# lambdaclass/AES_zero_knowledge_proof_circuit

Measured on AMD Instinct MI355X. Metric: AES-ECB blocks proven/sec (Marlin), proof verifies, higher is better.
Workload: dtype u32 limbs (253-bit Fr / 377-bit Fq modular integers)

## Files before the change

### aes_zero_knowledge_proof_circuit_amd/api.py

```python
import ctypes as C
import os

import numpy as np

HERE = os.path.dirname(os.path.abspath(__file__))
CIRCUIT_AES, CIRCUIT_OPS_XOR, CIRCUIT_OPS_ADD = 0, 1, 2
CIRCUIT_AES_CBC = 3
CIRCUIT_AES_CTR = 4
CIRCUIT_AES_GCM = 5
KEY_NO_TABLES = 1
PARITY = "parity"


class ZkAesError(RuntimeError):
    """The Err(..) side of the reference's anyhow::Result."""


def lib_path():
    return os.path.join(HERE, "libzkaes.so")


_lib = None


# ... 369 lines not shown
def verify_chunked_tagged(verifying_key, circuit, proofs, ciphertext, key_tag, iv=None):
    if len(key_tag) not in (16, 32):
        raise ZkAesError("key_tag must be 16 or 32 bytes")
    if iv is not None and len(iv) != 16:
        raise ZkAesError("iv / icb must be 16 bytes")
    n = len(proofs)
    lens = (C.c_size_t * max(n, 1))(*[len(p) for p in proofs])
    each = (C.c_int * max(n, 1))()
    ok = C.c_size_t()
    _check(lib().zkaes_verify_chunked_kt(verifying_key._p, int(circuit), b"".join(bytes(p) for p in proofs), lens, C.c_size_t(n), None if iv is None else bytes(iv), bytes(ciphertext),
                                         C.c_size_t(len(ciphertext)), bytes(key_tag), C.c_size_t(len(key_tag)), each, C.byref(ok)))
    return [bool(each[i]) for i in range(n)]


def _host_key(secret_key):
    if len(secret_key) not in (16, 24, 32):
        raise ZkAesError("secret_key must be 16, 24 or 32 bytes")


def ecb_ciphertext(message, secret_key):
    _host_key(secret_key)
    ct = C.create_string_buffer(max(len(message), 1))
    _check(lib().zkaes_ecb_ciphertext_ks(bytes(message), C.c_size_t(len(message)), bytes(secret_key), C.c_size_t(len(secret_key)), ct))
    return ct.raw[:len(message)]


def encrypt(message, secret_key, proving_key, zk_seed=None):
    proving_key._need_key(secret_key)
    out, n = C.c_void_p(), C.c_size_t()
    _check(lib().zkaes_encrypt_seeded(bytes(message), C.c_size_t(len(message)), bytes(secret_key), proving_key._p, zk_seed, C.byref(out), C.byref(n)))
    return _take(out, n)


def verify_encryption(verifying_key, proof, ciphertext):
    acc = C.c_int()
    _check(lib().zkaes_verify_encryption(verifying_key._p, bytes(proof), C.c_size_t(len(proof)), bytes(ciphertext), C.c_size_t(len(ciphertext)), C.byref(acc)))
    return bool(acc.value)


def cbc_ciphertext(message, secret_key, iv):
    if len(secret_key) not in (16, 24, 32) or len(iv) != 16:
        raise ZkAesError("secret_key must be 16, 24 or 32 bytes and iv 16 bytes")
    ct = C.create_string_buffer(max(len(message), 1))
    _check(lib().zkaes_cbc_ciphertext_ks(bytes(message), C.c_size_t(len(message)), bytes(secret_key), C.c_size_t(len(secret_key)), bytes(iv), ct))
    return ct.raw[:len(message)]


def encrypt_cbc(message, secret_key, iv, proving_key, zk_seed=None):
    proving_key._need_key(secret_key, iv, "iv")
    ct = C.create_string_buffer(max(len(message), 1))
    out, n = C.c_void_p(), C.c_size_t()
    _check(lib().zkaes_encrypt_cbc_seeded(bytes(message), C.c_size_t(len(message)), bytes(secret_key), bytes(iv), proving_key._p, zk_seed, ct, C.byref(out), C.byref(n)))
    return ct.raw[:len(message)], _take(out, n)


def verify_encryption_cbc(verifying_key, proof, iv, ciphertext):
    if len(iv) != 16:
        raise ZkAesError("iv must be 16 bytes")
    acc = C.c_int()
    _check(lib().zkaes_verify_encryption_cbc(verifying_key._p, bytes(proof), C.c_size_t(len(proof)), bytes(iv), bytes(ciphertext), C.c_size_t(len(ciphertext)), C.byref(acc)))
    return bool(acc.value)


def verify_cbc_chunked(verifying_key, proofs, iv, ciphertext):
    if len(iv) != 16:
        raise ZkAesError("iv must be 16 bytes")
    n = len(proofs)
    lens = (C.c_size_t * max(n, 1))(*[len(p) for p in proofs])
    each = (C.c_int * max(n, 1))()
    ok = C.c_size_t()
    _check(lib().zkaes_verify_cbc_chunked(verifying_key._p, b"".join(bytes(p) for p in proofs), lens, C.c_size_t(n), bytes(iv), bytes(ciphertext), C.c_size_t(len(ciphertext)), each, C.byref(ok)))
    return [bool(each[i]) for i in range(n)]


def ctr_crypt(data, secret_key, icb):
    if len(secret_key) not in (16, 24, 32) or len(icb) != 16:
        raise ZkAesError("secret_key must be 16, 24 or 32 bytes and icb 16 bytes")
    out = C.create_string_buffer(max(len(data), 1))
    _check(lib().zkaes_ctr_crypt_ks(bytes(data), C.c_size_t(len(data)), bytes(secret_key), C.c_size_t(len(secret_key)), bytes(icb), out))
    return out.raw[:len(data)]


def ctr_counter_add(icb, n_blocks):
    if len(icb) != 16 or not 0 <= n_blocks < 1 << 64:
        raise ZkAesError("icb must be 16 bytes and n_blocks a 64-bit count")
    out = C.create_string_buffer(16)
    _check(lib().zkaes_ctr_counter_add(bytes(icb), C.c_uint64(n_blocks), out))
    return out.raw


def encrypt_ctr(message, secret_key, icb, proving_key, zk_seed=None):
    proving_key._need_key(secret_key, icb, "icb")
    ct = C.create_string_buffer(max(len(message), 1))
    out, n = C.c_void_p(), C.c_size_t()
    _check(lib().zkaes_encrypt_ctr_seeded(bytes(message), C.c_size_t(len(message)), bytes(secret_key), bytes(icb), proving_key._p, zk_seed, ct, C.byref(out), C.byref(n)))
    return ct.raw[:len(message)], _take(out, n)


def verify_encryption_ctr(verifying_key, proof, icb, ciphertext):
    if len(icb) != 16:
        raise ZkAesError("icb must be 16 bytes")
    acc = C.c_int()
    _check(lib().zkaes_verify_encryption_ctr(verifying_key._p, bytes(proof), C.c_size_t(len(proof)), bytes(icb), bytes(ciphertext), C.c_size_t(len(ciphertext)), C.byref(acc)))
    return bool(acc.value)


def verify_ctr_chunked(verifying_key, proofs, icb, ciphertext):
    if len(icb) != 16:
        raise ZkAesError("icb must be 16 bytes")
    n = len(proofs)
    lens = (C.c_size_t * max(n, 1))(*[len(p) for p in proofs])
    each = (C.c_int * max(n, 1))()
    ok = C.c_size_t()
    _check(lib().zkaes_verify_ctr_chunked(verifying_key._p, b"".join(bytes(p) for p in proofs), lens, C.c_size_t(n), bytes(icb), bytes(ciphertext), C.c_size_t(len(ciphertext)), each, C.byref(ok)))
    return [bool(each[i]) for i in range(n)]


def _gcm_args(secret_key, iv, key_bytes=None):
    if key_bytes is None:
        _host_key(secret_key)
    elif len(secret_key) != key_bytes:
        raise ZkAesError("secret_key must be %d bytes" % key_bytes)
    if len(iv) != 12:
        raise ZkAesError("GCM: only 96-bit (12-byte) IVs are supported")


def synthesize_keys_gcm(plaintext_length, aad_length=0, srs=(866_944, 513, 4_062_064), flags=0, key_bits=128, key_tag_blocks=0):
    return _synthesize(CIRCUIT_AES_GCM, key_bits, plaintext_length, aad_length, srs, flags, key_tag_blocks)


def gcm_encrypt(message, secret_key, iv, aad=b""):
    _gcm_args(secret_key, iv)
    ct, tag = C.create_string_buffer(max(len(message), 1)), C.create_string_buffer(16)
    _check(lib().zkaes_gcm_encrypt_ks(bytes(message), C.c_size_t(len(message)), bytes(secret_key), C.c_size_t(len(secret_key)), bytes(iv), bytes(aad), C.c_size_t(len(aad)), ct, tag))
    return ct.raw[:len(message)], tag.raw


def gcm_decrypt(ciphertext, secret_key, iv, aad, tag):
    _gcm_args(secret_key, iv)
    if len(tag) != 16:
        raise ZkAesError("GCM: only full 16-byte tags are supported")
    msg, ok = C.create_string_buffer(max(len(ciphertext), 1)), C.c_int()
    _check(lib().zkaes_gcm_decrypt_ks(bytes(ciphertext), C.c_size_t(len(ciphertext)), bytes(secret_key), C.c_size_t(len(secret_key)), bytes(iv), bytes(aad), C.c_size_t(len(aad)), bytes(tag),
                                      msg, C.byref(ok)))
    if not ok.value:
        return None
    return msg.raw[:len(ciphertext)]


def encrypt_gcm(message, secret_key, iv, aad, proving_key, zk_seed=None):
    _gcm_args(secret_key, iv, proving_key.key_bytes())
    ct, tag = C.create_string_buffer(max(len(message), 1)), C.create_string_buffer(16)
    out, n = C.c_void_p(), C.c_size_t()
    _check(lib().zkaes_encrypt_gcm_seeded(bytes(message), C.c_size_t(len(message)), bytes(secret_key), bytes(iv), bytes(aad), C.c_size_t(len(aad)), proving_key._p, zk_seed, ct, tag,
                                          C.byref(out), C.byref(n)))
    return ct.raw[:len(message)], tag.raw, _take(out, n)


def verify_encryption_gcm(verifying_key, proof, iv, aad, ciphertext, tag):
    if len(iv) != 12:
        raise ZkAesError("GCM: only 96-bit (12-byte) IVs are supported")
    if len(tag) != 16:
        raise ZkAesError("GCM: only full 16-byte tags are supported")
    acc = C.c_int()
    _check(lib().zkaes_verify_encryption_gcm(verifying_key._p, bytes(proof), C.c_size_t(len(proof)), bytes(iv), bytes(aad), C.c_size_t(len(aad)), bytes(ciphertext),
                                             C.c_size_t(len(ciphertext)), bytes(tag), C.byref(acc)))
    return bool(acc.value)


def verify_encryption_gcm_tagged(verifying_key, proof, iv, aad, ciphertext, tag, key_tag):
    if len(iv) != 12:
        raise ZkAesError("GCM: only 96-bit (12-byte) IVs are supported")
    if len(tag) != 16:
        raise ZkAesError("GCM: only full 16-byte tags are supported")
    if len(key_tag) not in (16, 32):
        raise ZkAesError("key_tag must be 16 or 32 bytes")
    acc = C.c_int()
    _check(lib().zkaes_verify_encryption_gcm_kt(verifying_key._p, bytes(proof), C.c_size_t(len(proof)), bytes(iv), bytes(aad), C.c_size_t(len(aad)), bytes(ciphertext),
                                                C.c_size_t(len(ciphertext)), bytes(tag), bytes(key_tag), C.c_size_t(len(key_tag)), C.byref(acc)))
    return bool(acc.value)


def proof_roundtrip(proof):
    out, n = C.c_void_p(), C.c_size_t()
    _check(lib().zkaes_proof_roundtrip(bytes(proof), C.c_size_t(len(proof)), C.byref(out), C.byref(n)))
    return _take(out, n)


def circuit_info(circuit, plaintext_length, aad_length=0, key_bits=128, key_tag_blocks=0):
    out = (C.c_uint64 * 12)()
    _check(lib().zkaes_circuit_info_kt(int(circuit), C.c_uint(int(key_bits)), _tag_blocks(key_tag_blocks), C.c_size_t(plaintext_length), C.c_size_t(aad_length), out))
    keys = ["raw_constraints", "raw_instance", "raw_witness", "nnz_a", "nnz_b", "nnz_c", "constraints", "instance", "witness", "joint_nnz", "h", "k"]
    return dict(zip(keys, out))


def circuit_matrix(circuit, plaintext_length, which, aad_length=0, key_bits=128, key_tag_blocks=0):
    rows, nnz = C.c_uint64(), C.c_uint64()
    head = (int(circuit), C.c_uint(int(key_bits)), _tag_blocks(key_tag_blocks), C.c_size_t(plaintext_length), C.c_size_t(aad_length), which)
    _check(lib().zkaes_circuit_matrix_kt(*head, C.byref(rows), C.byref(nnz), None, None, None))
    rowptr = np.zeros(rows.value + 1, dtype=np.uint32)
    col = np.zeros(max(nnz.value, 1), dtype=np.uint32)
    coeff = np.zeros(max(nnz.value, 1), dtype=np.int64)
    _check(lib().zkaes_circuit_matrix_kt(*head, None, None, rowptr.ctypes.data_as(C.c_void_p), col.ctypes.data_as(C.c_void_p), coeff.ctypes.data_as(C.c_void_p)))
    return rowptr, col[:nnz.value], coeff[:nnz.value]


def ntt(field_id, data_mont_bytes, inverse=False):
    n = len(data_mont_bytes) // 32
    buf = C.create_string_buffer(bytes(data_mont_bytes), len(data_mont_bytes))
    _check(lib().zkaes_ntt(int(field_id), buf, C.c_size_t(n), 1 if inverse else 0))
    return buf.raw


def ntt_coset(field_id, data_mont_bytes, coset_c, lg_big, inverse=False):
    n = len(data_mont_bytes) // 32
    buf = C.create_string_buffer(bytes(data_mont_bytes), len(data_mont_bytes))
    _check(lib().zkaes_ntt_coset(int(field_id), buf, C.c_size_t(n), 1 if inverse else 0, int(coset_c), int(lg_big)))
    return buf.raw


def ntt_batch(field_id, vectors, cosets=None, lg_big=0, inverse=False):
    count, n = len(vectors), len(vectors[0]) // 32
    if any(len(v) != 32 * n for v in vectors):
        raise ZkAesError("ntt_batch: vectors of one length")
    buf = C.create_string_buffer(b"".join(bytes(v) for v in vectors), 32 * n * count)
    cs = (C.c_int * count)(*[int(c) for c in cosets]) if cosets is not None else None
    _check(lib().zkaes_ntt_batch(int(field_id), buf, C.c_size_t(n), count, 1 if inverse else 0, cs, int(lg_big)))
    return [buf.raw[32 * n * i:32 * n * (i + 1)] for i in range(count)]


def _ptr_array(bufs):
    n = len(bufs)
    return (C.c_char_p * n)(*[bytes(b) if len(b) else None for b in bufs]), (C.c_size_t * n)(*[len(b) // 32 for b in bufs])


def poly_divide_by_vanishing(p, m, with_scratch=False, want_rem=True):
    n = len(p) // 32
    q = C.create_string_buffer(32 * max(n - m, 0) or 1)
    rem = C.create_string_buffer(32 * m or 1) if want_rem else None
    _check(lib().zkaes_poly_divide_by_vanishing(bytes(p), C.c_size_t(n), C.c_size_t(m), 1 if with_scratch else 0, q, rem))
    return q.raw[:32 * (n - m)], (rem.raw[:32 * m] if want_rem else None)


def poly_divide_by_linear(p, z):
    n = len(p) // 32
    q = C.create_string_buffer(32 * max(n - 1, 0) or 1)
    _check(lib().zkaes_poly_divide_by_linear(bytes(p), C.c_size_t(n), bytes(z), q))
    return q.raw[:32 * max(n - 1, 0)]


def poly_eval_multi(polys, xs):
    count = len(polys)
    ptrs, lens = _ptr_array(polys)
    out = C.create_string_buffer(32 * max(count, 1))
    _check(lib().zkaes_poly_eval_multi(ptrs, lens, b"".join(bytes(x) for x in xs), count, out))
    return [out.raw[32 * i:32 * i + 32] for i in range(count)]


def batch_inverse(v, post=None, throughput_variant=False):
    n = len(v) // 32
    buf = C.create_string_buffer(bytes(v), max(len(v), 1))
    _check(lib().zkaes_batch_inverse(buf, C.c_size_t(n), None if post is None else bytes(post), 1 if throughput_variant else 0))
    return buf.raw[:32 * n]


def poly_lincomb(polys, scalars, n):
    count = len(polys)
    ptrs, lens = _ptr_array(polys)
    out = C.create_string_buffer(32 * n or 1)
    _check(lib().zkaes_poly_lincomb(ptrs, lens, b"".join(bytes(x) for x in scalars), count, C.c_size_t(n), out))
    return out.raw[:32 * n]


def vanishing_quotient_evals(lg_n, gs, a, indices=None):
    ncosets, per = len(gs), (1 << lg_n) if indices is None else len(indices)
    out = C.create_string_buffer(32 * per * ncosets or 1)
    idx = None if indices is None else (C.c_uint32 * max(per, 1))(*indices)
    _check(lib().zkaes_vanishing_quotient_evals(int(lg_n), b"".join(bytes(g) for g in gs), ncosets, bytes(a), idx, C.c_size_t(0 if indices is None else per), out))
    return [out.raw[32 * per * c:32 * per * (c + 1)] for c in range(ncosets)]


def q1_coset_pointwise(r, za, zb, t, z, ca, cb, cz, eta_a, eta_b, eta_c):
    n = len(r) // 32
    out = C.create_string_buffer(32 * n or 1)
    consts = b"".join(bytes(x) for x in (ca, cb, cz, eta_a, eta_b, eta_c))
    _check(lib().zkaes_q1_coset_pointwise(bytes(r), bytes(za), bytes(zb), bytes(t), bytes(z), consts, C.c_size_t(n), out))
    return out.raw[:32 * n]


def h2_coset(row, col, va, vb, vc, rc, f, alpha, beta, alpha_beta, ea, eb, ec, vinv):
    k = len(row) // 32
    out = C.create_string_buffer(32 * k or 1)
    arrays = (C.c_char_p * 7)(*[bytes(x) for x in (row, col, va, vb, vc, rc, f)])
    consts = b"".join(bytes(x) for x in (alpha, beta, alpha_beta, ea, eb, ec, vinv))
    _check(lib().zkaes_h2_coset(arrays, consts, C.c_size_t(k), out))
    return out.raw[:32 * k]


def q1_combine(q0, q1, q3, mask, inv2, inv2zeta):
    n = len(q0) // 32
    h1, g1 = C.create_string_buffer(64 * n or 1), C.create_string_buffer(32 * max(n - 1, 0) or 1)
    _check(lib().zkaes_q1_combine(bytes(q0), bytes(q1), bytes(q3), bytes(mask), bytes(inv2), bytes(inv2zeta), C.c_size_t(n), h1, g1))
    return h1.raw[:64 * n], g1.raw[:32 * max(n - 1, 0)]


def coset_scale(data, g, n):
    out = C.create_string_buffer(32 * n or 1)
    _check(lib().zkaes_coset_scale(bytes(data), C.c_size_t(len(data) // 32), bytes(g), C.c_size_t(n), out))
    return out.raw[:32 * n]


def z_poly_from_w(w, x_poly, n):
    out = C.create_string_buffer(32 * (n + 1))
    _check(lib().zkaes_z_poly_from_w(bytes(w), C.c_size_t(len(w) // 32), bytes(x_poly), C.c_uint32(len(x_poly) // 32), C.c_size_t(n), out))
    return out.raw


def ntt_padded(field_id, data_mont_bytes, n, inverse=False, coset_c=0, lg_big=0):
    out = C.create_string_buffer(32 * n)
    _check(lib().zkaes_ntt_padded(int(field_id), bytes(data_mont_bytes), C.c_size_t(len(data_mont_bytes) // 32), C.c_size_t(n), 1 if inverse else 0, int(coset_c), int(lg_big), out))
    return out.raw


def ntt_scaled(g, data_mont_bytes, n, inverse=False):
    out = C.create_string_buffer(32 * n)
    _check(lib().zkaes_ntt_scaled(bytes(g), bytes(data_mont_bytes), C.c_size_t(len(data_mont_bytes) // 32), C.c_size_t(n), 1 if inverse else 0, out))
    return out.raw


def _arith_ops():
    t = {}
    for base, f, n in ((0, "fr377", 8), (16, "fr381", 8), (32, "fq377", 12), (48, "fq381", 12)):
        for i, (name, nin) in enumerate((("mul", 2 * n), ("add", 2 * n), ("sub", 2 * n), ("neg", n), ("dbl", n), ("inverse", n), ("from_i64", 2), ("pow_u64", n + 2), ("from_raw", n), ("to_raw", n))):
            t["%s.%s" % (f, name)] = (base + i, nin, n)
    for base, f in ((64, "fq377x28"), (96, "fq381x28")):
        ops = [("mul", 28, 14), ("sqr", 14, 14), ("fma2", 56, 14), ("add", 28, 14), ("add_lazy", 28, 14), ("dbl_lazy", 14, 14)]
        ops += [("sub%d" % k, 28, 14) for k in (2, 3, 4, 5, 6, 7)] + [("sub_lazy%d" % k, 28, 14) for k in (2, 3)]
        ops += [("canonical", 14, 14), ("product_is_zero", 14, 1), ("is_zero_mod_p", 14, 1), ("from_std", 12, 14), ("to_std", 14, 12)]
        if f == "fq377x28":
            ops.append(("mul_biased", 28, 14))
        for i, (name, nin, nout) in enumerate(ops):
            t["%s.%s" % (f, name)] = (base + i, nin, nout)
    for base, f in ((128, "fr377x29"), (160, "fr381x29")):
        ops = [("mul", 18, 9), ("dot2", 36, 9), ("dot3", 54, 9), ("dot4", 72, 9), ("add", 18, 9), ("add_lazy", 18, 9)]
        ops += [("sub%d" % k, 18, 9) for k in (1, 2, 4, 8)] + [("sub_lazy2", 18, 9), ("normalized", 9, 9), ("shl5", 9, 9)]
        ops += [("canonical%d" % k, 9, 9) for k in (0, 1, 4)] + [("reduce_by_top_limb", 9, 9), ("twiddle_from_std", 8, 9), ("split", 8, 9), ("pack", 9, 8)]
        for i, (name, nin, nout) in enumerate(ops):
            t["%s.%s" % (f, name)] = (base + i, nin, nout)
    for i, (name, nin, nout) in enumerate((("te_madd", 98, 56), ("te_add", 112, 56), ("te_dbl", 56, 56), ("te_neg", 56, 56), ("te_to_std_point", 56, 48), ("niels_from_weierstrass", 24, 43),
                                           ("te_madd_hot", 142, 98), ("te_add_quad", 112, 56), ("te_dbl_quad", 56, 56))):
        t["te377.%s" % name] = (192 + i, nin, nout)
    for base, f in ((208, "w377"), (216, "w381")):
        for i, (name, nin, nout) in enumerate((("madd28", 84, 57), ("add28", 112, 56), ("dbl28", 56, 56), ("neg28", 56, 56), ("to_std_point", 56, 48))):
            t["%s.%s" % (f, name)] = (base + i, nin, nout)
    return t


ARITH_OPS = _arith_ops()
ARITH_QUAD_OPS = ("te377.te_add_quad", "te377.te_dbl_quad")


def arith_probe(op_name, cases):
    op, nin, nout = ARITH_OPS[op_name]
    cases = bytes(cases)
    n, rest = divmod(len(cases), 4 * nin)
    if rest:
        raise ZkAesError("arith_probe: %s takes %d words per case" % (op_name, nin))
    out = C.create_string_buffer(4 * nout * n or 1)
    _check(lib().zkaes_arith_probe(int(op), cases, C.c_size_t(n), out))
    return out.raw[:4 * nout * n]


def msm(curve_id, bases_bytes, scalars_bytes):
    n = len(scalars_bytes) // 32
    out = C.create_string_buffer(96)
    inf = C.c_int()
    _check(lib().zkaes_msm(int(curve_id), bytes(bases_bytes), bytes(scalars_bytes), C.c_size_t(n), out, C.byref(inf)))
    return out.raw, bool(inf.value)


def g1_sum(curve_id, points):
    n = len(points)
    buf = b"".join(bytes(p[0]) for p in points)
    inf = (C.c_int * max(n, 1))(*[1 if p[1] else 0 for p in points])
    out = C.create_string_buffer(96)
    oinf = C.c_int()
    _check(lib().zkaes_g1_sum(int(curve_id), buf, inf, C.c_size_t(n), out, C.byref(oinf)))
    return out.raw, bool(oinf.value)


def msm_sharded_plan(curve_id, n_total):
    c, w, b = C.c_int(), C.c_int(), C.c_size_t()
    _check(lib().zkaes_msm_sharded_plan(int(curve_id), C.c_size_t(n_total), C.byref(c), C.byref(w), C.byref(b)))
    return c.value, w.value, b.value


def msm_window_sums_dev(curve_id, bases_bytes, scalars_bytes, n_total, dev_ptr, dev_bytes):
    n = len(scalars_bytes) // 32
    _check(lib().zkaes_msm_window_sums_dev(int(curve_id), bytes(bases_bytes), bytes(scalars_bytes), C.c_size_t(n), C.c_size_t(n_total), C.c_void_p(dev_ptr), C.c_size_t(dev_bytes)))


def msm_fold_window_sums_dev(curve_id, dev_ptr, world, n_total):
    out = C.create_string_buffer(96)
    inf = C.c_int()
    _check(lib().zkaes_msm_fold_window_sums_dev(int(curve_id), C.c_void_p(dev_ptr), int(world), C.c_size_t(n_total), out, C.byref(inf)))
    return out.raw, bool(inf.value)


def msm_fold_partials_dev(curve_id, dev_ptr, world):
    out = C.create_string_buffer(96)
    inf = C.c_int()
    _check(lib().zkaes_msm_fold_partials_dev(int(curve_id), C.c_void_p(dev_ptr), int(world), out, C.byref(inf)))
    return out.raw, bool(inf.value)


def msm_table(curve_id, bases_bytes, scalars_bytes, window_bits, srs=False):
    n = len(scalars_bytes) // 32
    out = C.create_string_buffer(96)
    inf = C.c_int()
    if srs:
        if int(curve_id) != 377:
            raise ValueError("the SRS (twisted Edwards) table path exists for BLS12-377 only")
        _check(lib().zkaes_msm_table_srs(bytes(bases_bytes), bytes(scalars_bytes), C.c_size_t(n), int(window_bits), out, C.byref(inf)))
    else:
        _check(lib().zkaes_msm_table(int(curve_id), bytes(bases_bytes), bytes(scalars_bytes), C.c_size_t(n), int(window_bits), out, C.byref(inf)))
    return out.raw, bool(inf.value)


def _host(buf):
    if isinstance(buf, np.ndarray):
        if not buf.flags["C_CONTIGUOUS"]:
            raise ValueError("array arguments must be C-contiguous")
        return buf.ctypes.data_as(C.c_void_p)
    return bytes(buf)


def _nbytes(buf):
    return buf.nbytes if isinstance(buf, np.ndarray) else len(buf)


def class_sum(bases, vals, edwards=True, prior_msm_points=0):
    n, count = _nbytes(bases) // 96, len(vals)
    v = np.ascontiguousarray(np.stack([np.asarray(x, dtype=np.int8) for x in vals])) if count else np.zeros((0, n), dtype=np.int8)
    if count and v.shape[1] != n:
        raise ValueError("every value vector needs one value per base")
    ok, inf, out = (C.c_int * max(count, 1))(), (C.c_int * max(count, 1))(), C.create_string_buffer(96 * max(count, 1))
    _check(lib().zkaes_class_sum(_host(bases), C.c_size_t(n), v.ctypes.data_as(C.c_void_p), int(count), 1 if edwards else 0, C.c_size_t(prior_msm_points), ok, out, inf))
    return [(bool(ok[i]), out.raw[96 * i:96 * i + 96], bool(inf[i])) for i in range(count)]


def msm_pair(bases, scal1, scal2, val_off2, edwards=True):
    out, inf = C.create_string_buffer(96), C.c_int()
    _check(lib().zkaes_msm_pair(_host(bases), C.c_size_t(_nbytes(bases) // 96), bytes(scal1), C.c_size_t(len(scal1) // 32), bytes(scal2), C.c_size_t(len(scal2) // 32), C.c_size_t(val_off2),
                                1 if edwards else 0, out, C.byref(inf)))
    return out.raw, bool(inf.value)


def msm_table_pair(bases, scal1, off1, scal2, off2, window_bits, edwards=True):
    out, inf = C.create_string_buffer(96), C.c_int()
    _check(lib().zkaes_msm_table_pair(_host(bases), C.c_size_t(_nbytes(bases) // 96), bytes(scal1), C.c_size_t(len(scal1) // 32), C.c_size_t(off1), bytes(scal2), C.c_size_t(len(scal2) // 32),
                                      C.c_size_t(off2), int(window_bits), 1 if edwards else 0, out, C.byref(inf)))
    return out.raw, bool(inf.value)


def msm_second_bases(bases, scalars, off, shift, window_bits=0):
    out, inf = C.create_string_buffer(192), (C.c_int * 2)()
    _check(lib().zkaes_msm_second_bases(_host(bases), C.c_size_t(_nbytes(bases) // 96), bytes(scalars), C.c_size_t(len(scalars) // 32), C.c_size_t(off), C.c_size_t(shift), int(window_bits), out, inf))
    return [(out.raw[96 * i:96 * i + 96], bool(inf[i])) for i in range(2)]


def msm_bench(curve_id, bases_bytes, scalars_bytes, reps=3):
    n = len(scalars_bytes) // 32
    t, a = C.c_double(), C.c_double()
    _check(lib().zkaes_msm_bench(int(curve_id), bytes(bases_bytes), bytes(scalars_bytes), C.c_size_t(n), int(reps), C.byref(t), C.byref(a)))
    return t.value, a.value


def msm_bench_synth(n, window_bits=0, reps=3, want_point=False):
    t, a = C.c_double(), C.c_double()
    out = C.create_string_buffer(96)
    _check(lib().zkaes_msm_bench_synth(C.c_size_t(n), int(window_bits), int(reps), C.byref(t), C.byref(a), out))
    return (t.value, a.value, out.raw) if want_point else (t.value, a.value)


def set_default_contexts(n):
    _check(lib().zkaes_set_default_contexts(C.c_size_t(n)))


def srs_hold(hold=True):
    _check(lib().zkaes_srs_hold(1 if hold else 0))


def int_rate_bench(seconds=0.5):
    out = (C.c_double * 8)()
    _check(lib().zkaes_int_rate_bench(C.c_double(seconds), out))
    return {"fq_products_per_s": out[0], "fq_stream_sclk_mhz": out[1], "mad_per_s": 378.0 * out[0], "hot_loop_l2_additions_per_s": out[2], "hot_loop_l2_sclk_mhz": out[3],
            "hot_loop_cycles_per_addition_per_wave": out[4], "rounds": int(out[5])}


def stream_copy_bench(nbytes=1 << 30, reps=20):
    g = C.c_double()
    _check(lib().zkaes_stream_copy_bench(C.c_size_t(nbytes), int(reps), C.byref(g)))
    return g.value


def mem_info():
    f, t = C.c_uint64(), C.c_uint64()
    _check(lib().zkaes_mem_info(C.byref(f), C.byref(t)))
    return int(f.value), int(t.value)


def msm_stats(reset=False):
    out = (C.c_double * 5)()
    _check(lib().zkaes_msm_stats(out, 1 if reset else 0))
    return dict(accumulate_ms=out[0], total_ms=out[1], points=int(out[2]), launches=int(out[3]), pairs=int(out[4]))
```

### aes_zero_knowledge_proof_circuit_amd/build.py

```python
import os
import subprocess
import sys
from concurrent.futures import ThreadPoolExecutor

HERE = os.path.dirname(os.path.abspath(__file__))
CSRC = os.path.join(HERE, "csrc")
OUT = os.path.join(HERE, "libzkaes.so")
OBJ = os.path.join(CSRC, "build")
HIPCC = os.environ.get("HIPCC", "/opt/rocm/bin/hipcc")
HIP_SOURCES = ["runtime.hip", "kernels_ntt.hip", "kernels_msm.hip", "kernels_poly.hip", "kernels_witness.hip", "capi_kernels.hip", "capi_probe.hip"]
CXX_SOURCES = ["circuit.cpp", "marlin.cpp", "marlin_codec.cpp", "capi.cpp", "capi_host.cpp"]
HOST_ONLY_SOURCES = ["circuit.cpp", "marlin_codec.cpp", "capi_host.cpp"]
HEADERS = ["ff.cuh", "ff28.cuh", "ff29.cuh", "ec.cuh", "ec28.cuh", "te28.cuh", "gpu.hpp", "hip_util.hpp", "consts32.h", "trace_layout.h", "circuit.hpp", "marlin.hpp", "marlin_host.hpp", "capi_common.hpp", "pairing.hpp", "transcript.hpp", "arith_probe.cuh",
           os.path.join("..", "..", "include", "zkaes.h")]
COMMON = ["-O3", "-std=c++17", "-fPIC", "-I", CSRC, "-Wno-unused-result"]
if os.environ.get("ZK_EXTRA_DEFINES"):
    COMMON += os.environ["ZK_EXTRA_DEFINES"].split()


def _newer(target, deps):
    if not os.path.exists(target):
        return True
    t = os.path.getmtime(target)
    return any(os.path.getmtime(d) > t for d in deps)


def _compile(src):
    obj = os.path.join(OBJ, src + ".o")
    deps = [os.path.join(CSRC, src)] + [os.path.join(CSRC, h) for h in HEADERS]
    if not _newer(obj, deps):
        return obj
    if src.endswith(".hip"):
        cmd = [HIPCC, "--offload-arch=gfx950", "-x", "hip"] + COMMON + ["-c", os.path.join(CSRC, src), "-o", obj]
    else:
        cmd = [HIPCC, "-x", "c++"] + COMMON + ["-c", os.path.join(CSRC, src), "-o", obj]
    subprocess.check_call(cmd)
    return obj


def build(force=False):
    os.makedirs(OBJ, exist_ok=True)
    if force:
        for f in os.listdir(OBJ):
            os.remove(os.path.join(OBJ, f))
    with ThreadPoolExecutor(max_workers=8) as ex:
        objs = list(ex.map(_compile, HIP_SOURCES + CXX_SOURCES))
    if force or _newer(OUT, objs):
        subprocess.check_call([HIPCC, "--offload-arch=gfx950", "-shared", "-fPIC", "-o", OUT] + objs)
    return OUT


if __name__ == "__main__":
    print(build(force="--force" in sys.argv))
```

### aes_zero_knowledge_proof_circuit_amd/csrc/capi_kernels.hip

```cpp
#include "../../include/zkaes.h"
#include <cstring>
#include <string>
#include <type_traits>
#include <vector>
#include "hip_util.hpp"
#include "marlin.hpp"
#include "te28.cuh"
#include <algorithm>
#include <chrono>

typedef unsigned int v4u __attribute__((ext_vector_type(4)));
__global__ void __launch_bounds__(256) k_stream_copy(uint4 *__restrict__ dst_, const uint4 *__restrict__ src_, size_t n16) {
    v4u *dst = (v4u *)dst_; const v4u *src = (const v4u *)src_;
    size_t base = (size_t)blockIdx.x * 1024 + threadIdx.x;
    if (base + 768 < n16) {
        v4u v0 = __builtin_nontemporal_load(src + base), v1 = __builtin_nontemporal_load(src + base + 256);
        v4u v2 = __builtin_nontemporal_load(src + base + 512), v3 = __builtin_nontemporal_load(src + base + 768);
        __builtin_nontemporal_store(v0, dst + base); __builtin_nontemporal_store(v1, dst + base + 256);
        __builtin_nontemporal_store(v2, dst + base + 512); __builtin_nontemporal_store(v3, dst + base + 768);
    } else {
        for (size_t i = base; i < n16; i += 256) dst[i] = src[i];
    }
}

// ... 237 lines not shown
    WorkspaceGuard ws;
    if (prior) {
        std::vector<MFr> sc(prior);
        uint64_t x = 88172645463325252ull;
        for (size_t i = 0; i < prior; i++) { for (int k = 0; k < 8; k += 2) { x ^= x << 13; x ^= x >> 7; x ^= x << 17; sc[i].l[k] = (uint32_t)x; sc[i].l[k + 1] = (uint32_t)(x >> 32); } sc[i].l[7] &= 0x0fffffffu; }
        DevPtr<MFr> ds = upload_scalars((const uint8_t *)sc.data(), prior, s);
        zk::gpu::sync(s);
        (void)zk::gpu::msm<MC>(ws, (const MsmBase<EDWARDS> *)dl.get(), (const MFr *)ds.get(), prior, s);
    }
    for (int v = 0; v < count; v++) {
        zk::XYZZ<MFq> r;
        const bool ok = zk::gpu::class_sum<MC>(ws, (const MsmBase<EDWARDS> *)dl.get(), (const int8_t *)dv.get() + (size_t)v * n, n, &r, s);
        ok_out[v] = ok ? 1 : 0;
        if (ok) give_affine(r.to_affine(), out_xy + 96 * (size_t)v, out_inf + v);
        else { memset(out_xy + 96 * (size_t)v, 0, 96); out_inf[v] = 0; }
    }
}
template <bool EDWARDS>
void run_msm_pair(const uint8_t *bases, size_t nbases, const uint8_t *scal1, size_t n1, const uint8_t *scal2, size_t n2, size_t val_off2, uint8_t *out_xy, int *out_inf) {
    zk::gpu::require_device();
    StreamGuard s;
    DevPtr<zk::Affine<MFq>> db = upload_points(bases, nbases, nbases, s);
    DevPtr<MsmBase<EDWARDS>> dl = law_bases<EDWARDS>(db, nbases, s);
    DevPtr<MFr> d1 = upload_scalars(scal1, n1, s), d2 = upload_scalars(scal2, n2, s);
    zk::gpu::sync(s);
    WorkspaceGuard ws;
    zk::gpu::msm_prepare<MC>(ws, d1, n1, n2 ? d2.get() : nullptr, n2, n2 ? val_off2 : 0, s);
    give_affine(zk::gpu::msm_finish<MC>(ws, (const MsmBase<EDWARDS> *)dl.get(), s).to_affine(), out_xy, out_inf);
}
template <bool EDWARDS> DevPtr<MsmBase<EDWARDS>> law_tables(const uint8_t *bases, size_t stride, int c, zk::gpu::stream_t s) {
    const size_t nt = (size_t)zk::gpu::table_windows<MC>(c);
    DevPtr<zk::Affine<MFq>> tab = upload_points(bases, stride, nt * stride, s);
    zk::gpu::build_window_tables<MC>(tab, stride, c, s);
    return law_bases<EDWARDS>(tab, nt * stride, s);
}
template <bool EDWARDS>
void run_msm_table_pair(const uint8_t *bases, size_t stride, const uint8_t *scal1, size_t n1, size_t off1, const uint8_t *scal2, size_t n2, size_t off2, int c, uint8_t *out_xy, int *out_inf) {
    zk::gpu::require_device();
    StreamGuard s;
    DevPtr<MsmBase<EDWARDS>> tabs = law_tables<EDWARDS>(bases, stride, c, s);
    DevPtr<MFr> d1 = upload_scalars(scal1, n1, s), d2 = upload_scalars(scal2, n2, s);
    zk::gpu::sync(s);
    WorkspaceGuard ws;
    zk::gpu::msm_prepare_table<MC>(ws, d1, n1, off1, n2 ? d2.get() : nullptr, n2, n2 ? off2 : 0, c, stride, s);
    give_affine(zk::gpu::msm_finish<MC>(ws, (const MsmBase<EDWARDS> *)tabs.get(), s).to_affine(), out_xy, out_inf);
}
void run_msm_second_bases(const uint8_t *bases, size_t nbases, const uint8_t *scalars, size_t n, size_t off, size_t shift, int c, uint8_t *out_xy, int *out_inf) {
    zk::gpu::require_device();
    StreamGuard s;
    DevPtr<MFr> ds = upload_scalars(scalars, n, s);
    WorkspaceGuard ws;
    zk::XYZZ<MFq> r[2];
    if (c == 0) {
        DevPtr<zk::Affine<MFq>> db = upload_points(bases, nbases, nbases, s);
        DevPtr<zk::Niels28<MP>> dl = law_bases<true>(db, nbases, s);
        zk::gpu::msm_prepare<MC>(ws, ds, n, nullptr, 0, 0, s);
        zk::gpu::msm_finish2<MC>(ws, dl.get() + off, dl.get() + off + shift, r, s);
    } else {
        DevPtr<zk::Niels28<MP>> tabs = law_tables<true>(bases, nbases, c, s);
        zk::gpu::msm_prepare_table<MC>(ws, ds, n, off, nullptr, 0, 0, c, nbases, s);
        zk::gpu::msm_finish2<MC>(ws, tabs.get(), tabs.get() + shift, r, s);
    }
    for (int i = 0; i < 2; i++) give_affine(r[i].to_affine(), out_xy + 96 * i, out_inf + i);
}
}

extern "C" {
int zkaes_class_sum(const uint8_t *bases, size_t n, const int8_t *vals, int count, int edwards, size_t prior_msm_points, int *ok_out, uint8_t *out_xy, int *out_inf) {
    return guardk([&] {
        const char *who = "zkaes_class_sum";
        need(count >= 1 && count <= 8, who, "1..8 value vectors");
        need(bases && vals && ok_out && out_xy && out_inf, who, "null argument");
        need(n >= 1 && n <= MSM_FORM_MAX, who, "n out of range");
        need(prior_msm_points <= n, who, "the prior MSM runs over the same bases: at most n points");
        if (edwards) run_class_sum<true>(bases, n, vals, count, prior_msm_points, ok_out, out_xy, out_inf);
        else run_class_sum<false>(bases, n, vals, count, prior_msm_points, ok_out, out_xy, out_inf);
    });
}
int zkaes_msm_pair(const uint8_t *bases, size_t nbases, const uint8_t *scal1, size_t n1, const uint8_t *scal2, size_t n2, size_t val_off2, int edwards, uint8_t *out_xy, int *out_inf) {
    return guardk([&] {
        const char *who = "zkaes_msm_pair";
        need(out_xy && out_inf && (bases || !nbases) && (scal1 || !n1) && (scal2 || !n2), who, "null argument");
        need(nbases <= MSM_FORM_MAX, who, "too many bases");
        need(n1 <= nbases && val_off2 <= nbases && n2 <= nbases - val_off2, who, "range exceeds the bases");
        if (edwards) run_msm_pair<true>(bases, nbases, scal1, n1, scal2, n2, val_off2, out_xy, out_inf);
        else run_msm_pair<false>(bases, nbases, scal1, n1, scal2, n2, val_off2, out_xy, out_inf);
    });
}
int zkaes_msm_table_pair(const uint8_t *bases, size_t stride, const uint8_t *scal1, size_t n1, size_t off1, const uint8_t *scal2, size_t n2, size_t off2, int window_bits, int edwards,
                         uint8_t *out_xy, int *out_inf) {
    return guardk([&] {
        const char *who = "zkaes_msm_table_pair";
        need(out_xy && out_inf && (bases || !stride) && (scal1 || !n1) && (scal2 || !n2), who, "null argument");
        need(stride <= MSM_FORM_MAX, who, "too many bases");
        check_table_bits(window_bits, stride, who);
        if (off1 > stride || n1 > stride - off1 || off2 > stride || n2 > stride - off2) throw std::invalid_argument("msm_table: range exceeds the table");
        if (edwards) run_msm_table_pair<true>(bases, stride, scal1, n1, off1, scal2, n2, off2, window_bits, out_xy, out_inf);
        else run_msm_table_pair<false>(bases, stride, scal1, n1, off1, scal2, n2, off2, window_bits, out_xy, out_inf);
    });
}
int zkaes_msm_second_bases(const uint8_t *bases, size_t nbases, const uint8_t *scalars, size_t n, size_t off, size_t shift, int window_bits, uint8_t *out_xy, int *out_inf) {
    return guardk([&] {
        const char *who = "zkaes_msm_second_bases";
        need(out_xy && out_inf && (bases || !nbases) && (scalars || !n), who, "null argument");
        need(nbases <= MSM_FORM_MAX, who, "too many bases");
        if (window_bits) check_table_bits(window_bits, nbases, who);
        if (off > nbases || shift > nbases - off || n > nbases - off - shift) throw std::invalid_argument(window_bits ? "msm_table: range exceeds the table" : "zkaes_msm_second_bases: range exceeds the bases");
        run_msm_second_bases(bases, nbases, scalars, n, off, shift, window_bits, out_xy, out_inf);
    });
}
int zkaes_msm_sharded_plan(int curve_id, size_t n_total, int *window_bits, int *n_windows, size_t *bytes_per_rank) {
    return guardk([&] {
        int c = 0, w = 0;
        if (curve_id == 381) zk::gpu::msm_sharded_plan<zk::Bls381>(n_total, &c, &w); else if (curve_id == 377) zk::gpu::msm_sharded_plan<zk::Bls377>(n_total, &c, &w); else throw std::invalid_argument("curve_id must be 377 or 381");
        if (window_bits) *window_bits = c;
        if (n_windows) *n_windows = w;
        if (bytes_per_rank) *bytes_per_rank = (size_t)w * 192;
    });
}
int zkaes_msm_window_sums_dev(int curve_id, const uint8_t *bases, const uint8_t *scalars, size_t n_local, size_t n_total, void *dev_out, size_t dev_out_bytes) {
    return guardk([&] { if (curve_id == 381) run_msm_window_sums_dev<zk::Bls381>(bases, scalars, n_local, n_total, dev_out, dev_out_bytes); else if (curve_id == 377) run_msm_window_sums_dev<zk::Bls377>(bases, scalars, n_local, n_total, dev_out, dev_out_bytes); else throw std::invalid_argument("curve_id must be 377 or 381"); });
}
int zkaes_msm_fold_window_sums_dev(int curve_id, const void *dev_in, int world, size_t n_total, uint8_t *out_xy, int *out_inf) {
    return guardk([&] { if (curve_id == 381) run_msm_fold_dev<zk::Bls381>(dev_in, world, n_total, out_xy, out_inf); else if (curve_id == 377) run_msm_fold_dev<zk::Bls377>(dev_in, world, n_total, out_xy, out_inf); else throw std::invalid_argument("curve_id must be 377 or 381"); });
}
int zkaes_g1_sum(int curve_id, const uint8_t *points_xy, const int *inf, size_t n, uint8_t *out_xy, int *out_inf) {
    return guardk([&] { if (curve_id == 381) run_g1_sum<zk::Bls381>(points_xy, inf, n, out_xy, out_inf); else if (curve_id == 377) run_g1_sum<zk::Bls377>(points_xy, inf, n, out_xy, out_inf); else throw std::invalid_argument("curve_id must be 377 or 381"); });
}
int zkaes_msm_fold_partials_dev(int curve_id, const void *dev_in, int world, uint8_t *out_xy, int *out_inf) {
    return guardk([&] {
        if (!dev_in || world < 1 || world > MAX_FOLD_WORLD) throw std::invalid_argument("zkaes_msm_fold_partials_dev: bad arguments (world must be 1..4096)");
        if (curve_id != 377 && curve_id != 381) throw std::invalid_argument("curve_id must be 377 or 381");
        zk::gpu::require_device();
        StreamGuard s;
        if (curve_id == 377) give_affine(zk::gpu::msm_fold_points_device<zk::Bls377>((const zk::XYZZ<zk::Fq377> *)dev_in, world, s).to_affine(), out_xy, out_inf);
        else give_affine(zk::gpu::msm_fold_points_device<zk::Bls381>((const zk::XYZZ<zk::Fq381> *)dev_in, world, s).to_affine(), out_xy, out_inf);
    });
}
int zkaes_msm_table(int curve_id, const uint8_t *bases, const uint8_t *scalars, size_t n, int window_bits, uint8_t *out_xy, int *out_inf) {
    return guardk([&] { if (curve_id == 381) run_msm_table<zk::Bls381, false>(bases, scalars, n, window_bits, out_xy, out_inf); else if (curve_id == 377) run_msm_table<zk::Bls377, false>(bases, scalars, n, window_bits, out_xy, out_inf); else throw std::invalid_argument("curve_id must be 377 or 381"); });
}
int zkaes_msm_table_srs(const uint8_t *bases, const uint8_t *scalars, size_t n, int window_bits, uint8_t *out_xy, int *out_inf) {
    return guardk([&] { run_msm_table<zk::Bls377, true>(bases, scalars, n, window_bits, out_xy, out_inf); });
}
int zkaes_set_device(int ordinal) { return guardk([&] { HIP_CHECK(hipSetDevice(ordinal)); }); }
int zkaes_ntt(int field_id, uint8_t *data, size_t n, int inverse) {
    return guardk([&] { if (field_id == 381) run_ntt<zk::Fr381>(data, n, inverse, 0, 0); else if (field_id == 377) run_ntt<zk::Fr377>(data, n, inverse, 0, 0); else throw std::invalid_argument("field_id must be 377 or 381"); });
}
int zkaes_ntt_coset(int field_id, uint8_t *data, size_t n, int inverse, int coset_c, int lg_big) {
    return guardk([&] {
        if (coset_c <= 0) throw std::invalid_argument("zkaes_ntt_coset: coset index must be positive");
        if (field_id == 381) run_ntt<zk::Fr381>(data, n, inverse, coset_c, lg_big); else if (field_id == 377) run_ntt<zk::Fr377>(data, n, inverse, coset_c, lg_big); else throw std::invalid_argument("field_id must be 377 or 381");
    });
}
int zkaes_ntt_batch(int field_id, uint8_t *data, size_t n, int count, int inverse, const int *coset_c, int lg_big) {
    return guardk([&] {
        if (field_id == 381) run_ntt_batch<zk::Fr381>(data, n, count, inverse, coset_c, lg_big); else if (field_id == 377) run_ntt_batch<zk::Fr377>(data, n, count, inverse, coset_c, lg_big);
        else throw std::invalid_argument("field_id must be 377 or 381");
    });
}
int zkaes_poly_divide_by_vanishing(const uint8_t *p, size_t len, size_t m, int with_scratch, uint8_t *q, uint8_t *rem_or_null) {
    return guardk([&] {
        const char *who = "zkaes_poly_divide_by_vanishing";
        if (m == 0 || len <= m) throw std::invalid_argument("divide_by_vanishing: dividend shorter than divisor");
        need(p && q, who, "null argument"); need(len <= POLY_MAX, who, "polynomial too long");
        zk::gpu::require_device();
        StreamGuard s;
        DevPtr<PF> dp = upload(p, len, s), dq(len - m), drem(m), scratch;
        size_t scratch_len = 0;
        if (with_scratch) { scratch_len = zk::gpu::divide_by_vanishing_scratch(len, m); scratch.alloc(scratch_len ? scratch_len : 1); }
        zk::gpu::divide_by_vanishing(dq, rem_or_null ? drem.get() : nullptr, dp, len, m, s, with_scratch ? scratch.get() : nullptr, scratch_len);
        zk::gpu::d2h(q, dq, (len - m) * sizeof(PF), s);
        if (rem_or_null) zk::gpu::d2h(rem_or_null, drem, m * sizeof(PF), s);
    });
}
int zkaes_poly_divide_by_linear(const uint8_t *p, size_t len, const uint8_t z[32], uint8_t *q) {
    return guardk([&] {
        const char *who = "zkaes_poly_divide_by_linear";
        const PF zf = load_f(z, who);
        need(len <= POLY_MAX, who, "polynomial too long"); need(len < 2 || (p && q), who, "null argument");
        if (len < 2) return;
        zk::gpu::require_device();
        StreamGuard s;
        const size_t scratch_len = zk::gpu::divide_by_linear_scratch(len);
        DevPtr<PF> dp = upload(p, len, s), dq(len - 1), scratch(scratch_len);
        zk::gpu::divide_by_linear(dq, dp, len, zf, scratch, scratch_len, s);
        zk::gpu::d2h(q, dq, (len - 1) * sizeof(PF), s);
    });
}
int zkaes_poly_eval_multi(const uint8_t *const *polys, const size_t *lens, const uint8_t *x, int count, uint8_t *out) {
    return guardk([&] {
        const char *who = "zkaes_poly_eval_multi";
        need(count >= 1 && count <= 8, who, "1..8 polynomials"); need(polys && lens && x && out, who, "null argument");
        size_t scratch_len = 8;
        for (int i = 0; i < count; i++) { need(lens[i] <= POLY_MAX, who, "polynomial too long"); need(!lens[i] || polys[i], who, "null polynomial"); scratch_len += zk::gpu::poly_eval_scratch(lens[i]); }
        zk::gpu::require_device();
        StreamGuard s;
        DevPtr<PF> dp[8];
        const PF *ptr[8];
        PF xs[8], res[8];
        for (int i = 0; i < count; i++) { dp[i] = upload(polys[i], lens[i], s); ptr[i] = dp[i]; xs[i] = load_f(x + 32 * i, who); }
        DevPtr<PF> scratch(scratch_len);
        zk::gpu::poly_eval_multi(ptr, lens, xs, count, res, scratch, scratch_len, s);
        memcpy(out, res, (size_t)count * sizeof(PF));
    });
}
int zkaes_batch_inverse(uint8_t *v, size_t n, const uint8_t *post_or_null, int throughput_variant) {
    return guardk([&] {
        const char *who = "zkaes_batch_inverse";
        need(v || !n, who, "null argument"); need(n <= POLY_MAX, who, "vector too long");
        PF post; if (post_or_null) post = load_f(post_or_null, who);
        if (!n) return;
        zk::gpu::require_device();
        StreamGuard s;
        DevPtr<PF> dv = upload(v, n, s);
        {
            zk::gpu::ThroughputWaits as_between_overlapping_proofs(throughput_variant != 0);
            zk::gpu::batch_inverse(dv, n, post_or_null ? &post : nullptr, s);
            zk::gpu::sync(s);
        }
        zk::gpu::d2h(v, dv, n * sizeof(PF), s);
    });
}
int zkaes_poly_lincomb(const uint8_t *const *polys, const size_t *lens, const uint8_t *scalars, int count, size_t n, uint8_t *out) {
    return guardk([&] {
        const char *who = "zkaes_poly_lincomb";
        need(count >= 1 && count <= 8, who, "1..8 terms"); need(polys && lens && scalars && (out || !n), who, "null argument"); need(n <= POLY_MAX, who, "polynomial too long");
        for (int i = 0; i < count; i++) { need(lens[i] <= n, who, "a term longer than the result"); need(!lens[i] || polys[i], who, "null polynomial"); }
        if (!n) return;
        zk::gpu::require_device();
        StreamGuard s;
        DevPtr<PF> dp[8], dout(n);
        const PF *ptr[8];
        PF sc[8];
        for (int i = 0; i < count; i++) { dp[i] = upload(polys[i], lens[i], s); ptr[i] = dp[i]; sc[i] = load_f(scalars + 32 * i, who); }
        zk::gpu::poly_lincomb_n(dout, n, ptr, lens, sc, count, s);
        zk::gpu::d2h(out, dout, n * sizeof(PF), s);
    });
}
int zkaes_vanishing_quotient_evals(int lg_n, const uint8_t *g, int ncosets, const uint8_t a[32], const uint32_t *idx_or_null, size_t nidx, uint8_t *out) {
    return guardk([&] {
        const char *who = "zkaes_vanishing_quotient_evals";
        need(lg_n >= 0 && lg_n <= 24, who, "lg_n must be in [0, 24]"); need(ncosets >= 1 && ncosets <= 3, who, "1..3 cosets"); need(g && out, who, "null argument");
        const size_t n = (size_t)1 << lg_n;
        for (size_t i = 0; idx_or_null && i < nidx; i++) need(idx_or_null[i] < n, who, "index out of range");
        const PF af = load_f(a, who);
        PF gs[3];
        for (int c = 0; c < ncosets; c++) gs[c] = load_f(g + 32 * c, who);
        zk::gpu::require_device();
        StreamGuard s;
        const PF *elems = zk::gpu::domain_elements<zk::Fr377>(lg_n);
        const size_t scratch_len = zk::gpu::vanishing_quotient_scratch(lg_n, ncosets);
        DevPtr<PF> tabs[3], scratch(scratch_len);
        PF *outs[3] = {nullptr, nullptr, nullptr};
        for (int c = 0; c < ncosets; c++) { tabs[c].alloc(n); outs[c] = tabs[c]; }
        zk::gpu::vanishing_quotient_evals(outs, gs, ncosets, af, elems, (uint32_t)n, lg_n, scratch, scratch_len, s);
        if (!idx_or_null) { for (int c = 0; c < ncosets; c++) zk::gpu::d2h(out + (size_t)c * n * sizeof(PF), tabs[c], n * sizeof(PF), s); return; }
        std::vector<PF> host(n);
        for (int c = 0; c < ncosets; c++) {
            zk::gpu::d2h(host.data(), tabs[c], n * sizeof(PF), s);
            for (size_t i = 0; i < nidx; i++) memcpy(out + ((size_t)c * nidx + i) * sizeof(PF), &host[idx_or_null[i]], sizeof(PF));
        }
    });
}
int zkaes_q1_coset_pointwise(const uint8_t *r, const uint8_t *za, const uint8_t *zb, const uint8_t *t, const uint8_t *z, const uint8_t consts[192], size_t n, uint8_t *out) {
    return guardk([&] {
        const char *who = "zkaes_q1_coset_pointwise";
        need(r && za && zb && t && z && consts && out, who, "null argument"); need(n >= 1 && n <= POLY_MAX, who, "n out of range");
        PF c[6];
        for (int i = 0; i < 6; i++) c[i] = load_f(consts + 32 * i, who);
        zk::gpu::require_device();
        StreamGuard s;
        DevPtr<PF> dr = upload(r, n, s), dza = upload(za, n, s), dzb = upload(zb, n, s), dt = upload(t, n, s), dz = upload(z, n, s), dout(n);
        zk::gpu::q1_coset_pointwise(dout, dr, dza, dzb, dt, dz, c[0], c[1], c[2], c[3], c[4], c[5], n, s);
        zk::gpu::d2h(out, dout, n * sizeof(PF), s);
    });
}
int zkaes_h2_coset(const uint8_t *const arrays[7], const uint8_t consts[224], size_t k, uint8_t *out) {
    return guardk([&] {
        const char *who = "zkaes_h2_coset";
        need(arrays && consts && out, who, "null argument"); need(k >= 1 && k <= POLY_MAX, who, "k out of range");
        for (int i = 0; i < 7; i++) need(arrays[i], who, "null array");
        PF c[7];
        for (int i = 0; i < 7; i++) c[i] = load_f(consts + 32 * i, who);
        zk::gpu::require_device();
        StreamGuard s;
        DevPtr<PF> d[7], dout(k);
        for (int i = 0; i < 7; i++) d[i] = upload(arrays[i], k, s);
        zk::gpu::h2_coset(dout, d[0], d[1], d[2], d[3], d[4], d[5], d[6], c[0], c[1], c[2], c[3], c[4], c[5], c[6], k, s);
        zk::gpu::d2h(out, dout, k * sizeof(PF), s);
    });
}
int zkaes_q1_combine(const uint8_t *q0, const uint8_t *q1, const uint8_t *q3, const uint8_t *mask, const uint8_t inv2[32], const uint8_t inv2zeta[32], size_t n, uint8_t *h1, uint8_t *g1) {
    return guardk([&] {
        const char *who = "zkaes_q1_combine";
        need(q0 && q1 && q3 && mask && h1 && (g1 || n < 2), who, "null argument"); need(n >= 1 && n <= POLY_MAX / 4, who, "n out of range");
        const PF i2 = load_f(inv2, who), i2z = load_f(inv2zeta, who);
        zk::gpu::require_device();
        StreamGuard s;
        DevPtr<PF> d0 = upload(q0, n, s), d1 = upload(q1, n, s), d3 = upload(q3, n, s), dm = upload(mask, 3 * n, s), dh(2 * n), dg(n);
        zk::gpu::q1_combine(dh, dg, d0, d1, d3, dm, i2, i2z, n, s);
        zk::gpu::d2h(h1, dh, 2 * n * sizeof(PF), s);
        zk::gpu::d2h(g1, dg, (n - 1) * sizeof(PF), s);
    });
}
int zkaes_coset_scale(const uint8_t *in, size_t in_len, const uint8_t g[32], size_t n, uint8_t *out) {
    return guardk([&] {
        const char *who = "zkaes_coset_scale";
        need((in || !in_len) && (out || !n), who, "null argument"); need(n <= POLY_MAX && in_len <= POLY_MAX, who, "polynomial too long");
        const PF gf = load_f(g, who);
        if (!n) return;
        zk::gpu::require_device();
        StreamGuard s;
        DevPtr<PF> din = upload(in, in_len, s), dout(n);
        zk::gpu::coset_scale(dout, din, gf, in_len, n, s);
        zk::gpu::d2h(out, dout, n * sizeof(PF), s);
    });
}
int zkaes_z_poly_from_w(const uint8_t *w, size_t wlen, const uint8_t *x_poly, uint32_t m, size_t n, uint8_t *zp) {
    return guardk([&] {
        const char *who = "zkaes_z_poly_from_w";
        need((w || !wlen) && (x_poly || !m) && zp, who, "null argument"); need(n < POLY_MAX && wlen <= POLY_MAX, who, "polynomial too long");
        zk::gpu::require_device();
        StreamGuard s;
        DevPtr<PF> dw = upload(w, wlen, s), dx = upload(x_poly, m, s), dz(n + 1);
        zk::gpu::z_poly_from_w(dz, dw, wlen, dx, m, n, s);
        zk::gpu::d2h(zp, dz, (n + 1) * sizeof(PF), s);
    });
}
int zkaes_ntt_padded(int field_id, const uint8_t *in, size_t in_len, size_t n, int inverse, int coset_c, int lg_big, uint8_t *out) {
    return guardk([&] {
        if (field_id == 381) run_ntt_padded<zk::Fr381>(in, in_len, n, inverse, coset_c, lg_big, out); else if (field_id == 377) run_ntt_padded<zk::Fr377>(in, in_len, n, inverse, coset_c, lg_big, out);
        else throw std::invalid_argument("field_id must be 377 or 381");
    });
}
int zkaes_ntt_scaled(const uint8_t g[32], const uint8_t *in, size_t in_len, size_t n, int inverse, uint8_t *out) {
    return guardk([&] {
        const char *who = "zkaes_ntt_scaled";
        const int lg = exact_log2(n, who);
        need(lg >= 1 && lg <= 28, who, "n must be in [2, 2^28]"); need(in_len <= n, who, "in_len must not exceed n"); need(out && (in || !in_len), who, "null argument");
        const PF gf = load_f(g, who);
        need(!gf.is_zero(), who, "the coset generator must not be zero");
        zk::gpu::require_device();
        StreamGuard s;
        DevPtr<void> table = zk::gpu::coset_power_table<PF>(inverse ? gf.inverse() : gf, n, s);
        DevPtr<PF> a = upload(in, in_len, s), b(n);
        zk::gpu::ntt_scaled<PF>(b, a, in_len, lg, inverse != 0, table, s);
        zk::gpu::d2h(out, b, n * sizeof(PF), s);
    });
}
int zkaes_msm(int curve_id, const uint8_t *bases, const uint8_t *scalars, size_t n, uint8_t *out_xy, int *out_inf) {
    return guardk([&] { if (curve_id == 381) run_msm<zk::Bls381>(bases, scalars, n, out_xy, out_inf, 0, nullptr, nullptr); else if (curve_id == 377) run_msm<zk::Bls377>(bases, scalars, n, out_xy, out_inf, 0, nullptr, nullptr); else throw std::invalid_argument("curve_id must be 377 or 381"); });
}
int zkaes_msm_bench(int curve_id, const uint8_t *bases, const uint8_t *scalars, size_t n, int reps, double *ms_total, double *ms_accumulate) {
    return guardk([&] { if (curve_id == 381) run_msm<zk::Bls381>(bases, scalars, n, nullptr, nullptr, reps, ms_total, ms_accumulate); else run_msm<zk::Bls377>(bases, scalars, n, nullptr, nullptr, reps, ms_total, ms_accumulate); });
}
int zkaes_msm_bench_synth(size_t n, int window_bits, int reps, double *ms_total, double *ms_accumulate, uint8_t *out_xy) {
    return guardk([&] {
        using Fq = zk::Fq377; using Fr = zk::Fr377;
        if (!ms_total || !ms_accumulate || reps < 1 || n == 0 || window_bits > 22) throw std::invalid_argument("zkaes_msm_bench_synth: bad arguments");
        zk::gpu::require_device();
        const size_t nt = window_bits > 0 ? (size_t)zk::gpu::table_windows<zk::Bls377>(window_bits) : 1;
        if ((uint64_t)nt * n >= (1ull << 30)) throw std::invalid_argument("zkaes_msm_bench_synth: n x table copies exceeds the 2^30 base indices of one MSM");
        StreamGuard s;
        DevPtr<zk::Affine<Fq>> tab(nt * n);
        zk::Affine<Fq> g; for (int i = 0; i < 12; i++) { g.x.l[i] = G1_377_X_MONT[i]; g.y.l[i] = G1_377_Y_MONT[i]; }
        Fr beta = Fr::from_u64(0x9e3779b97f4a7c15ull) * Fr::from_u64(0xc2b2ae3d27d4eb4full);
        zk::gpu::fixed_base_powers<zk::Bls377>(tab, g, beta, 1, n, s);
        if (window_bits > 0) zk::gpu::build_window_tables<zk::Bls377>(tab, n, window_bits, s);
        const bool edwards = window_bits != 0;
        DevPtr<zk::Affine28<zk::Fq377P>> tab28;
        DevPtr<zk::Niels28<zk::Fq377P>> tabte;
        if (edwards) { tabte.alloc(nt * n); zk::gpu::convert_bases_te<zk::Bls377>(tabte, tab, nt * n, s); }
        else { tab28.alloc(nt * n); zk::gpu::convert_bases<zk::Bls377>(tab28, tab, nt * n, s); }
        std::vector<Fr> sc(n);
        uint64_t x = 88172645463325252ull;
        for (size_t i = 0; i < n; i++) { for (int k = 0; k < 8; k += 2) { x ^= x << 13; x ^= x >> 7; x ^= x << 17; sc[i].l[k] = (uint32_t)x; sc[i].l[k + 1] = (uint32_t)(x >> 32); } sc[i].l[7] &= 0x0fffffffu; }
        DevPtr<Fr> ds(n);
        zk::gpu::h2d(ds, sc.data(), n * 32, s);
        zk::gpu::sync(s);
        WorkspaceGuard ws;
        auto run = [&]() -> zk::XYZZ<Fq> {
            if (edwards) return window_bits > 0 ? zk::gpu::msm_table<zk::Bls377>(ws, tabte, n, 0, window_bits, ds, n, s) : zk::gpu::msm<zk::Bls377>(ws, tabte.get(), ds.get(), n, s);
            return window_bits > 0 ? zk::gpu::msm_table<zk::Bls377>(ws, tab28, n, 0, window_bits, ds, n, s) : zk::gpu::msm<zk::Bls377>(ws, tab28.get(), ds.get(), n, s);
        };
        give_affine(run().to_affine(), out_xy, nullptr);
        zk::gpu::MsmStats before = zk::gpu::msm_stats(false);
        EventGuard e0, e1;
        zk::gpu::event_record(e0, s);
        for (int i = 0; i < reps; i++) run();
        zk::gpu::event_record(e1, s);
        float ms = zk::gpu::event_elapsed_ms(e0, e1);
        zk::gpu::MsmStats after = zk::gpu::msm_stats(false);
        *ms_total = ms / reps; *ms_accumulate = (after.accumulate_ms - before.accumulate_ms) / reps;
    });
}

int zkaes_stream_copy_bench(size_t bytes, int reps, double *gb_per_s) {
    return guardk([&] {
        if (bytes < 4096 || reps < 1 || !gb_per_s) throw std::invalid_argument("zkaes_stream_copy_bench: bytes >= 4096, reps >= 1");
        zk::gpu::require_device();
        StreamGuard s;
        const size_t n16 = bytes / 16;
        DevPtr<uint4> a(n16), b(n16);
        zk::gpu::dzero(a, n16 * 16, s);
        hipStream_t hs = (hipStream_t)s.h;
        k_stream_copy<<<(unsigned)((n16 + 1023) / 1024), 256, 0, hs>>>(b, a, n16);
        EventGuard e0, e1;
        zk::gpu::event_record(e0, s);
        for (int i = 0; i < reps; i++) k_stream_copy<<<(unsigned)((n16 + 1023) / 1024), 256, 0, hs>>>(i & 1 ? a.get() : b.get(), i & 1 ? b.get() : a.get(), n16);
        zk::gpu::event_record(e1, s);
        float ms = zk::gpu::event_elapsed_ms(e0, e1);
        *gb_per_s = 2.0 * (double)(n16 * 16) * reps / 1e9 / (ms / 1e3);
    });
}
int zkaes_int_rate_bench(double seconds, double out[8]) {
    return guardk([&] {
        if (!out || !(seconds > 0.0) || seconds > 30.0) throw std::invalid_argument("zkaes_int_rate_bench: 0 < seconds <= 30, out != NULL");
        zk::gpu::require_device();
        using P = zk::Fq377P; using G = zk::FpMsm<P>;
        StreamGuard s;
        hipStream_t hs = (hipStream_t)s.h;
        const int GRID_A = 4096, ITERS_A = 300, GRID_B = 8192, ITERS_B = 83;
        const uint32_t NREC = 4096;
        DevPtr<CalStamp> st(GRID_B);
        DevPtr<G> sink_a((size_t)GRID_A * 64);
        DevPtr<zk::AccTE<P>> sink_b((size_t)GRID_B * 64);
        DevPtr<zk::Niels28<P>> tab(NREC);
        k_cal_fill<<<NREC / 256, 256, 0, hs>>>(tab, NREC);
        G ga; for (int k = 0; k < 14; k++) ga.l[k] = 0x0123457u + 977u * k;
        std::vector<double> rate_a, mhz_a, rate_b, mhz_b, cyc_b;
        std::vector<CalStamp> h(GRID_B);
        auto median = [](std::vector<double> &v) { std::sort(v.begin(), v.end()); return v.empty() ? 0.0 : v[v.size() / 2]; };
        auto stamps = [&](int grid, double per_wave_units, double *mhz, double *cyc_per_unit) {
            zk::gpu::d2h(h.data(), st, (size_t)grid * sizeof(CalStamp), s);
            std::vector<double> m(grid), c(grid);
            for (int i = 0; i < grid; i++) { m[i] = (double)h[i].cyc / ((double)h[i].rt / 1e8) / 1e6; c[i] = (double)h[i].cyc / per_wave_units; }
            *mhz = median(m); *cyc_per_unit = median(c);
        };
        EventGuard e0, e1;
        const auto t_begin = std::chrono::steady_clock::now();
        int rounds = 0;
        while (rounds < 3 || std::chrono::duration<double>(std::chrono::steady_clock::now() - t_begin).count() < seconds) {
            double mhz, cyc;
            zk::gpu::event_record(e0, s);
            k_cal_fqmul<<<GRID_A, 64, 0, hs>>>(st, sink_a, ga, ITERS_A);
            zk::gpu::event_record(e1, s);
            stamps(GRID_A, 2.0 * ITERS_A, &mhz, &cyc);
            rate_a.push_back(2.0 * ITERS_A * 64.0 * GRID_A / (zk::gpu::event_elapsed_ms(e0, e1) * 1e-3)); mhz_a.push_back(mhz);
            zk::gpu::event_record(e0, s);
            k_cal_hot_loop<<<GRID_B, 64, 0, hs>>>(st, sink_b, tab, NREC - 1, ITERS_B);
            zk::gpu::event_record(e1, s);
            stamps(GRID_B, (double)ITERS_B, &mhz, &cyc);
            rate_b.push_back((double)ITERS_B * 64.0 * GRID_B / (zk::gpu::event_elapsed_ms(e0, e1) * 1e-3)); mhz_b.push_back(mhz); cyc_b.push_back(cyc);
            rounds++;
        }
        out[0] = median(rate_a); out[1] = median(mhz_a); out[2] = median(rate_b); out[3] = median(mhz_b); out[4] = median(cyc_b); out[5] = (double)rounds; out[6] = 0; out[7] = 0;
    });
}
int zkaes_mem_info(uint64_t *free_bytes, uint64_t *total_bytes) {
    return guardk([&] {
        zk::gpu::require_device();
        size_t f = 0, t = 0;
        HIP_CHECK(hipMemGetInfo(&f, &t));
        if (free_bytes) *free_bytes = f;
        if (total_bytes) *total_bytes = t;
    });
}
}
```

### aes_zero_knowledge_proof_circuit_amd/csrc/kernels_poly.hip

```cpp
#include <cstring>
#include <rocprim/device/device_scan.hpp>
#include "ff29.cuh"
#include "hip_util.hpp"

namespace zk {
namespace gpu {

#define GRID(n) dim3((unsigned)(((n) + 255) / 256)), dim3(256)

__global__ void k_set_at(F *p, size_t idx, F val, bool add) { if (threadIdx.x == 0 && blockIdx.x == 0) p[idx] = add ? p[idx] + val : val; }
void poly_set_at(F *p, size_t idx, const F &val, stream_t s) { hipLaunchKernelGGL(k_set_at, dim3(1), dim3(64), 0, (hipStream_t)s, p, idx, val, false); HIP_LAUNCH_CHECK(); }
void poly_add_at(F *p, size_t idx, const F &val, stream_t s) { hipLaunchKernelGGL(k_set_at, dim3(1), dim3(64), 0, (hipStream_t)s, p, idx, val, true); HIP_LAUNCH_CHECK(); }

__global__ void k_scale(F *p, F sc, size_t n) { size_t i = (size_t)blockIdx.x * blockDim.x + threadIdx.x; if (i < n) p[i] = p[i] * sc; }
void poly_scale(F *p, const F &sc, size_t n, stream_t s) { if (!n) return; hipLaunchKernelGGL(k_scale, GRID(n), 0, (hipStream_t)s, p, sc, n); HIP_LAUNCH_CHECK(); }
using G29 = Fp29<Fr377P>;
__device__ __forceinline__ G29 ld29(const F &x) { return G29::split(x.l); }
__device__ __forceinline__ F st29(const G29 &g) { F r; g.template canonical<1>().pack(r.l); return r; }
struct LincombArgs { const F *p[8]; size_t len[8]; G29 sc[8]; int count; };
__global__ void k_lincomb_n(F *__restrict__ out, LincombArgs a, size_t n) {
    size_t i = (size_t)blockIdx.x * blockDim.x + threadIdx.x;
    if (i >= n) return;
    G29 v[8];
#pragma unroll
    for (int j = 0; j < 8; j++) v[j] = (j < a.count && i < a.len[j]) ? ld29(a.p[j][i]) : G29::zero();
    G29 acc = G29::dot<4>(v, a.sc);
    if (a.count > 4) acc = acc + G29::dot<4>(v + 4, a.sc + 4);
    out[i] = st29(acc);
}
void poly_lincomb_n(F *out, size_t n, const F *const *polys, const size_t *lens, const F *scalars, int count, stream_t s) {
    if (!n) return;
    if (count < 1 || count > 8) throw GpuError("poly_lincomb_n: 1..8 terms");
    LincombArgs a;
    a.count = count;
    for (int j = 0; j < 8; j++) { a.p[j] = j < count ? polys[j] : nullptr; a.len[j] = j < count ? lens[j] : 0; a.sc[j] = j < count ? G29::twiddle_from_std(scalars[j]) : G29::zero(); }
    hipLaunchKernelGGL(k_lincomb_n, GRID(n), 0, (hipStream_t)s, out, a, n); HIP_LAUNCH_CHECK();
}

__global__ void k_div_vanishing(F *__restrict__ q, F *__restrict__ rem, const F *__restrict__ p, size_t len, size_t m) {
    size_t j = (size_t)blockIdx.x * blockDim.x + threadIdx.x;
    if (j >= m) return;
    size_t qlen = len - m;
    F carry = F::zero();
    if (qlen > j) {
        size_t top = j + ((qlen - 1 - j) / m) * m;
        for (size_t i = top;; i -= m) {
            carry = p[i + m] + carry;
            q[i] = carry;
            if (i < m) break;
        }
    }
    if (rem) rem[j] = (j < len ? p[j] : F::zero()) + carry;
}
__global__ void k_divvan_sums(F *__restrict__ part, const F *__restrict__ p, size_t qlen, size_t m, size_t C, size_t S) {
    size_t idx = (size_t)blockIdx.x * blockDim.x + threadIdx.x;
    if (idx >= S * m) return;
    const size_t seg = idx / m, j = idx % m;
    F sum = F::zero();
    for (size_t t = seg * C; t < (seg + 1) * C; t++) { size_t i = j + t * m; if (i < qlen) sum = sum + p[i + m]; }
    part[idx] = sum;
}
__global__ void k_divvan_apply(F *__restrict__ q, F *__restrict__ rem, const F *__restrict__ p, const F *__restrict__ part, size_t len, size_t m, size_t C, size_t S) {
    size_t idx = (size_t)blockIdx.x * blockDim.x + threadIdx.x;
    if (idx >= S * m) return;
    const size_t seg = idx / m, j = idx % m, qlen = len - m;
    F carry = F::zero();
    for (size_t u = S; u-- > seg + 1;) carry = carry + part[u * m + j];
    for (size_t t = (seg + 1) * C; t-- > seg * C;) { size_t i = j + t * m; if (i < qlen) { carry = carry + p[i + m]; q[i] = carry; } }
    if (seg == 0 && rem) rem[j] = (j < len ? p[j] : F::zero()) + carry;
}
size_t divide_by_vanishing_scratch(size_t len, size_t m) {
    if (m == 0 || len <= m) return 0;
    const size_t chain = (len - m + m - 1) / m;
    return chain >= 64 ? (chain + 15) / 16 * m : 0;
}
void divide_by_vanishing(F *q, F *rem, const F *p, size_t len, size_t m, stream_t s, F *scratch, size_t scratch_len) {
    if (m == 0 || len <= m) throw GpuError("divide_by_vanishing: dividend shorter than divisor");
    const size_t chain = (len - m + m - 1) / m;
    const size_t C = 16, S = (chain + C - 1) / C;
    if (chain >= 64 && scratch && S * m <= scratch_len) {
        hipLaunchKernelGGL(k_divvan_sums, GRID(S * m), 0, (hipStream_t)s, scratch, p, len - m, m, C, S); HIP_LAUNCH_CHECK();
        hipLaunchKernelGGL(k_divvan_apply, GRID(S * m), 0, (hipStream_t)s, q, rem, p, (const F *)scratch, len, m, C, S); HIP_LAUNCH_CHECK();
        return;
    }
    hipLaunchKernelGGL(k_div_vanishing, GRID(m), 0, (hipStream_t)s, q, rem, p, len, m); HIP_LAUNCH_CHECK();
}

constexpr int DL_B = 16;
__global__ void k_divlin_local(F *__restrict__ q, const F *__restrict__ p, size_t len, F z, F *__restrict__ v, F *__restrict__ zp) {
    if (blockIdx.x == 0 && threadIdx.x < DL_B) zp[threadIdx.x] = z.pow_u64(threadIdx.x);
    const size_t t = (size_t)blockIdx.x * blockDim.x + threadIdx.x, s0 = t * DL_B;
    if (s0 >= len) return;
    const size_t e = s0 + DL_B < len ? s0 + DL_B : len;
    F l = F::zero();
    for (size_t i = e; i-- > s0;) {
        if (i + 1 < len) q[i] = l;
        l = p[i] + z * l;
    }
    v[t] = l;
}
constexpr int DL_TOP_THREADS = 256;
constexpr size_t DL_TOP = (size_t)DL_TOP_THREADS * DL_B;
__global__ void __launch_bounds__(DL_TOP_THREADS) k_divlin_top(F *__restrict__ q, const F *__restrict__ p, size_t len, F z) {
    __shared__ F sh[DL_TOP_THREADS];
    const uint32_t t = threadIdx.x;
    const size_t s0 = (size_t)t * DL_B, e = s0 + DL_B < len ? s0 + DL_B : len;
    F l = F::zero();
    if (s0 < len) {
        for (size_t i = e; i-- > s0;) {
            if (i + 1 < len) q[i] = l;
            l = p[i] + z * l;
        }
    }
    sh[t] = l;
    __syncthreads();
    F y = z.pow_u64(DL_B);
    for (int k = 1; k < DL_TOP_THREADS; k <<= 1) {
        const F other = t + k < DL_TOP_THREADS ? sh[t + k] : F::zero();
        __syncthreads();
        sh[t] = sh[t] + y * other;
        __syncthreads();
        y = y.sqr();
    }
    if (s0 >= len || e >= len) return;
    const F c = sh[t + 1];
    F w = F::one();
    for (size_t i = e; i-- > s0;) { q[i] = q[i] + w * c; w = w * z; }
}
__global__ void __launch_bounds__(256) k_divlin_apply(F *__restrict__ q, size_t qlen, const F *__restrict__ zp_table, const F *__restrict__ carry, size_t nblocks) {
    __shared__ F zp[DL_B];
    if (threadIdx.x < DL_B) zp[threadIdx.x] = zp_table[threadIdx.x];
    __syncthreads();
    const size_t i = (size_t)blockIdx.x * blockDim.x + threadIdx.x;
    if (i >= qlen) return;
    const size_t t = i / DL_B;
    if (t + 1 >= nblocks) return;
    const size_t e = (t + 1) * DL_B;
    q[i] = q[i] + zp[e - 1 - i] * carry[t];
}
size_t divide_by_linear_scratch(size_t len) {
    size_t total = 8;
    for (size_t n = len; n > DL_B; ) { n = (n + DL_B - 1) / DL_B; total += 2 * n + 2 + DL_B; }
    return total;
}
static void divlin_rec(F *q, const F *p, size_t len, const F &z, F *scratch, hipStream_t s) {
    if (len < 2) return;
    if (len <= DL_TOP) { hipLaunchKernelGGL(k_divlin_top, dim3(1), dim3(DL_TOP_THREADS), 0, s, q, p, len, z); HIP_LAUNCH_CHECK(); return; }
    const size_t nblocks = (len + DL_B - 1) / DL_B;
    F *v = scratch, *carry = scratch + nblocks + 1, *zp = carry + nblocks + 1;
    hipLaunchKernelGGL(k_divlin_local, GRID(nblocks), 0, s, q, p, len, z, v, zp); HIP_LAUNCH_CHECK();
    divlin_rec(carry, v, nblocks, z.pow_u64(DL_B), zp + DL_B, s);
    hipLaunchKernelGGL(k_divlin_apply, GRID(len - 1), 0, s, q, len - 1, (const F *)zp, (const F *)carry, nblocks); HIP_LAUNCH_CHECK();
}
void divide_by_linear(F *q, const F *p, size_t len, const F &z, F *scratch, size_t scratch_elems, stream_t s_) {
    hipStream_t s = (hipStream_t)s_;
    if (len < 2) return;
    if (len >= ((size_t)1 << 31)) throw GpuError("divide_by_linear: polynomial too long");
    if (z.is_zero()) { HIP_CHECK(hipMemcpyAsync(q, p + 1, (len - 1) * sizeof(F), hipMemcpyDeviceToDevice, s)); return; }
    if (divide_by_linear_scratch(len) > scratch_elems) throw GpuError("divide_by_linear: scratch too small");
    divlin_rec(q, p, len, z, scratch, s);
}

constexpr size_t EV_CHUNK = 16, EV_COMBINE_MAX = 1024;
__global__ void k_eval_chunks(const F *__restrict__ p, size_t len, F x, F *__restrict__ partial) {
    size_t t = (size_t)blockIdx.x * blockDim.x + threadIdx.x;
    size_t nch = (len + EV_CHUNK - 1) / EV_CHUNK;
    if (t >= nch) return;
    size_t s0 = t * EV_CHUNK, e = s0 + EV_CHUNK < len ? s0 + EV_CHUNK : len;
    F acc = F::zero();
    for (size_t i = e; i-- > s0;) acc = acc * x + p[i];
    partial[t] = acc;
}
__global__ void __launch_bounds__(256) k_eval_combine(const F *__restrict__ partial, size_t nch, F y, F *__restrict__ out) {
    __shared__ F sh[256];
    uint32_t t = threadIdx.x;
    F y256 = y.pow_u64(256), pw = y.pow_u64(t), acc = F::zero();
    for (size_t i = t; i < nch; i += 256) { acc = acc + partial[i] * pw; pw = pw * y256; }
    sh[t] = acc;
    __syncthreads();
    for (int s = 128; s > 0; s >>= 1) { if ((int)t < s) sh[t] = sh[t] + sh[t + s]; __syncthreads(); }
    if (t == 0) out[0] = sh[0];
}
size_t poly_eval_scratch(size_t len) {
    size_t tot = 0, n = len;
    do { n = (n + EV_CHUNK - 1) / EV_CHUNK; tot += n; } while (n > EV_COMBINE_MAX);
    return tot;
}
static void eval_launch(const F *p, size_t len, F x, F *scratch, F *out, hipStream_t s) {
    const F *src = p;
    size_t n = len;
    F y = x;
    do {
        size_t nch = (n + EV_CHUNK - 1) / EV_CHUNK;
        hipLaunchKernelGGL(k_eval_chunks, GRID(nch), 0, s, src, n, y, scratch); HIP_LAUNCH_CHECK();
        src = scratch; scratch += nch; n = nch; y = y.pow_u64(EV_CHUNK);
    } while (n > EV_COMBINE_MAX);
    hipLaunchKernelGGL(k_eval_combine, dim3(1), dim3(256), 0, s, src, n, y, out); HIP_LAUNCH_CHECK();
}
void poly_eval_multi(const F *const *p, const size_t *len, const F *x, int count, F *out, F *scratch, size_t scratch_elems, stream_t s_) {
    hipStream_t s = (hipStream_t)s_;
    if (count < 1 || count > 8) throw GpuError("poly_eval_multi: 1..8 polynomials");
    size_t need = 8;
    for (int i = 0; i < count; i++) need += poly_eval_scratch(len[i]);
    if (need > scratch_elems) throw GpuError("poly_eval_multi: scratch too small");
    F *res = scratch, *at = scratch + 8;
    bool any = false;
    for (int i = 0; i < count; i++) {
        if (!len[i]) continue;
        eval_launch(p[i], len[i], x[i], at, res + i, s);
        at += poly_eval_scratch(len[i]); any = true;
    }
    F host[8];
    if (any) {
        sync((stream_t)s);
        HIP_CHECK(hipMemcpyAsync(host, res, count * sizeof(F), hipMemcpyDeviceToHost, s));
        sync((stream_t)s);
    }
    for (int i = 0; i < count; i++) out[i] = len[i] ? host[i] : F::zero();
}
F poly_eval(const F *p, size_t len, const F &x, F *scratch, stream_t s_) {
    F out;
    poly_eval_multi(&p, &len, &x, 1, &out, scratch, 8 + poly_eval_scratch(len), s_);
    return out;
}

constexpr int BI_BLOCK = 512;
template <int BI_CHUNK>
__global__ void __launch_bounds__(BI_BLOCK) k_batch_inverse(F *__restrict__ v, size_t n, bool has_post, F post) {
    __shared__ F pre_s[BI_BLOCK], suf_s[BI_BLOCK];
    __shared__ F inv_total;
    const int lane = threadIdx.x;
    size_t t = (size_t)blockIdx.x * BI_BLOCK + lane;
    size_t s0 = t * BI_CHUNK;
    if (s0 > n) s0 = n;
    size_t e = s0 + BI_CHUNK < n ? s0 + BI_CHUNK : n;
    F pre[BI_CHUNK];
    F acc = F::one();
    for (size_t i = s0; i < e; i++) { pre[i - s0] = acc; F x = v[i]; if (!x.is_zero()) acc = acc * x; }
    pre_s[lane] = acc; suf_s[lane] = acc;
    __syncthreads();
    for (int d = 1; d < BI_BLOCK; d <<= 1) {
        F a, b;
        const bool ha = lane >= d, hb = lane + d < BI_BLOCK;
        if (ha) a = pre_s[lane - d];
        if (hb) b = suf_s[lane + d];
        __syncthreads();
        if (ha) pre_s[lane] = pre_s[lane] * a;
        if (hb) suf_s[lane] = suf_s[lane] * b;
        __syncthreads();
    }
    if (lane == 0) { F iv = BI_CHUNK == 4 ? suf_s[0].inverse() : suf_s[0].inverse_fermat(); inv_total = has_post ? iv * post : iv; }
    __syncthreads();
    acc = inv_total;
    if (lane > 0) acc = acc * pre_s[lane - 1];
    if (lane + 1 < BI_BLOCK) acc = acc * suf_s[lane + 1];
    for (size_t i = e; i-- > s0;) {
        F x = v[i];
        if (x.is_zero()) continue;
        v[i] = acc * pre[i - s0];
        acc = acc * x;
    }
}
constexpr int VQ_MAX_COSETS = 3, VQ_STEP = 10;
struct VqArgs { F *out[VQ_MAX_COSETS]; const F *tab; const F *elems; uint32_t n; int lg_n; bool unit_g[VQ_MAX_COSETS]; };
__device__ __forceinline__ F vq_factor(const VqArgs &A, int c, int k, uint32_t j) {
    const F e = A.elems[(size_t)j << k];
    return A.tab[k] + (A.unit_g[c] ? e : e * A.tab[(size_t)(c + 1) * A.lg_n + k]);
}
__global__ void __launch_bounds__(1024) k_vq_top(VqArgs A, F *__restrict__ mid) {
    __shared__ F buf[2][1 << VQ_STEP];
    const int c = blockIdx.x, L = A.lg_n, k_stop = L > VQ_STEP ? L - VQ_STEP : 0;
    const uint32_t t = threadIdx.x;
    if (t == 0) buf[0][0] = F::one();
    __syncthreads();
    int cur = 0;
    for (int k = L - 1; k >= k_stop; k--) {
        const uint32_t s = A.n >> k;
        if (t < s) buf[cur ^ 1][t] = vq_factor(A, c, k, t) * buf[cur][t & ((s >> 1) - 1)];
        __syncthreads();
        cur ^= 1;
    }
    const uint32_t s = A.n >> k_stop;
    F *dst = k_stop == 0 ? A.out[c] : mid + (size_t)c * (1u << VQ_STEP);
    if (t < s) dst[t] = buf[cur][t];
}
__global__ void __launch_bounds__(256) k_vq_expand(VqArgs A, const F *__restrict__ src, F *__restrict__ dst, int k_hi, int k_lo) {
    __shared__ F buf[2][1 << VQ_STEP];
    const uint32_t s_hi = A.n >> k_hi;
    const int c = blockIdx.x / s_hi;
    const uint32_t j = blockIdx.x % s_hi, t = threadIdx.x;
    if (t == 0) buf[0][0] = src[(size_t)c * s_hi + j];
    __syncthreads();
    int cur = 0;
    for (int k = k_hi - 1; k >= k_lo; k--) {
        const uint32_t cnt = 1u << (k_hi - k);
        for (uint32_t m = t; m < cnt; m += 256) buf[cur ^ 1][m] = vq_factor(A, c, k, j + m * s_hi) * buf[cur][m & ((cnt >> 1) - 1)];
        __syncthreads();
        cur ^= 1;
    }
    const uint32_t cnt = 1u << (k_hi - k_lo);
    F *o = k_lo == 0 ? A.out[c] : dst + (size_t)c * (A.n >> k_lo);
    for (uint32_t m = t; m < cnt; m += 256) o[j + (size_t)m * s_hi] = buf[cur][m];
}
static inline int vq_next_level(int k_hi) { const int r = k_hi % VQ_STEP; return k_hi - (r ? r : VQ_STEP); }
size_t vanishing_quotient_scratch(int lg_n, int ncosets) {
    size_t tab = (size_t)(ncosets + 1) * (lg_n > 0 ? lg_n : 1), mids = 0;
    for (int k = lg_n - VQ_STEP; k > 0; k = vq_next_level(k)) mids += (size_t)ncosets << (lg_n - k);
    return tab + mids + 8;
}
void vanishing_quotient_evals(F *const *out, const F *g, int ncosets, const F &a, const F *elems, uint32_t n, int lg_n, F *scratch, size_t scratch_elems, stream_t s_) {
    hipStream_t s = (hipStream_t)s_;
    if (ncosets < 1 || ncosets > VQ_MAX_COSETS) throw GpuError("vanishing_quotient_evals: 1..3 cosets");
    if (n == 0 || n != (1u << lg_n)) throw GpuError("vanishing_quotient_evals: n must be 2^lg_n");
    if (vanishing_quotient_scratch(lg_n, ncosets) > scratch_elems) throw GpuError("vanishing_quotient_evals: scratch too small");
    if (lg_n == 0) { for (int c = 0; c < ncosets; c++) { F one = F::one(); h2d(out[c], &one, sizeof(F), s_); } return; }
    std::vector<F> tab((size_t)(ncosets + 1) * lg_n);
    F v = a;
    for (int k = 0; k < lg_n; k++) { tab[k] = v; v = v.sqr(); }
    VqArgs A;
    for (int c = 0; c < VQ_MAX_COSETS; c++) { A.out[c] = c < ncosets ? out[c] : nullptr; A.unit_g[c] = true; }
    for (int c = 0; c < ncosets; c++) {
        A.unit_g[c] = g[c] == F::one();
        v = g[c];
        for (int k = 0; k < lg_n; k++) { tab[(size_t)(c + 1) * lg_n + k] = v; v = v.sqr(); }
    }
    h2d(scratch, tab.data(), tab.size() * sizeof(F), s_);
    A.tab = scratch; A.elems = elems; A.n = n; A.lg_n = lg_n;
    F *mid = scratch + tab.size();
    hipLaunchKernelGGL(k_vq_top, dim3(ncosets), dim3(1024), 0, s, A, mid); HIP_LAUNCH_CHECK();
    for (int k_hi = lg_n - VQ_STEP; k_hi > 0; ) {
        const int k_lo = vq_next_level(k_hi);
        F *dst = mid + ((size_t)ncosets << (lg_n - k_hi));
        hipLaunchKernelGGL(k_vq_expand, dim3((unsigned)((size_t)ncosets * (n >> k_hi))), dim3(256), 0, s, A, (const F *)mid, dst, k_hi, k_lo); HIP_LAUNCH_CHECK();
        mid = dst; k_hi = k_lo;
    }
}
__global__ void k_f_from_tables(F *__restrict__ out, const F *__restrict__ va, const F *__restrict__ vb, const F *__restrict__ vc, G29 ea, G29 eb, G29 ec, const F *__restrict__ ra,
                                const F *__restrict__ rb, const uint32_t *__restrict__ ri, const uint32_t *__restrict__ ci, size_t k) {
    size_t i = (size_t)blockIdx.x * blockDim.x + threadIdx.x;
    if (i >= k) return;
    const G29 v[3] = {ld29(va[i]), ld29(vb[i]), ld29(vc[i])}, w[3] = {ea, eb, ec};
    const F num = st29(G29::dot<3>(v, w));
    out[i] = num.is_zero() ? num : num * (rb[ci[i]] * ra[ri[i]]);
}
void f_evals_from_tables(F *out, const F *va, const F *vb, const F *vc, const F &ea, const F &eb, const F &ec, const F *ra, const F *rb, const uint32_t *ri, const uint32_t *ci, size_t k,
                         stream_t s) {
    if (!k) return;
    hipLaunchKernelGGL(k_f_from_tables, GRID(k), 0, (hipStream_t)s, out, va, vb, vc, G29::twiddle_from_std(ea), G29::twiddle_from_std(eb), G29::twiddle_from_std(ec), ra, rb, ri, ci, k);
    HIP_LAUNCH_CHECK();
}
void batch_inverse(F *v, size_t n, const F *post, stream_t s) {
    if (!n) return;
    const F post_v = post ? *post : F::one();
    if (throughput_mode() || n > ((size_t)1 << 21)) {
        size_t threads = (n + 15) / 16;
        hipLaunchKernelGGL(k_batch_inverse<16>, dim3((unsigned)((threads + BI_BLOCK - 1) / BI_BLOCK)), dim3(BI_BLOCK), 0, (hipStream_t)s, v, n, post != nullptr, post_v); HIP_LAUNCH_CHECK();
    } else {
        size_t threads = (n + 3) / 4;
        hipLaunchKernelGGL(k_batch_inverse<4>, dim3((unsigned)((threads + BI_BLOCK - 1) / BI_BLOCK)), dim3(BI_BLOCK), 0, (hipStream_t)s, v, n, post != nullptr, post_v); HIP_LAUNCH_CHECK();
    }
}

__global__ void k_q1_coset(F *__restrict__ out, const F *__restrict__ r, const F *__restrict__ za, const F *__restrict__ zb, const F *__restrict__ t, const F *__restrict__ z,
                           F ca, F cb, F cz, G29 ea, G29 eb, G29 ec, size_t n) {
    size_t i = (size_t)blockIdx.x * blockDim.x + threadIdx.x;
    if (i >= n) return;
    const G29 a = ld29(za[i]) + ld29(ca), b = ld29(zb[i]) + ld29(cb), zz = ld29(z[i]) + ld29(cz);
    const G29 v[3] = {a.shl5() * b, a, b}, w[3] = {ec, ea, eb};
    const G29 sum = G29::dot<3>(v, w);
    const G29 l[2] = {ld29(r[i]).shl5(), ld29(t[i]).shl5()}, m[2] = {sum, G29::zero().template sub<2>(zz)};
    out[i] = st29(G29::dot<2>(l, m));
}
void q1_coset_pointwise(F *out, const F *r, const F *za, const F *zb, const F *t, const F *z, const F &ca, const F &cb, const F &cz, const F &ea, const F &eb, const F &ec, size_t n, stream_t s) {
    hipLaunchKernelGGL(k_q1_coset, GRID(n), 0, (hipStream_t)s, out, r, za, zb, t, z, ca, cb, cz, G29::twiddle_from_std(ea), G29::twiddle_from_std(eb), G29::twiddle_from_std(ec), n); HIP_LAUNCH_CHECK();
}
__global__ void k_z_evals_h(F *__restrict__ out, const uint8_t *__restrict__ z, uint32_t n, uint32_t m, uint32_t num_witness) {
    uint32_t k = blockIdx.x * blockDim.x + threadIdx.x;
    if (k >= n) return;
    const uint32_t ratio = n / m;
    uint8_t bit;
    if (k % ratio == 0) bit = z[k / ratio];
    else { const uint32_t wi = k - k / ratio - 1; bit = wi < num_witness ? z[m + wi] : 0; }
    out[k] = bit ? F::one() : F::zero();
}
void z_evals_h(F *out, const uint8_t *z, uint32_t n, uint32_t m, uint32_t num_witness, stream_t s) {
    hipLaunchKernelGGL(k_z_evals_h, GRID(n), 0, (hipStream_t)s, out, z, n, m, num_witness); HIP_LAUNCH_CHECK();
}
__global__ void k_q1_combine(F *__restrict__ h1, F *__restrict__ g1, const F *__restrict__ q0, const F *__restrict__ q1, const F *__restrict__ q3, const F *__restrict__ mask,
                             F inv2, F inv2zeta, size_t n) {
    size_t i = (size_t)blockIdx.x * blockDim.x + threadIdx.x;
    if (i >= n) return;
    const F a = q1[i], b = q3[i], c = q0[i];
    const F q_mid = (a - b) * inv2zeta;
    const F q_hi = ((c - q_mid) - (a + b) * inv2) * inv2;
    const F m_lo = mask[i], m_mid = mask[n + i], m_hi = mask[2 * n + i];
    h1[i] = q_mid + q_hi + m_mid + m_hi;
    h1[n + i] = q_hi + m_hi;
    if (i >= 1) g1[i - 1] = c + m_lo + m_mid + m_hi;
}
void q1_combine(F *h1, F *g1, const F *q0, const F *q1, const F *q3, const F *mask, const F &inv2, const F &inv2zeta, size_t n, stream_t s) {
    hipLaunchKernelGGL(k_q1_combine, GRID(n), 0, (hipStream_t)s, h1, g1, q0, q1, q3, mask, inv2, inv2zeta, n); HIP_LAUNCH_CHECK();
}
__global__ void k_coset_scale(F *__restrict__ out, const F *__restrict__ in, F g, size_t in_len, size_t n) {
    size_t t = (size_t)blockIdx.x * blockDim.x + threadIdx.x;
    size_t j0 = t * 16;
    if (j0 >= n) return;
    size_t e = j0 + 16 < n ? j0 + 16 : n;
    F pw = g.pow_u64(j0);
    for (size_t j = j0; j < e; j++) { out[j] = j < in_len ? in[j] * pw : F::zero(); pw = pw * g; }
}
void coset_scale(F *out, const F *in, const F &g, size_t in_len, size_t n, stream_t s) {
    if (!n) return;
    hipLaunchKernelGGL(k_coset_scale, GRID((n + 15) / 16), 0, (hipStream_t)s, out, in, g, in_len, n); HIP_LAUNCH_CHECK();
}
__global__ void k_h2_coset(F *__restrict__ out, const F *__restrict__ row, const F *__restrict__ col, const F *__restrict__ va, const F *__restrict__ vb,
                           const F *__restrict__ vc, const F *__restrict__ rc, const F *__restrict__ f, G29 alpha, G29 beta, F alpha_beta, G29 ea, G29 eb, G29 ec, G29 vinv, size_t k) {
    size_t i = (size_t)blockIdx.x * blockDim.x + threadIdx.x;
    if (i >= k) return;
    const G29 v3[3] = {ld29(va[i]), ld29(vb[i]), ld29(vc[i])}, w3[3] = {ea, eb, ec};
    const G29 a = G29::dot<3>(v3, w3);
    const G29 v2[2] = {ld29(row[i]), ld29(col[i])}, w2[2] = {alpha, beta};
    const G29 b = (ld29(alpha_beta) + ld29(rc[i])).template sub<2>(G29::dot<2>(v2, w2));
    const G29 bf = b.shl5() * ld29(f[i]);
    out[i] = st29(a.template sub<2>(bf) * vinv);
}
void h2_coset(F *out, const F *row, const F *col, const F *va, const F *vb, const F *vc, const F *rc, const F *f, const F &alpha, const F &beta, const F &alpha_beta,
              const F &ea, const F &eb, const F &ec, const F &vinv, size_t k, stream_t s) {
    hipLaunchKernelGGL(k_h2_coset, GRID(k), 0, (hipStream_t)s, out, row, col, va, vb, vc, rc, f, G29::twiddle_from_std(alpha), G29::twiddle_from_std(beta), alpha_beta,
                       G29::twiddle_from_std(ea), G29::twiddle_from_std(eb), G29::twiddle_from_std(ec), G29::twiddle_from_std(vinv), k); HIP_LAUNCH_CHECK();
}
__global__ void k_z_poly(F *__restrict__ zp, const F *__restrict__ w, size_t wlen, const F *__restrict__ x, uint32_t m, size_t n1) {
    size_t i = (size_t)blockIdx.x * blockDim.x + threadIdx.x;
    if (i >= n1) return;
    F v = F::zero();
    if (i >= m && i - m < wlen) v = w[i - m];
    if (i < wlen) v = v - w[i];
    if (i < m) v = v + x[i];
    zp[i] = v;
}
void z_poly_from_w(F *zp, const F *w, size_t wlen, const F *x_poly, uint32_t m, size_t n, stream_t s) { hipLaunchKernelGGL(k_z_poly, GRID(n + 1), 0, (hipStream_t)s, zp, w, wlen, x_poly, m, n + 1); HIP_LAUNCH_CHECK(); }

__device__ __forceinline__ uint32_t rotl32(uint32_t x, int n) { return (x << n) | (x >> (32 - n)); }
__global__ void k_chacha_blocks(uint32_t *__restrict__ words, uint64_t first_block, uint32_t nblocks, uint32_t k0, uint32_t k1, uint32_t k2, uint32_t k3, uint32_t k4, uint32_t k5,
                                uint32_t k6, uint32_t k7, int rounds) {
    uint32_t b = blockIdx.x * blockDim.x + threadIdx.x;
    if (b >= nblocks) return;
    uint64_t ctr = first_block + b;
    uint32_t s[16] = {0x61707865u, 0x3320646eu, 0x79622d32u, 0x6b206574u, k0, k1, k2, k3, k4, k5, k6, k7, (uint32_t)ctr, (uint32_t)(ctr >> 32), 0, 0};
    uint32_t x[16];
#pragma unroll
    for (int i = 0; i < 16; i++) x[i] = s[i];
#define ZK_QR(a, b, c, d) \
    x[a] += x[b]; x[d] = rotl32(x[d] ^ x[a], 16); x[c] += x[d]; x[b] = rotl32(x[b] ^ x[c], 12); \
    x[a] += x[b]; x[d] = rotl32(x[d] ^ x[a], 8); x[c] += x[d]; x[b] = rotl32(x[b] ^ x[c], 7);
    for (int r = 0; r < rounds; r += 2) {
        ZK_QR(0, 4, 8, 12) ZK_QR(1, 5, 9, 13) ZK_QR(2, 6, 10, 14) ZK_QR(3, 7, 11, 15)
        ZK_QR(0, 5, 10, 15) ZK_QR(1, 6, 11, 12) ZK_QR(2, 7, 8, 13) ZK_QR(3, 4, 9, 14)
    }
#undef ZK_QR
#pragma unroll
    for (int i = 0; i < 16; i++) words[(size_t)b * 16 + i] = x[i] + s[i];
}
__global__ void k_rand_flags(const uint32_t *__restrict__ words, uint32_t word_off, uint32_t ncand, uint32_t *__restrict__ flags) {
    uint32_t j = blockIdx.x * blockDim.x + threadIdx.x;
    if (j >= ncand) return;
    uint32_t l[8];
#pragma unroll
    for (int i = 0; i < 8; i++) l[i] = words[(size_t)word_off + 8 * (size_t)j + i];
    l[7] &= 0xffffffffu >> (256 - F::BITS);
    flags[j] = F::geq_mod(l) ? 0u : 1u;
}
__global__ void k_rand_compact(const uint32_t *__restrict__ words, uint32_t word_off, uint32_t ncand, const uint32_t *__restrict__ flags, const uint32_t *__restrict__ pos,
                               F *__restrict__ out, uint32_t count, uint32_t *__restrict__ last_cand) {
    uint32_t j = blockIdx.x * blockDim.x + threadIdx.x;
    if (j >= ncand || !flags[j]) return;
    uint32_t q = pos[j];
    if (q >= count) return;
    F v;
#pragma unroll
    for (int i = 0; i < 8; i++) v.l[i] = words[(size_t)word_off + 8 * (size_t)j + i];
    v.l[7] &= 0xffffffffu >> (256 - F::BITS);
    out[q] = v;
    if (q + 1 == count) *last_cand = j;
}
uint64_t chacha_field_stream(F *out, size_t count, const uint32_t key[8], int rounds, uint64_t word_pos, void *scratch, size_t scratch_bytes, stream_t s_) {
    hipStream_t s = (hipStream_t)s_;
    if (count == 0) return word_pos;
    const double accept = 0.58;
    uint64_t pos_words = word_pos;
    size_t done = 0;
    while (done < count) {
        size_t want = count - done;
        uint32_t ncand = (uint32_t)((double)want / accept * 1.02) + 4096;
        uint64_t first_block = pos_words / 16;
        uint32_t word_off = (uint32_t)(pos_words % 16);
        uint32_t nblocks = (uint32_t)(((uint64_t)word_off + 8ull * ncand + 15) / 16);
        size_t need = (size_t)nblocks * 64 + (size_t)ncand * 8 + 64 + (1 << 20);
        if (need > scratch_bytes) throw GpuError("chacha_field_stream: scratch too small");
        uint32_t *words = (uint32_t *)scratch, *flags = words + (size_t)nblocks * 16, *pos = flags + ncand, *last = pos + ncand;
        void *tmp = (void *)(last + 16);
        size_t tmp_bytes = scratch_bytes - ((char *)tmp - (char *)scratch);
        hipLaunchKernelGGL(k_chacha_blocks, GRID(nblocks), 0, s, words, first_block, nblocks, key[0], key[1], key[2], key[3], key[4], key[5], key[6], key[7], rounds); HIP_LAUNCH_CHECK();
        hipLaunchKernelGGL(k_rand_flags, GRID(ncand), 0, s, (const uint32_t *)words, word_off, ncand, flags); HIP_LAUNCH_CHECK();
        size_t tb = 0;
        HIP_CHECK(rocprim::exclusive_scan(nullptr, tb, flags, pos, 0u, (size_t)ncand, rocprim::plus<uint32_t>(), s));
        if (tb > tmp_bytes) throw GpuError("chacha_field_stream: scan scratch too small");
        HIP_CHECK(rocprim::exclusive_scan(tmp, tb, flags, pos, 0u, (size_t)ncand, rocprim::plus<uint32_t>(), s));
        HIP_CHECK(hipMemsetAsync(last, 0xff, 4, s));
        hipLaunchKernelGGL(k_rand_compact, GRID(ncand), 0, s, (const uint32_t *)words, word_off, ncand, (const uint32_t *)flags, (const uint32_t *)pos, out + done, (uint32_t)want, last); HIP_LAUNCH_CHECK();
        uint32_t h_last = 0, h_tail[2] = {0, 0};
        sync((stream_t)s);
        HIP_CHECK(hipMemcpyAsync(&h_last, last, 4, hipMemcpyDeviceToHost, s));
        HIP_CHECK(hipMemcpyAsync(&h_tail[0], pos + ncand - 1, 4, hipMemcpyDeviceToHost, s));
        HIP_CHECK(hipMemcpyAsync(&h_tail[1], flags + ncand - 1, 4, hipMemcpyDeviceToHost, s));
        sync((stream_t)s);
        if (h_last != 0xffffffffu) { pos_words += 8ull * ((uint64_t)h_last + 1); done = count; }
        else { done += (size_t)h_tail[0] + h_tail[1]; pos_words += 8ull * ncand; }
    }
    return pos_words;
}
__global__ void k_mask_fixup(F *p, size_t n) { if (blockIdx.x == 0 && threadIdx.x == 0) p[0] = p[0] - (p[0] + p[n] + p[2 * n]); }
void mask_fixup(F *p, size_t n, stream_t s) { hipLaunchKernelGGL(k_mask_fixup, dim3(1), dim3(64), 0, (hipStream_t)s, p, n); HIP_LAUNCH_CHECK(); }

__global__ void k_index_rowcol(F *__restrict__ row, F *__restrict__ col, F *__restrict__ rowcol, F *__restrict__ u, const uint32_t *__restrict__ ci, const uint32_t *__restrict__ ri,
                               size_t cnt, size_t k, const F *__restrict__ elems, uint32_t n, F n_fe) {
    size_t i = (size_t)blockIdx.x * blockDim.x + threadIdx.x;
    if (i >= k) return;
    if (i < cnt) {
        uint32_t c = ci[i], r = ri[i];
        F rv = elems[c], cv = elems[r];
        row[i] = rv; col[i] = cv; rowcol[i] = rv * cv;
        u[i] = elems[(n - c) & (n - 1)] * n_fe;
    } else {
        row[i] = elems[0]; col[i] = elems[0]; rowcol[i] = elems[0]; u[i] = F::zero();
    }
}
__global__ void k_index_vals(F *__restrict__ va, F *__restrict__ vb, F *__restrict__ vc, const F *__restrict__ uinv, const int64_t *__restrict__ ca, const int64_t *__restrict__ cb,
                             const int64_t *__restrict__ cc, size_t cnt, size_t k) {
    size_t i = (size_t)blockIdx.x * blockDim.x + threadIdx.x;
    if (i >= k) return;
    if (i < cnt) {
        F w = uinv[i];
        va[i] = ca[i] ? F::from_i64(ca[i]) * w : F::zero();
        vb[i] = cb[i] ? F::from_i64(cb[i]) * w : F::zero();
        vc[i] = cc[i] ? F::from_i64(cc[i]) * w : F::zero();
    } else { va[i] = F::zero(); vb[i] = F::zero(); vc[i] = F::zero(); }
}
void index_evals(F *row, F *col, F *rowcol, F *va, F *vb, F *vc, F *tmp, const uint32_t *ci, const uint32_t *ri, const int64_t *ca, const int64_t *cb, const int64_t *cc, size_t cnt,
                 size_t k, const F *elems, uint32_t n, stream_t s) {
    hipLaunchKernelGGL(k_index_rowcol, GRID(k), 0, (hipStream_t)s, row, col, rowcol, tmp, ci, ri, cnt, k, elems, n, F::from_u64(n)); HIP_LAUNCH_CHECK();
    batch_inverse(tmp, k, nullptr, s);
    hipLaunchKernelGGL(k_index_vals, GRID(k), 0, (hipStream_t)s, va, vb, vc, tmp, ca, cb, cc, cnt, k); HIP_LAUNCH_CHECK();
}

}
}
```

### aes_zero_knowledge_proof_circuit_amd/csrc/kernels_witness.hip

```cpp
#include <mutex>
#include "hip_util.hpp"
#include "trace_layout.h"

namespace zk {
namespace gpu {

#define GRID(n) dim3((unsigned)(((n) + 255) / 256)), dim3(256)

static uint8_t *g_sbox_dev[64] = {nullptr};
static std::mutex g_sbox_mu;
static uint8_t *sbox_here() {
    int d = 0;
    HIP_CHECK(hipGetDevice(&d));
    if (d < 0 || d >= 64) throw GpuError("device ordinal out of range");
    std::lock_guard<std::mutex> g(g_sbox_mu);
    return g_sbox_dev[d];
}
void upload_sbox(const uint8_t table[256]) {
    int d = 0;
    HIP_CHECK(hipGetDevice(&d));
    if (d < 0 || d >= 64) throw GpuError("device ordinal out of range");
    std::lock_guard<std::mutex> g(g_sbox_mu);
    if (!g_sbox_dev[d]) g_sbox_dev[d] = (uint8_t *)dmalloc(256);
    HIP_CHECK(hipMemcpy(g_sbox_dev[d], table, 256, hipMemcpyHostToDevice));
}

static int trace_nk(const char *who, size_t key_bytes) {
    if (key_bytes != 16 && key_bytes != 24 && key_bytes != 32) throw GpuError(std::string(who) + ": the AES key must have 16, 24 or 32 bytes");
    return (int)(key_bytes / 4);
}
static size_t trace_bytes_of(int nk, size_t b4, size_t b6, size_t b8) { return nk == 4 ? b4 : nk == 6 ? b6 : b8; }

__device__ __forceinline__ uint8_t xtime(uint8_t c) { return (uint8_t)((c << 1) ^ (((c >> 7) & 1) * 0x1B)); }

template <bool STORE, int NK = 4>
__device__ __forceinline__ void aes_block_rounds(uint8_t s[16], const uint8_t (*w)[4], const uint8_t *__restrict__ sbox, uint8_t *__restrict__ bl) {
    uint8_t u[16], v[16];
    for (int r = 1; r <= TRK_NR(NK); r++) {
        for (int i = 0; i < 16; i++) { v[i] = sbox[s[i]]; if (STORE) bl[TRK_BL_SB(NK) + 16 * (r - 1) + i] = v[i]; }
        for (int c = 0; c < 4; c++) for (int rr = 0; rr < 4; rr++) u[4 * c + rr] = v[4 * ((c + rr) & 3) + rr];
        if (r <= TRK_NR(NK) - 1) {
            for (int c = 0; c < 4; c++) {
                uint8_t a[4], xb[4];
                for (int k = 0; k < 4; k++) { a[k] = u[4 * c + k]; xb[k] = xtime(a[k]); if (STORE) bl[TRK_BL_XT(NK) + 16 * (r - 1) + 4 * c + k] = xb[k]; }
                const uint8_t term[4][5] = {{xb[0], a[3], a[2], xb[1], a[1]}, {xb[1], a[0], a[3], xb[2], a[2]}, {xb[2], a[1], a[0], xb[3], a[3]}, {xb[3], a[2], a[1], xb[0], a[0]}};
                for (int o = 0; o < 4; o++) {
                    uint8_t acc = term[o][0];
                    for (int q = 1; q < 5; q++) { acc ^= term[o][q]; if (STORE) bl[TRK_BL_MP(NK) + 64 * (r - 1) + 4 * (4 * c + o) + (q - 1)] = acc; }
                    v[4 * c + o] = acc;
                }
            }
        } else {
            for (int i = 0; i < 16; i++) v[i] = u[i];
        }
        for (int i = 0; i < 16; i++) { s[i] = v[i] ^ w[4 * r + i / 4][i % 4]; if (STORE) bl[TRK_BL_S(NK) + 16 * r + i] = s[i]; }
    }
}

template <int NK = 4>
__device__ __forceinline__ void aes_key_schedule(const uint8_t *__restrict__ key, const uint8_t *__restrict__ sbox, uint8_t (*w)[4], uint8_t *__restrict__ tr) {
    const uint8_t rc[10] = {0x01, 0x02, 0x04, 0x08, 0x10, 0x20, 0x40, 0x80, 0x1B, 0x36};
    for (int i = 0; i < NK; i++) for (int k = 0; k < 4; k++) w[i][k] = key[4 * i + k];
    for (int i = NK; i < TRK_KS_WORDS(NK); i++) {
        if (i % NK == 0) {
            int q = TRK_KS_INST_OF(NK, i);
            uint8_t sub[4], pre[4];
            for (int k = 0; k < 4; k++) sub[k] = sbox[w[i - 1][(k + 1) & 3]];
            for (int k = 0; k < 4; k++) { pre[k] = w[i - NK][k] ^ sub[k]; w[i][k] = pre[k]; }
            w[i][0] ^= rc[i / NK - 1];
            if (tr) for (int k = 0; k < 4; k++) { tr[TRK_KS_SUB(NK) + 4 * q + k] = sub[k]; tr[TRK_KS_PRE(NK) + 4 * q + k] = pre[k]; }
        } else if (NK == 8 && i % 8 == 4) {
            int q = TRK_KS_INST_OF(NK, i);
            uint8_t sub[4];
            for (int k = 0; k < 4; k++) sub[k] = sbox[w[i - 1][k]];
            for (int k = 0; k < 4; k++) w[i][k] = w[i - NK][k] ^ sub[k];
            if (tr) for (int k = 0; k < 4; k++) { tr[TRK_KS_SUB(NK) + 4 * q + k] = sub[k]; tr[TRK_KS_PRE(NK) + 4 * q + k] = w[i][k]; }
        } else {
            for (int k = 0; k < 4; k++) w[i][k] = w[i - NK][k] ^ w[i - 1][k];
        }
    }
}
template <int NK = 4>
__device__ __forceinline__ void aes_store_schedule(uint8_t *__restrict__ tr, const uint8_t *__restrict__ key, const uint8_t (*w)[4]) {
    for (int i = 0; i < TRK_KEY_BYTES(NK); i++) tr[TR_KEY + i] = key[i];
    for (int i = 0; i < TRK_KS_WORDS(NK); i++) for (int k = 0; k < 4; k++) tr[TRK_KS_W(NK) + 4 * i + k] = w[i][k];
}

template <bool CBC, int NK = 4>
__global__ void k_aes_trace(uint8_t *__restrict__ trace, size_t stride, const uint8_t *__restrict__ msgs, const uint8_t *__restrict__ keys, const uint8_t *__restrict__ ivs,
                            uint32_t nproofs, uint32_t nblocks, const uint8_t *__restrict__ sbox) {
    uint32_t t = blockIdx.x * blockDim.x + threadIdx.x;
    if (t >= nproofs * (nblocks + 1)) return;
    uint32_t p = t / (nblocks + 1), which = t % (nblocks + 1);
    uint8_t *tr = trace + (size_t)p * stride;
    const uint8_t *key = keys + TRK_KEY_BYTES(NK) * (size_t)p;
    uint8_t w[TRK_KS_WORDS(NK)][4];
    aes_key_schedule<NK>(key, sbox, w, which == 0 ? tr : nullptr);
    uint8_t *tail = tr + TRK_CBC(NK, (size_t)nblocks);
    if (which == 0) {
        aes_store_schedule<NK>(tr, key, w);
        if (CBC) for (int i = 0; i < 16; i++) tail[TR_CBC_IV + i] = ivs[16 * (size_t)p + i];
        return;
    }
    uint32_t b = which - 1;
    uint8_t *bl = tr + TRK_BLOCK0(NK) + (size_t)b * TRK_BLOCK_STRIDE(NK);
    const uint8_t *msg = msgs + ((size_t)p * nblocks + b) * 16;
    uint8_t s[16];
    if (CBC) {
        uint8_t prev[16];
        for (int i = 0; i < 16; i++) prev[i] = ivs[16 * (size_t)p + i];
        for (uint32_t j = 0; j < b; j++) {
            const uint8_t *mj = msgs + ((size_t)p * nblocks + j) * 16;
            for (int i = 0; i < 16; i++) s[i] = mj[i] ^ prev[i] ^ key[i];
            aes_block_rounds<false, NK>(s, w, sbox, nullptr);
            for (int i = 0; i < 16; i++) prev[i] = s[i];
        }
        for (int i = 0; i < 16; i++) {
            uint8_t x = msg[i] ^ prev[i];
            bl[TR_BL_MSG + i] = msg[i]; tail[TR_CBC_X + 16 * b + i] = x; s[i] = x ^ key[i]; bl[TR_BL_S + i] = s[i];
        }
    } else {
        for (int i = 0; i < 16; i++) { bl[TR_BL_MSG + i] = msg[i]; s[i] = msg[i] ^ key[i]; bl[TR_BL_S + i] = s[i]; }
    }
    aes_block_rounds<true, NK>(s, w, sbox, bl);
}

__device__ __forceinline__ void ctr_add(const uint8_t *__restrict__ in, uint32_t n, uint8_t out[16]) {
    uint32_t c = n;
    for (int i = 15; i >= 0; i--) { uint32_t t = in[i] + (c & 0xff); out[i] = (uint8_t)t; c = (c >> 8) + (t >> 8); }
}

template <int NK = 4>
__global__ void k_aes_trace_ctr(uint8_t *__restrict__ trace, size_t stride, const uint8_t *__restrict__ msgs, const uint8_t *__restrict__ keys, const uint8_t *__restrict__ icbs,
                                uint32_t nproofs, uint32_t nblocks, uint32_t msg_len, const uint8_t *__restrict__ sbox) {
    uint32_t t = blockIdx.x * blockDim.x + threadIdx.x;
    if (t >= nproofs * (nblocks + 1)) return;
    uint32_t p = t / (nblocks + 1), which = t % (nblocks + 1);
    uint8_t *tr = trace + (size_t)p * stride;
    const uint8_t *key = keys + TRK_KEY_BYTES(NK) * (size_t)p, *icb = icbs + 16 * (size_t)p;
    uint8_t w[TRK_KS_WORDS(NK)][4];
    aes_key_schedule<NK>(key, sbox, w, which == 0 ? tr : nullptr);
    uint8_t *tail = tr + TRK_CTR(NK, (size_t)nblocks);
    if (which == 0) {
        aes_store_schedule<NK>(tr, key, w);
        for (int i = 0; i < 16; i++) tail[TR_CTR_ICB + i] = icb[i];
        return;
    }
    uint32_t b = which - 1;
    uint8_t *bl = tr + TRK_BLOCK0(NK) + (size_t)b * TRK_BLOCK_STRIDE(NK), *slot = tail + TR_CTR_BLOCK0 + (size_t)b * TR_CTR_BLOCK_STRIDE;
    uint8_t ctr[16], carry[16], s[16], m[16];
    ctr_add(icb, b, ctr);
    for (int i = 0; i < 16; i++) carry[i] = 0;
    if (b) {
        uint8_t prev[16];
        ctr_add(icb, b - 1, prev);
        for (int i = 0; i < 128 && ((prev[15 - i / 8] >> (i % 8)) & 1); i++) carry[15 - i / 8] |= (uint8_t)(1u << (i % 8));
    }
    uint32_t have = msg_len - 16 * b < 16 ? msg_len - 16 * b : 16;
    const uint8_t *msg = msgs + (size_t)p * msg_len + 16 * (size_t)b;
    for (uint32_t i = 0; i < 16; i++) m[i] = i < have ? msg[i] : 0;
    for (int i = 0; i < 16; i++) { slot[TR_CTR_BL_CTR + i] = ctr[i]; slot[TR_CTR_BL_CARRY + i] = carry[i]; bl[TR_BL_MSG + i] = m[i]; s[i] = ctr[i] ^ key[i]; bl[TR_BL_S + i] = s[i]; }
    aes_block_rounds<true, NK>(s, w, sbox, bl);
    for (uint32_t i = 0; i < 16; i++) slot[TR_CTR_BL_CT + i] = i < have ? (uint8_t)(m[i] ^ s[i]) : 0;
}

template <int NK = 4>
__global__ void k_aes_trace_gcm(uint8_t *__restrict__ trace, size_t stride, const uint8_t *__restrict__ msgs, const uint8_t *__restrict__ keys, const uint8_t *__restrict__ hdrs,
                                uint32_t nproofs, uint32_t nblocks, uint32_t naad, uint32_t msg_len, uint32_t aad_len, const uint8_t *__restrict__ sbox) {
    uint32_t t = blockIdx.x * blockDim.x + threadIdx.x;
    if (t >= nproofs * (nblocks + 3)) return;
    uint32_t p = t / (nblocks + 3), which = t % (nblocks + 3);
    uint8_t *tr = trace + (size_t)p * stride;
    const uint8_t *key = keys + TRK_KEY_BYTES(NK) * (size_t)p, *hdr = hdrs + (size_t)p * (12 + (size_t)aad_len);
    uint8_t w[TRK_KS_WORDS(NK)][4];
    aes_key_schedule<NK>(key, sbox, w, which == 0 ? tr : nullptr);
    uint8_t *tail = tr + TRK_GCM(NK, (size_t)nblocks);
    if (which == 0) {
        aes_store_schedule<NK>(tr, key, w);
        for (int i = 0; i < 16; i++) tail[TR_GCM_IV + i] = i < 12 ? hdr[i] : 0;
        for (uint32_t i = 0; i < 16 * naad; i++) tail[TR_GCM_AAD + i] = i < aad_len ? hdr[12 + i] : 0;
        return;
    }
    uint32_t slot = which - 1;
    uint8_t *bl = tr + TRK_BLOCK0(NK) + (size_t)slot * TRK_BLOCK_STRIDE(NK);
    uint8_t in[16], s[16], m[16];
    uint32_t ctr = slot < nblocks ? slot + 2 : 1, have = 0;
    for (int i = 0; i < 16; i++) in[i] = slot == nblocks ? 0 : (i < 12 ? hdr[i] : (uint8_t)(ctr >> (8 * (15 - i))));
    if (slot < nblocks) have = msg_len - 16 * slot < 16 ? msg_len - 16 * slot : 16;
    const uint8_t *msg = msgs + (size_t)p * msg_len + 16 * (size_t)(slot < nblocks ? slot : 0);
    for (uint32_t i = 0; i < 16; i++) m[i] = i < have ? msg[i] : 0;
    for (int i = 0; i < 16; i++) { bl[TR_BL_MSG + i] = m[i]; s[i] = in[i] ^ key[i]; bl[TR_BL_S + i] = s[i]; }
    aes_block_rounds<true, NK>(s, w, sbox, bl);
    if (slot < nblocks) for (uint32_t i = 0; i < 16; i++) tail[TR_GCM_CT(naad) + 16 * slot + i] = i < have ? (uint8_t)(m[i] ^ s[i]) : 0;
}

struct Gf128 { uint64_t hi, lo; };
struct alignas(16) Bytes16 { uint8_t b[16]; };
__device__ __forceinline__ Gf128 gf_load(const uint8_t *__restrict__ b) { Gf128 r = {0, 0}; for (int i = 0; i < 8; i++) { r.hi = (r.hi << 8) | b[i]; r.lo = (r.lo << 8) | b[8 + i]; } return r; }
__device__ __forceinline__ uint8_t gf_byte(const Gf128 &v, uint32_t j) { return (uint8_t)(j < 8 ? v.hi >> (56 - 8 * j) : v.lo >> (56 - 8 * (j - 8))); }
__device__ __forceinline__ uint32_t gf_bit(const Gf128 &v, int k) { return (uint32_t)(k < 64 ? v.hi >> (63 - k) : v.lo >> (127 - k)) & 1u; }
__device__ __forceinline__ void gf_times_alpha(Gf128 &v) {
    uint64_t lsb = v.lo & 1;
    v.lo = (v.lo >> 1) | (v.hi << 63); v.hi >>= 1;
    if (lsb) v.hi ^= 0xE100000000000000ull;
}
__device__ __forceinline__ Gf128 gf_mul(const Gf128 &x, Gf128 v) {
    Gf128 z = {0, 0};
    for (int i = 0; i < 128; i++) { if (gf_bit(x, i)) { z.hi ^= v.hi; z.lo ^= v.lo; } gf_times_alpha(v); }
    return z;
}

template <int NK = 4>
__global__ void k_ghash_trace(uint8_t *__restrict__ trace, size_t stride, uint32_t nproofs, uint32_t nblocks, uint32_t naad, uint32_t msg_len, uint32_t aad_len) {
    uint32_t t = blockIdx.x * blockDim.x + threadIdx.x;
    const uint32_t n_mul = naad + nblocks + 1, per_proof = (n_mul + 1) * 16;
    if (t >= nproofs * per_proof) return;
    uint32_t p = t / per_proof, m = (t % per_proof) / 16, j = t % 16;
    uint8_t *tr = trace + (size_t)p * stride, *tail = tr + TRK_GCM(NK, (size_t)nblocks);
    const Gf128 h = gf_load(tr + TRK_BLOCK0(NK) + (size_t)nblocks * TRK_BLOCK_STRIDE(NK) + TRK_BL_CT(NK));
    Gf128 v = h;
    if (m == n_mul) {
        uint8_t *col = tail + TR_GCM_V(naad, nblocks) + 128 * j;
        for (int c = 0; c < 8; c++) {
            Bytes16 o;
            for (int u = 0; u < 16; u++) { o.b[u] = gf_byte(v, j); gf_times_alpha(v); }
            *reinterpret_cast<Bytes16 *>(col + 16 * c) = o;
        }
        return;
    }
    Gf128 x = {0, 0};
    for (uint32_t mm = 0;; mm++) {
        Gf128 blk;
        if (mm < naad + nblocks) blk = gf_load(tail + TR_GCM_AAD + 16 * (size_t)mm);
        else { blk.hi = 8 * (uint64_t)aad_len; blk.lo = 8 * (uint64_t)msg_len; }
        x.hi ^= blk.hi; x.lo ^= blk.lo;
        if (mm == m) break;
        x = gf_mul(x, h);
    }
    uint8_t *mul = tail + TR_GCM_MUL0(naad, nblocks) + (size_t)m * TR_GCM_MUL_STRIDE;
    mul[TR_GCM_MUL_X + j] = gf_byte(x, j);
    uint32_t cnt[8] = {0, 0, 0, 0, 0, 0, 0, 0};
    for (int c = 0; c < 8; c++) {
        Bytes16 o;
        for (int u = 0; u < 16; u++) {
            uint8_t pb = gf_bit(x, 16 * c + u) ? gf_byte(v, j) : 0;
            o.b[u] = pb;
            for (int bit = 0; bit < 8; bit++) cnt[bit] += (pb >> bit) & 1u;
            gf_times_alpha(v);
        }
        *reinterpret_cast<Bytes16 *>(mul + TR_GCM_MUL_P + 128 * j + 16 * c) = o;
    }
    uint8_t y = 0;
    for (int bit = 0; bit < 8; bit++) {
        mul[TR_GCM_MUL_Q + 8 * j + 7 - bit] = (uint8_t)(cnt[bit] >> 1);
        y |= (uint8_t)((cnt[bit] & 1u) << bit);
    }
    mul[TR_GCM_MUL_Y + j] = y;
    if (m + 1 == n_mul) tail[TR_GCM_TAG(naad, nblocks) + j] = y ^ tr[TRK_BLOCK0(NK) + (size_t)(nblocks + 1) * TRK_BLOCK_STRIDE(NK) + TRK_BL_CT(NK) + j];
}

template <int NK = 4>
__global__ void k_key_tag_trace(uint8_t *__restrict__ trace, size_t stride, size_t tag_off, const uint8_t *__restrict__ keys, uint32_t nproofs, uint32_t ntags, const uint8_t *__restrict__ sbox) {
    uint32_t t = blockIdx.x * blockDim.x + threadIdx.x;
    if (t >= nproofs * ntags) return;
    uint32_t p = t / ntags, which = t % ntags;
    const uint8_t *key = keys + TRK_KEY_BYTES(NK) * (size_t)p;
    uint8_t w[TRK_KS_WORDS(NK)][4];
    aes_key_schedule<NK>(key, sbox, w, nullptr);
    uint8_t *bl = trace + (size_t)p * stride + tag_off + (size_t)which * TRK_BLOCK_STRIDE(NK);
    const char prefix[] = TRK_KT_D_PREFIX;
    uint8_t s[16];
    for (int i = 0; i < 16; i++) {
        uint8_t d = i < 11 ? (uint8_t)prefix[i] : i == 11 ? (uint8_t)which : 0;
        bl[TR_BL_MSG + i] = d; s[i] = d ^ key[i]; bl[TR_BL_S + i] = s[i];
    }
    aes_block_rounds<true, NK>(s, w, sbox, bl);
}
template <bool CBC>
static void launch_aes_trace(const char *who, uint8_t *trace, size_t stride, const uint8_t *msgs, const uint8_t *keys, const uint8_t *ivs, uint32_t nproofs, uint32_t nblocks, size_t key_bytes, stream_t s) {
    const int nk = trace_nk(who, key_bytes);
    const size_t need = CBC ? trace_bytes_of(nk, TRK_CBC_BYTES(4, (size_t)nblocks), TRK_CBC_BYTES(6, (size_t)nblocks), TRK_CBC_BYTES(8, (size_t)nblocks))
                            : trace_bytes_of(nk, TRK_ECB_BYTES(4, (size_t)nblocks), TRK_ECB_BYTES(6, (size_t)nblocks), TRK_ECB_BYTES(8, (size_t)nblocks));
    if (stride < need) throw GpuError(std::string(who) + ": trace stride " + std::to_string(stride) + " is short of the " + std::to_string(need) + " bytes a " + std::to_string(8 * key_bytes) + "-bit key's trace takes");
    uint8_t *g_sbox = sbox_here();
    if (!g_sbox) throw GpuError(std::string(who) + ": S-box table not uploaded on this device");
    uint32_t lanes = nproofs * (nblocks + 1);
    const dim3 grid((lanes + 63) / 64), block(64);
    if (nk == 4) hipLaunchKernelGGL((k_aes_trace<CBC, 4>), grid, block, 0, (hipStream_t)s, trace, stride, msgs, keys, ivs, nproofs, nblocks, g_sbox);
    else if (nk == 6) hipLaunchKernelGGL((k_aes_trace<CBC, 6>), grid, block, 0, (hipStream_t)s, trace, stride, msgs, keys, ivs, nproofs, nblocks, g_sbox);
    else hipLaunchKernelGGL((k_aes_trace<CBC, 8>), grid, block, 0, (hipStream_t)s, trace, stride, msgs, keys, ivs, nproofs, nblocks, g_sbox);
    HIP_LAUNCH_CHECK();
}
void aes_trace(uint8_t *trace, size_t stride, const uint8_t *msgs, const uint8_t *keys, uint32_t nproofs, uint32_t nblocks, stream_t s, size_t key_bytes) {
    launch_aes_trace<false>("aes_trace", trace, stride, msgs, keys, nullptr, nproofs, nblocks, key_bytes, s);
}
void aes_trace_cbc(uint8_t *trace, size_t stride, const uint8_t *msgs, const uint8_t *keys, const uint8_t *ivs, uint32_t nproofs, uint32_t nblocks, stream_t s, size_t key_bytes) {
    if (!ivs) throw GpuError("aes_trace_cbc: no IV buffer");
    launch_aes_trace<true>("aes_trace_cbc", trace, stride, msgs, keys, ivs, nproofs, nblocks, key_bytes, s);
}
void aes_trace_ctr(uint8_t *trace, size_t stride, const uint8_t *msgs, const uint8_t *keys, const uint8_t *icbs, uint32_t nproofs, uint32_t msg_len, stream_t s, size_t key_bytes) {
    if (!icbs) throw GpuError("aes_trace_ctr: no counter buffer");
    if (msg_len == 0 || msg_len > 0xfffffff0u) throw GpuError("aes_trace_ctr: the message length must be 1 .. 2^32 - 16 bytes");
    const int nk = trace_nk("aes_trace_ctr", key_bytes);
    uint32_t nblocks = (msg_len + 15) / 16;
    if (stride < trace_bytes_of(nk, TRK_CTR_BYTES(4, (size_t)nblocks), TRK_CTR_BYTES(6, (size_t)nblocks), TRK_CTR_BYTES(8, (size_t)nblocks))) throw GpuError("aes_trace_ctr: trace stride is short of the CTR tail");
    uint8_t *g_sbox = sbox_here();
    if (!g_sbox) throw GpuError("aes_trace_ctr: S-box table not uploaded on this device");
    uint32_t lanes = nproofs * (nblocks + 1);
    const dim3 grid((lanes + 63) / 64), block(64);
    if (nk == 4) hipLaunchKernelGGL(k_aes_trace_ctr<4>, grid, block, 0, (hipStream_t)s, trace, stride, msgs, keys, icbs, nproofs, nblocks, msg_len, g_sbox);
    else if (nk == 6) hipLaunchKernelGGL(k_aes_trace_ctr<6>, grid, block, 0, (hipStream_t)s, trace, stride, msgs, keys, icbs, nproofs, nblocks, msg_len, g_sbox);
    else hipLaunchKernelGGL(k_aes_trace_ctr<8>, grid, block, 0, (hipStream_t)s, trace, stride, msgs, keys, icbs, nproofs, nblocks, msg_len, g_sbox);
    HIP_LAUNCH_CHECK();
}
static int gcm_shape(const char *who, const uint8_t *trace, size_t stride, uint32_t nproofs, uint32_t msg_len, uint32_t aad_len, size_t key_bytes, uint32_t &nblocks, uint32_t &naad) {
    const int nk = trace_nk(who, key_bytes);
    if (msg_len == 0 || msg_len > (1u << 16) || aad_len > (1u << 16)) throw GpuError(std::string(who) + ": the message must have 1 .. 65536 bytes, the aad at most 65536");
    nblocks = (msg_len + 15) / 16; naad = (aad_len + 15) / 16;
    const size_t na = naad, nb = nblocks;
    if (stride < trace_bytes_of(nk, TRK_GCM_BYTES(4, na, nb), TRK_GCM_BYTES(6, na, nb), TRK_GCM_BYTES(8, na, nb))) throw GpuError(std::string(who) + ": trace stride is short of the GCM tail");
    if (stride % 16 || (uintptr_t)trace % 16) throw GpuError(std::string(who) + ": traces must be 16-byte aligned");
    if (nproofs == 0 || nproofs > (1u << 20)) throw GpuError(std::string(who) + ": 1 .. 2^20 proofs per launch");
    return nk;
}
void aes_trace_gcm(uint8_t *trace, size_t stride, const uint8_t *msgs, const uint8_t *keys, const uint8_t *hdrs, uint32_t nproofs, uint32_t msg_len, uint32_t aad_len, stream_t s, size_t key_bytes) {
    if (!hdrs) throw GpuError("aes_trace_gcm: no iv / aad buffer");
    uint32_t nblocks, naad;
    const int nk = gcm_shape("aes_trace_gcm", trace, stride, nproofs, msg_len, aad_len, key_bytes, nblocks, naad);
    uint8_t *g_sbox = sbox_here();
    if (!g_sbox) throw GpuError("aes_trace_gcm: S-box table not uploaded on this device");
    uint32_t lanes = nproofs * (nblocks + 3);
    const dim3 grid((lanes + 63) / 64), block(64);
    if (nk == 4) hipLaunchKernelGGL(k_aes_trace_gcm<4>, grid, block, 0, (hipStream_t)s, trace, stride, msgs, keys, hdrs, nproofs, nblocks, naad, msg_len, aad_len, g_sbox);
    else if (nk == 6) hipLaunchKernelGGL(k_aes_trace_gcm<6>, grid, block, 0, (hipStream_t)s, trace, stride, msgs, keys, hdrs, nproofs, nblocks, naad, msg_len, aad_len, g_sbox);
    else hipLaunchKernelGGL(k_aes_trace_gcm<8>, grid, block, 0, (hipStream_t)s, trace, stride, msgs, keys, hdrs, nproofs, nblocks, naad, msg_len, aad_len, g_sbox);
    HIP_LAUNCH_CHECK();
}
void ghash_trace(uint8_t *trace, size_t stride, uint32_t nproofs, uint32_t msg_len, uint32_t aad_len, stream_t s, size_t key_bytes) {
    uint32_t nblocks, naad;
    const int nk = gcm_shape("ghash_trace", trace, stride, nproofs, msg_len, aad_len, key_bytes, nblocks, naad);
    uint32_t lanes = nproofs * (naad + nblocks + 2) * 16;
    const dim3 grid((lanes + 63) / 64), block(64);
    if (nk == 4) hipLaunchKernelGGL(k_ghash_trace<4>, grid, block, 0, (hipStream_t)s, trace, stride, nproofs, nblocks, naad, msg_len, aad_len);
    else if (nk == 6) hipLaunchKernelGGL(k_ghash_trace<6>, grid, block, 0, (hipStream_t)s, trace, stride, nproofs, nblocks, naad, msg_len, aad_len);
    else hipLaunchKernelGGL(k_ghash_trace<8>, grid, block, 0, (hipStream_t)s, trace, stride, nproofs, nblocks, naad, msg_len, aad_len);
    HIP_LAUNCH_CHECK();
}
void key_tag_trace(uint8_t *trace, size_t stride, size_t tag_off, const uint8_t *keys, uint32_t nproofs, uint32_t tag_blocks, stream_t s, size_t key_bytes) {
    const int nk = trace_nk("key_tag_trace", key_bytes);
    if (!trace || !keys) throw GpuError("key_tag_trace: no trace or key buffer");
    if (tag_blocks != 1 && tag_blocks != 2) throw GpuError("key_tag_trace: 1 or 2 tag blocks");
    const size_t slot = trace_bytes_of(nk, TRK_BLOCK_STRIDE(4), TRK_BLOCK_STRIDE(6), TRK_BLOCK_STRIDE(8));
    if (tag_off < trace_bytes_of(nk, TRK_BLOCK0(4), TRK_BLOCK0(6), TRK_BLOCK0(8)) || tag_off > stride || stride - tag_off < tag_blocks * slot)
        throw GpuError("key_tag_trace: trace stride " + std::to_string(stride) + " does not hold " + std::to_string(tag_blocks) + " tag slots of " + std::to_string(slot) + " bytes at offset " + std::to_string(tag_off));
    if (tag_off % 16 || stride % 16 || (uintptr_t)trace % 16) throw GpuError("key_tag_trace: tagged traces and the tag offset must be 16-byte aligned");
    if (nproofs == 0 || nproofs > (1u << 20)) throw GpuError("key_tag_trace: 1 .. 2^20 proofs per launch");
    uint8_t *g_sbox = sbox_here();
    if (!g_sbox) throw GpuError("key_tag_trace: S-box table not uploaded on this device");
    uint32_t lanes = nproofs * tag_blocks;
    const dim3 grid((lanes + 63) / 64), block(64);
    if (nk == 4) hipLaunchKernelGGL(k_key_tag_trace<4>, grid, block, 0, (hipStream_t)s, trace, stride, tag_off, keys, nproofs, tag_blocks, g_sbox);
    else if (nk == 6) hipLaunchKernelGGL(k_key_tag_trace<6>, grid, block, 0, (hipStream_t)s, trace, stride, tag_off, keys, nproofs, tag_blocks, g_sbox);
    else hipLaunchKernelGGL(k_key_tag_trace<8>, grid, block, 0, (hipStream_t)s, trace, stride, tag_off, keys, nproofs, tag_blocks, g_sbox);
    HIP_LAUNCH_CHECK();
}

__global__ void k_witness_expand(uint8_t *__restrict__ z, const uint32_t *__restrict__ desc, uint32_t ncols, const uint8_t *__restrict__ trace,
                                 const uint32_t *__restrict__ sbox_in_off, const uint32_t *__restrict__ sbox_tmpl, const uint8_t *__restrict__ sbox) {
    uint32_t i = blockIdx.x * blockDim.x + threadIdx.x;
    if (i >= ncols) return;
    uint32_t d = desc[i], kind = d >> WD_KIND_SHIFT, bit;
    if (kind == WD_BYTEBIT) {
        uint32_t off = (d >> 4) & 0x3ffffff, b = (d >> 1) & 7;
        bit = ((trace[off] >> b) & 1) ^ (d & 1);
    } else if (kind == WD_SBOX) {
        uint32_t inst = (d >> 11) & 0x7ffff, te = sbox_tmpl[(d >> 1) & 0x3ff];
        uint32_t lvl = (te >> 12) & 7, node = (te >> 4) & 0xff, b = (te >> 1) & 7;
        uint32_t x = trace[sbox_in_off[inst]];
        uint32_t idx = (node << (lvl + 1)) | (x & ((2u << lvl) - 1));
        bit = ((sbox[idx] >> b) & 1) ^ (d & 1);
    } else {
        bit = d & 1;
    }
    z[i] = (uint8_t)bit;
}
void witness_expand(uint8_t *z, const uint32_t *desc, uint32_t ncols, const uint8_t *trace, const uint32_t *sbox_in_off, const uint32_t *sbox_tmpl, stream_t s) {
    uint8_t *g_sbox = sbox_here();
    if (!g_sbox) throw GpuError("witness_expand: S-box table not uploaded on this device");
    hipLaunchKernelGGL(k_witness_expand, GRID(ncols), 0, (hipStream_t)s, z, desc, ncols, trace, sbox_in_off, sbox_tmpl, g_sbox);
    HIP_LAUNCH_CHECK();
}

__device__ __forceinline__ F small_to_field(long long v) { return F::from_i64(v); }

__global__ void k_spmv_bits(F *__restrict__ out, int8_t *__restrict__ small_out, size_t rows_out, const uint32_t *__restrict__ rowptr, const uint32_t *__restrict__ col, const int64_t *__restrict__ coeff,
                            size_t rows, const uint8_t *__restrict__ z) {
    size_t r = (size_t)blockIdx.x * blockDim.x + threadIdx.x;
    if (r >= rows_out) return;
    long long acc = 0;
    if (r < rows) for (uint32_t i = rowptr[r]; i < rowptr[r + 1]; i++) acc += z[col[i]] ? coeff[i] : 0;
    out[r] = acc == 0 ? F::zero() : small_to_field(acc);
    if (small_out) small_out[r] = (int8_t)(acc > 127 ? 127 : (acc < -127 ? -127 : acc));
}
void spmv_bits(F *out, int8_t *small_out, size_t rows_out, const uint32_t *rowptr, const uint32_t *col, const int64_t *coeff, size_t rows, const uint8_t *z, stream_t s) {
    hipLaunchKernelGGL(k_spmv_bits, GRID(rows_out), 0, (hipStream_t)s, out, small_out, rows_out, rowptr, col, coeff, rows, z); HIP_LAUNCH_CHECK();
}
__global__ void k_w_classes(int8_t *__restrict__ out, const uint8_t *__restrict__ z, uint32_t n, uint32_t m, uint32_t num_witness) {
    uint32_t k = blockIdx.x * blockDim.x + threadIdx.x;
    if (k >= n) return;
    uint32_t ratio = n / m;
    if (k % ratio == 0) { out[k] = 0; return; }
    uint32_t wi = k - k / ratio - 1;
    out[k] = (wi < num_witness && z[m + wi]) ? 1 : 0;
}
void w_classes(int8_t *out, const uint8_t *z, uint32_t n, uint32_t m, uint32_t num_witness, stream_t s) {
    hipLaunchKernelGGL(k_w_classes, GRID(n), 0, (hipStream_t)s, out, z, n, m, num_witness); HIP_LAUNCH_CHECK();
}
__global__ void k_lagrange_finish(F *__restrict__ lag, F *__restrict__ lag_w, const F *__restrict__ elems, uint32_t n, uint32_t m, F vx_inv, F n_inv) {
    uint32_t k = blockIdx.x * blockDim.x + threadIdx.x;
    if (k >= n) return;
    F v = lag[k] * (elems[k] * n_inv);
    lag[k] = v;
    lag_w[k] = (k % (n / m) == 0) ? F::zero() : v * vx_inv;
}
void lagrange_scalars(F *lag, F *lag_w, const F *elems, const F &beta, uint32_t n, uint32_t m, stream_t s) {
    int lg_n = 0;
    while ((1u << lg_n) < n) lg_n++;
    F vx_inv = (beta.pow_u64(m) - F::one()).inverse();
    const size_t need = vanishing_quotient_scratch(lg_n, 1);
    DevPtr<F> scratch(need);
    F *outs[1] = {lag};
    const F one = F::one();
    vanishing_quotient_evals(outs, &one, 1, beta, elems, n, lg_n, scratch, need, s);
    hipLaunchKernelGGL(k_lagrange_finish, GRID(n), 0, (hipStream_t)s, lag, lag_w, elems, n, m, vx_inv, F::from_u64(n).inverse()); HIP_LAUNCH_CHECK();
    sync(s);
}

__global__ void k_w_evals(F *__restrict__ out, const uint8_t *__restrict__ z, const F *__restrict__ x_evals, uint32_t n, uint32_t m, uint32_t num_witness) {
    uint32_t k = blockIdx.x * blockDim.x + threadIdx.x;
    if (k >= n) return;
    uint32_t ratio = n / m;
    if (k % ratio == 0) { out[k] = F::zero(); return; }
    uint32_t wi = k - k / ratio - 1;
    F w = (wi < num_witness && z[m + wi]) ? F::one() : F::zero();
    out[k] = w - x_evals[k];
}
void w_evals(F *out, const uint8_t *z, const F *x_evals, uint32_t n, uint32_t m, uint32_t num_witness, stream_t s) {
    hipLaunchKernelGGL(k_w_evals, GRID(n), 0, (hipStream_t)s, out, z, x_evals, n, m, num_witness); HIP_LAUNCH_CHECK();
}
__global__ void k_bits_to_field(F *__restrict__ out, const uint8_t *__restrict__ z, size_t n) { size_t i = (size_t)blockIdx.x * blockDim.x + threadIdx.x; if (i < n) out[i] = z[i] ? F::one() : F::zero(); }
void bits_to_field(F *out, const uint8_t *z, size_t n, stream_t s) { if (!n) return; hipLaunchKernelGGL(k_bits_to_field, GRID(n), 0, (hipStream_t)s, out, z, n); HIP_LAUNCH_CHECK(); }

__global__ void k_t_partials(F *__restrict__ partial, uint32_t nseg, const uint32_t *__restrict__ seg_start, const uint32_t *__restrict__ seg_end, const uint32_t *__restrict__ row,
                             const uint8_t *__restrict__ mat, const int64_t *__restrict__ coeff, const F *__restrict__ r_alpha, F eta_a, F eta_b, F eta_c) {
    uint32_t sgi = blockIdx.x * blockDim.x + threadIdx.x;
    if (sgi >= nseg) return;
    F acc = F::zero();
    for (uint32_t i = seg_start[sgi]; i < seg_end[sgi]; i++) {
        F eta = mat[i] == 0 ? eta_a : (mat[i] == 1 ? eta_b : eta_c);
        long long c = coeff[i];
        F term = eta * r_alpha[row[i]];
        if (c == 1) acc = acc + term;
        else if (c == -1) acc = acc - term;
        else acc = acc + term * small_to_field(c);
    }
    partial[sgi] = acc;
}
__global__ void k_t_columns(F *__restrict__ out, uint32_t n, const uint32_t *__restrict__ col_seg_ptr, const F *__restrict__ partial) {
    uint32_t h = blockIdx.x * blockDim.x + threadIdx.x;
    if (h >= n) return;
    uint32_t a = col_seg_ptr[h], b = col_seg_ptr[h + 1];
    if (b - a > T_HEAVY_SEGMENTS) return;
    F acc = F::zero();
    for (uint32_t i = a; i < b; i++) acc = acc + partial[i];
    out[h] = acc;
}
__global__ void __launch_bounds__(256) k_t_heavy(F *__restrict__ out, const uint32_t *__restrict__ heavy, const uint32_t *__restrict__ col_seg_ptr, const F *__restrict__ partial) {
    __shared__ F sh[256];
    uint32_t h = heavy[blockIdx.x], t = threadIdx.x;
    F acc = F::zero();
    for (uint32_t i = col_seg_ptr[h] + t; i < col_seg_ptr[h + 1]; i += 256) acc = acc + partial[i];
    sh[t] = acc;
    __syncthreads();
    for (int s = 128; s > 0; s >>= 1) { if ((int)t < s) sh[t] = sh[t] + sh[t + s]; __syncthreads(); }
    if (t == 0) out[h] = sh[0];
}
void t_evals(F *out, uint32_t n, F *partial, uint32_t nseg, const uint32_t *col_seg_ptr, const uint32_t *seg_start, const uint32_t *seg_end, const uint32_t *heavy, uint32_t n_heavy,
             const uint32_t *row, const uint8_t *mat, const int64_t *coeff, const F *r_alpha, const F &eta_a, const F &eta_b, const F &eta_c, stream_t s) {
    if (nseg) { hipLaunchKernelGGL(k_t_partials, GRID(nseg), 0, (hipStream_t)s, partial, nseg, seg_start, seg_end, row, mat, coeff, r_alpha, eta_a, eta_b, eta_c); HIP_LAUNCH_CHECK(); }
    hipLaunchKernelGGL(k_t_columns, GRID(n), 0, (hipStream_t)s, out, n, col_seg_ptr, partial); HIP_LAUNCH_CHECK();
    if (n_heavy) { hipLaunchKernelGGL(k_t_heavy, dim3(n_heavy), dim3(256), 0, (hipStream_t)s, out, heavy, col_seg_ptr, partial); HIP_LAUNCH_CHECK(); }
}

}
}
```

### include/zkaes.h

```cpp
#ifndef ZKAES_H
#define ZKAES_H
#include <stddef.h>
#include <stdint.h>
#ifdef __cplusplus
extern "C" {
#endif

typedef struct zkaes_pk zkaes_pk;
typedef struct zkaes_vk zkaes_vk;

const char *zkaes_last_error(void);
void zkaes_bytes_free(uint8_t *p);
void zkaes_pk_free(zkaes_pk *pk);
void zkaes_vk_free(zkaes_vk *vk);
int zkaes_device_count(void);
int zkaes_set_device(int ordinal);

int zkaes_synthesize_keys(size_t plaintext_length, zkaes_pk **pk, zkaes_vk **vk);
int zkaes_encrypt(const uint8_t *message, size_t message_len, const uint8_t secret_key[16], const zkaes_pk *pk, uint8_t **proof, size_t *proof_len);
int zkaes_verify_encryption(const zkaes_vk *vk, const uint8_t *proof, size_t proof_len, const uint8_t *ciphertext, size_t ciphertext_len, int *accepted);
int zkaes_proof_roundtrip(const uint8_t *proof, size_t proof_len, uint8_t **out, size_t *out_len);

#define ZKAES_CIRCUIT_AES 0
#define ZKAES_CIRCUIT_OPS_XOR 1
#define ZKAES_CIRCUIT_OPS_ADD 2
#define ZKAES_CIRCUIT_AES_CTR 4
#define ZKAES_CIRCUIT_AES_GCM 5
#define ZKAES_CIRCUIT_AES_CBC 3
int zkaes_synthesize_keys_ex(int circuit_kind, size_t plaintext_length, size_t srs_num_constraints, size_t srs_num_variables, size_t srs_num_non_zero, zkaes_pk **pk,
                             zkaes_vk **vk);
#define ZKAES_KEY_NO_TABLES 1u
int zkaes_synthesize_keys_ex2(int circuit_kind, size_t plaintext_length, size_t srs_num_constraints, size_t srs_num_variables, size_t srs_num_non_zero, unsigned flags,
                              zkaes_pk **pk, zkaes_vk **vk);
int zkaes_encrypt_seeded(const uint8_t *message, size_t message_len, const uint8_t secret_key[16], const zkaes_pk *pk, const uint8_t *zk_seed32, uint8_t **proof,
                         size_t *proof_len);
int zkaes_encrypt_chunked(const uint8_t *message, size_t message_len, const uint8_t secret_key[16], const zkaes_pk *pk, uint8_t **proofs, size_t *proofs_len,
                          size_t *proof_lens, size_t n_chunks);
#define ZKAES_DEFAULT_CONTEXTS 12
int zkaes_encrypt_batch(size_t n, const uint8_t *messages, const uint8_t *secret_keys, const zkaes_pk *pk, uint8_t **proofs, size_t *proofs_len, size_t *proof_lens);
int zkaes_pk_set_contexts(zkaes_pk *pk, size_t n);
int zkaes_pk_get_contexts(const zkaes_pk *pk, size_t *n);
int zkaes_encrypt_chunked_seeded(const uint8_t *message, size_t message_len, const uint8_t secret_key[16], const zkaes_pk *pk, const uint8_t *zk_seed32, uint8_t **proofs,
                                 size_t *proofs_len, size_t *proof_lens, size_t n_chunks);
int zkaes_encrypt_chunked_seeded_at(const uint8_t *message, size_t message_len, const uint8_t secret_key[16], const zkaes_pk *pk, const uint8_t *zk_seed32,
                                    uint64_t first_proof_index, uint8_t **proofs, size_t *proofs_len, size_t *proof_lens, size_t n_chunks);
int zkaes_encrypt_batch_seeded(size_t n, const uint8_t *messages, size_t messages_len, const uint8_t *secret_keys, size_t secret_keys_len, const zkaes_pk *pk,
                               const uint8_t *zk_seed32, uint8_t **proofs, size_t *proofs_len, size_t *proof_lens);
int zkaes_encrypt_batch_seeded_at(size_t n, const uint8_t *messages, size_t messages_len, const uint8_t *secret_keys, size_t secret_keys_len, const zkaes_pk *pk,
                                  const uint8_t *zk_seed32, uint64_t first_proof_index, uint8_t **proofs, size_t *proofs_len, size_t *proof_lens);
int zkaes_cbc_ciphertext(const uint8_t *message, size_t message_len, const uint8_t secret_key[16], const uint8_t iv[16], uint8_t *ciphertext);
int zkaes_encrypt_cbc_seeded(const uint8_t *message, size_t message_len, const uint8_t secret_key[16], const uint8_t iv[16], const zkaes_pk *pk, const uint8_t *zk_seed32,
                             uint8_t *ciphertext_or_null, uint8_t **proof, size_t *proof_len);
int zkaes_encrypt_cbc_chunked(const uint8_t *message, size_t message_len, const uint8_t secret_key[16], const uint8_t iv[16], const zkaes_pk *pk, uint8_t *ciphertext_or_null,
                              uint8_t **proofs, size_t *proofs_len, size_t *proof_lens, size_t n_chunks);
int zkaes_encrypt_cbc_chunked_seeded_at(const uint8_t *message, size_t message_len, const uint8_t secret_key[16], const uint8_t iv[16], const zkaes_pk *pk, const uint8_t *zk_seed32,
                                        uint64_t first_proof_index, uint8_t *ciphertext_or_null, uint8_t **proofs, size_t *proofs_len, size_t *proof_lens, size_t n_chunks);
int zkaes_aes_witness_cbc(const zkaes_pk *pk, const uint8_t *message, size_t message_len, const uint8_t secret_key[16], const uint8_t iv[16], uint8_t *z, size_t z_cap, size_t *z_len);
int zkaes_verify_encryption_cbc(const zkaes_vk *vk, const uint8_t *proof, size_t proof_len, const uint8_t iv[16], const uint8_t *ciphertext, size_t ciphertext_len, int *accepted);
int zkaes_verify_cbc_chunked(const zkaes_vk *vk, const uint8_t *proofs, const size_t *proof_lens, size_t n_chunks, const uint8_t iv[16], const uint8_t *ciphertext,
                             size_t ciphertext_len, int *accepted_each, size_t *n_accepted);
int zkaes_ctr_crypt(const uint8_t *in, size_t len, const uint8_t secret_key[16], const uint8_t icb[16], uint8_t *out);
int zkaes_ctr_counter_add(const uint8_t icb[16], uint64_t n_blocks, uint8_t out16[16]);
int zkaes_encrypt_ctr_seeded(const uint8_t *message, size_t message_len, const uint8_t secret_key[16], const uint8_t icb[16], const zkaes_pk *pk, const uint8_t *zk_seed32,
                             uint8_t *ciphertext_or_null, uint8_t **proof, size_t *proof_len);
int zkaes_encrypt_ctr_chunked(const uint8_t *message, size_t message_len, const uint8_t secret_key[16], const uint8_t icb[16], const zkaes_pk *pk, uint8_t *ciphertext_or_null,
                              uint8_t **proofs, size_t *proofs_len, size_t *proof_lens, size_t n_chunks);
int zkaes_encrypt_ctr_chunked_seeded_at(const uint8_t *message, size_t message_len, const uint8_t secret_key[16], const uint8_t icb[16], const zkaes_pk *pk, const uint8_t *zk_seed32,
                                        uint64_t first_proof_index, uint8_t *ciphertext_or_null, uint8_t **proofs, size_t *proofs_len, size_t *proof_lens, size_t n_chunks);
int zkaes_aes_witness_ctr(const zkaes_pk *pk, const uint8_t *message, size_t message_len, const uint8_t secret_key[16], const uint8_t icb[16], uint8_t *z, size_t z_cap, size_t *z_len);
int zkaes_verify_encryption_ctr(const zkaes_vk *vk, const uint8_t *proof, size_t proof_len, const uint8_t icb[16], const uint8_t *ciphertext, size_t ciphertext_len, int *accepted);
int zkaes_verify_ctr_chunked(const zkaes_vk *vk, const uint8_t *proofs, const size_t *proof_lens, size_t n_chunks, const uint8_t icb[16], const uint8_t *ciphertext,
                             size_t ciphertext_len, int *accepted_each, size_t *n_accepted);
int zkaes_synthesize_keys_gcm(size_t plaintext_length, size_t aad_length, size_t srs_num_constraints, size_t srs_num_variables, size_t srs_num_non_zero, unsigned flags,
                              zkaes_pk **pk, zkaes_vk **vk);
int zkaes_gcm_encrypt(const uint8_t *message, size_t message_len, const uint8_t secret_key[16], const uint8_t iv12[12], const uint8_t *aad, size_t aad_len,
                      uint8_t *ciphertext, uint8_t tag16[16]);
int zkaes_gcm_decrypt(const uint8_t *ciphertext, size_t ciphertext_len, const uint8_t secret_key[16], const uint8_t iv12[12], const uint8_t *aad, size_t aad_len,
                      const uint8_t tag16[16], uint8_t *message, int *ok);
int zkaes_encrypt_gcm_seeded(const uint8_t *message, size_t message_len, const uint8_t secret_key[16], const uint8_t iv12[12], const uint8_t *aad, size_t aad_len,
                             const zkaes_pk *pk, const uint8_t *zk_seed32, uint8_t *ciphertext_or_null, uint8_t *tag_or_null, uint8_t **proof, size_t *proof_len);
int zkaes_encrypt_gcm_batch_seeded_at(size_t n, const uint8_t *messages, size_t messages_len, const uint8_t *secret_keys, size_t secret_keys_len, const uint8_t *headers,
                                      size_t headers_len, const zkaes_pk *pk, const uint8_t *zk_seed32, uint64_t first_proof_index, uint8_t *ciphertexts_or_null,
                                      uint8_t *tags_or_null, uint8_t **proofs, size_t *proofs_len, size_t *proof_lens);
int zkaes_aes_witness_gcm(const zkaes_pk *pk, const uint8_t *message, size_t message_len, const uint8_t secret_key[16], const uint8_t iv12[12], const uint8_t *aad, size_t aad_len,
                          uint8_t *z, size_t z_cap, size_t *z_len);
int zkaes_verify_encryption_gcm(const zkaes_vk *vk, const uint8_t *proof, size_t proof_len, const uint8_t iv12[12], const uint8_t *aad, size_t aad_len,
                                const uint8_t *ciphertext, size_t ciphertext_len, const uint8_t tag16[16], int *accepted);
int zkaes_circuit_info_gcm(size_t plaintext_length, size_t aad_length, uint64_t out[12]);
int zkaes_circuit_matrix_gcm(size_t plaintext_length, size_t aad_length, int which, uint64_t *n_rows, uint64_t *nnz, uint32_t *rowptr, uint32_t *col, int64_t *coeff);
int zkaes_synthesize_keys_ks(int circuit_kind, unsigned key_bits, size_t plaintext_length, size_t aad_length, size_t srs_num_constraints, size_t srs_num_variables,
                             size_t srs_num_non_zero, unsigned flags, zkaes_pk **pk, zkaes_vk **vk);
int zkaes_pk_key_bytes(const zkaes_pk *pk, size_t *n);
int zkaes_circuit_info_ks(int circuit_kind, unsigned key_bits, size_t plaintext_length, size_t aad_length, uint64_t out[12]);
int zkaes_circuit_matrix_ks(int circuit_kind, unsigned key_bits, size_t plaintext_length, size_t aad_length, int which, uint64_t *n_rows, uint64_t *nnz, uint32_t *rowptr,
                            uint32_t *col, int64_t *coeff);
int zkaes_ecb_ciphertext_ks(const uint8_t *message, size_t message_len, const uint8_t *secret_key, size_t key_len, uint8_t *ciphertext);
int zkaes_cbc_ciphertext_ks(const uint8_t *message, size_t message_len, const uint8_t *secret_key, size_t key_len, const uint8_t iv[16], uint8_t *ciphertext);
int zkaes_ctr_crypt_ks(const uint8_t *in, size_t len, const uint8_t *secret_key, size_t key_len, const uint8_t icb[16], uint8_t *out);
int zkaes_gcm_encrypt_ks(const uint8_t *message, size_t message_len, const uint8_t *secret_key, size_t key_len, const uint8_t iv12[12], const uint8_t *aad, size_t aad_len,
                         uint8_t *ciphertext, uint8_t tag16[16]);
int zkaes_gcm_decrypt_ks(const uint8_t *ciphertext, size_t ciphertext_len, const uint8_t *secret_key, size_t key_len, const uint8_t iv12[12], const uint8_t *aad, size_t aad_len,
                         const uint8_t tag16[16], uint8_t *message, int *ok);
int zkaes_synthesize_keys_kt(int circuit_kind, unsigned key_bits, unsigned key_tag_blocks, size_t plaintext_length, size_t aad_length, size_t srs_num_constraints,
                             size_t srs_num_variables, size_t srs_num_non_zero, unsigned flags, zkaes_pk **pk, zkaes_vk **vk);
int zkaes_pk_key_tag_blocks(const zkaes_pk *pk, size_t *n);
int zkaes_key_tag(const uint8_t *secret_key, size_t key_len, size_t tag_blocks, uint8_t *out);
int zkaes_circuit_info_kt(int circuit_kind, unsigned key_bits, unsigned key_tag_blocks, size_t plaintext_length, size_t aad_length, uint64_t out[12]);
int zkaes_circuit_matrix_kt(int circuit_kind, unsigned key_bits, unsigned key_tag_blocks, size_t plaintext_length, size_t aad_length, int which, uint64_t *n_rows, uint64_t *nnz,
                            uint32_t *rowptr, uint32_t *col, int64_t *coeff);
int zkaes_verify_chunked_kt(const zkaes_vk *vk, int circuit_kind, const uint8_t *proofs, const size_t *proof_lens, size_t n_chunks, const uint8_t *iv_or_icb, const uint8_t *ciphertext,
                            size_t ciphertext_len, const uint8_t *key_tag, size_t key_tag_len, int *accepted_each, size_t *n_accepted);
int zkaes_verify_encryption_gcm_kt(const zkaes_vk *vk, const uint8_t *proof, size_t proof_len, const uint8_t iv12[12], const uint8_t *aad, size_t aad_len, const uint8_t *ciphertext,
                                   size_t ciphertext_len, const uint8_t tag16[16], const uint8_t *key_tag, size_t key_tag_len, int *accepted);
int zkaes_prove_ops(const zkaes_pk *pk, uint32_t x, uint32_t y, const uint8_t *zk_seed32, uint8_t **proof, size_t *proof_len);
int zkaes_verify(const zkaes_vk *vk, const uint8_t *proof, size_t proof_len, const uint8_t *public_input_bits, size_t n_bits, int *accepted);
int zkaes_vk_serialize(const zkaes_vk *vk, uint8_t **out, size_t *out_len);
int zkaes_vk_deserialize(const uint8_t *bytes, size_t len, zkaes_vk **vk);
int zkaes_vk_serialize_ark(const zkaes_vk *vk, uint8_t **out, size_t *out_len);
int zkaes_vk_deserialize_ark(const uint8_t *bytes, size_t len, zkaes_vk **vk);
int zkaes_vk_serialize_ark_uncompressed(const zkaes_vk *vk, uint8_t **out, size_t *out_len);

int zkaes_vk_from_trapdoor(const uint64_t info[7], const uint8_t *index_comms, const uint8_t *beta, zkaes_vk **vk);

int zkaes_pk_info(const zkaes_pk *pk, uint64_t out[12]);
int zkaes_circuit_info(int circuit_kind, size_t plaintext_length, uint64_t out[12]);
int zkaes_circuit_matrix(int circuit_kind, size_t plaintext_length, int which, uint64_t *n_rows, uint64_t *nnz, uint32_t *rowptr, uint32_t *col, int64_t *coeff);
int zkaes_pk_debug_fetch(const zkaes_pk *pk, const char *name, uint8_t **out, size_t *len);
int zkaes_pk_timings(const zkaes_pk *pk, double out[6]);
int zkaes_msm_stats(double out[5], int reset);
int zkaes_pk_op_lists(const zkaes_pk *pk, const uint8_t *message, size_t message_len, const uint8_t secret_key[16], int throughput_path, uint8_t **json, size_t *json_len);
int zkaes_mem_info(uint64_t *free_bytes, uint64_t *total_bytes);

int zkaes_ntt(int field_id, uint8_t *data, size_t n, int inverse);
int zkaes_ntt_coset(int field_id, uint8_t *data, size_t n, int inverse, int coset_c, int lg_big);
int zkaes_ntt_batch(int field_id, uint8_t *data, size_t n, int count, int inverse, const int *coset_c, int lg_big);
int zkaes_poly_divide_by_vanishing(const uint8_t *p, size_t len, size_t m, int with_scratch, uint8_t *q, uint8_t *rem_or_null);
int zkaes_poly_divide_by_linear(const uint8_t *p, size_t len, const uint8_t z[32], uint8_t *q);
int zkaes_poly_eval_multi(const uint8_t *const *polys, const size_t *lens, const uint8_t *x, int count, uint8_t *out);
int zkaes_batch_inverse(uint8_t *v, size_t n, const uint8_t *post_or_null, int throughput_variant);
int zkaes_poly_lincomb(const uint8_t *const *polys, const size_t *lens, const uint8_t *scalars, int count, size_t n, uint8_t *out);
int zkaes_vanishing_quotient_evals(int lg_n, const uint8_t *g, int ncosets, const uint8_t a[32], const uint32_t *idx_or_null, size_t nidx, uint8_t *out);
int zkaes_q1_coset_pointwise(const uint8_t *r, const uint8_t *za, const uint8_t *zb, const uint8_t *t, const uint8_t *z, const uint8_t consts[192], size_t n, uint8_t *out);
int zkaes_h2_coset(const uint8_t *const arrays[7], const uint8_t consts[224], size_t k, uint8_t *out);
int zkaes_q1_combine(const uint8_t *q0, const uint8_t *q1, const uint8_t *q3, const uint8_t *mask, const uint8_t inv2[32], const uint8_t inv2zeta[32], size_t n, uint8_t *h1, uint8_t *g1);
int zkaes_coset_scale(const uint8_t *in, size_t in_len, const uint8_t g[32], size_t n, uint8_t *out);
int zkaes_z_poly_from_w(const uint8_t *w, size_t wlen, const uint8_t *x_poly, uint32_t m, size_t n, uint8_t *zp);
int zkaes_ntt_padded(int field_id, const uint8_t *in, size_t in_len, size_t n, int inverse, int coset_c, int lg_big, uint8_t *out);
int zkaes_ntt_scaled(const uint8_t g[32], const uint8_t *in, size_t in_len, size_t n, int inverse, uint8_t *out);
int zkaes_class_sum(const uint8_t *bases, size_t n, const int8_t *vals, int count, int edwards, size_t prior_msm_points, int *ok_out, uint8_t *out_xy, int *out_inf);
int zkaes_msm_pair(const uint8_t *bases, size_t nbases, const uint8_t *scal1, size_t n1, const uint8_t *scal2, size_t n2, size_t val_off2, int edwards, uint8_t *out_xy, int *out_inf);
int zkaes_msm_table_pair(const uint8_t *bases, size_t stride, const uint8_t *scal1, size_t n1, size_t off1, const uint8_t *scal2, size_t n2, size_t off2, int window_bits, int edwards,
                         uint8_t *out_xy, int *out_inf);
int zkaes_msm_second_bases(const uint8_t *bases, size_t nbases, const uint8_t *scalars, size_t n, size_t off, size_t shift, int window_bits, uint8_t *out_xy, int *out_inf);
int zkaes_arith_probe(int op, const uint32_t *in, size_t n_cases, uint32_t *out);

int zkaes_msm(int curve_id, const uint8_t *bases, const uint8_t *scalars, size_t n, uint8_t *out_xy, int *out_inf);
int zkaes_g1_sum(int curve_id, const uint8_t *points_xy, const int *inf, size_t n, uint8_t *out_xy, int *out_inf);
int zkaes_msm_sharded_plan(int curve_id, size_t n_total, int *window_bits, int *n_windows, size_t *bytes_per_rank);
int zkaes_msm_window_sums_dev(int curve_id, const uint8_t *bases, const uint8_t *scalars, size_t n_local, size_t n_total, void *dev_out, size_t dev_out_bytes);
int zkaes_msm_fold_window_sums_dev(int curve_id, const void *dev_in, int world, size_t n_total, uint8_t *out_xy, int *out_inf);
int zkaes_pk_msm_partial_dev(const zkaes_pk *pk, const uint8_t *scalars, size_t n_local, size_t offset, void *dev_out, size_t dev_out_bytes);
int zkaes_msm_fold_partials_dev(int curve_id, const void *dev_in, int world, uint8_t *out_xy, int *out_inf);
int zkaes_pk_serialize_ark_to_file(const zkaes_pk *pk, const char *path, uint64_t *bytes_written);
int zkaes_pk_serialize_ark_to_file_ex(const zkaes_pk *pk, const char *path, int uncompressed, uint64_t *bytes_written);
int zkaes_pk_tables_built(const zkaes_pk *pk, int *built, uint64_t *table_bytes);
int zkaes_pk_srs_info(const zkaes_pk *pk, uint64_t out[6], double secs[2]);
int zkaes_set_default_contexts(size_t n);
int zkaes_srs_hold(int hold);
int zkaes_msm_table(int curve_id, const uint8_t *bases, const uint8_t *scalars, size_t n, int window_bits, uint8_t *out_xy, int *out_inf);
int zkaes_msm_table_srs(const uint8_t *bases, const uint8_t *scalars, size_t n, int window_bits, uint8_t *out_xy, int *out_inf);
int zkaes_msm_bench(int curve_id, const uint8_t *bases, const uint8_t *scalars, size_t n, int reps, double *ms_total, double *ms_accumulate);
int zkaes_msm_bench_synth(size_t n, int window_bits, int reps, double *ms_total, double *ms_accumulate, uint8_t *out_xy);
int zkaes_stream_copy_bench(size_t bytes, int reps, double *gb_per_s);
int zkaes_int_rate_bench(double seconds, double out[8]);
int zkaes_aes_witness(const zkaes_pk *pk, const uint8_t *message, size_t message_len, const uint8_t secret_key[16], uint8_t *z, size_t z_cap, size_t *z_len);

#ifdef __cplusplus
}
#endif
#endif
```

Measured before the change: 97.96.

## Port polynomial kernels to 29-bit-limb field arithmetic with lazy reduction

Moves the poly_scale, divide-by-linear, Horner evaluation, vanishing-quotient, q1_combine and t_evals kernels from the 32-bit-limb Montgomery type to the Fp29 split representation, keeping lazy, partially reduced values between operations. t_evals now accumulates per-matrix sums and multiplies by eta once per segment instead of once per entry. New C API entry points for poly_scale and t_evals are added so these paths can be tested. The change relies on hand-derived value bounds that are enforced with static_asserts, which adds correctness risk.

```diff
diff --git a/aes_zero_knowledge_proof_circuit_amd/api.py b/aes_zero_knowledge_proof_circuit_amd/api.py
--- a/aes_zero_knowledge_proof_circuit_amd/api.py
+++ b/aes_zero_knowledge_proof_circuit_amd/api.py
@@ -695,6 +695,21 @@
     h1, g1 = C.create_string_buffer(64 * n or 1), C.create_string_buffer(32 * max(n - 1, 0) or 1)
     _check(lib().zkaes_q1_combine(bytes(q0), bytes(q1), bytes(q3), bytes(mask), bytes(inv2), bytes(inv2zeta), C.c_size_t(n), h1, g1))
     return h1.raw[:64 * n], g1.raw[:32 * max(n - 1, 0)]
+
+
+def poly_scale(p, sc):
+    n = len(p) // 32
+    buf = C.create_string_buffer(bytes(p), max(len(p), 1))
+    _check(lib().zkaes_poly_scale(buf, C.c_size_t(n), bytes(sc)))
+    return buf.raw[:32 * n]
+
+
+def t_evals(colptr, row, mat, coeff, r_alpha, eta_a, eta_b, eta_c):
+    n, total = len(colptr) - 1, len(row)
+    out = C.create_string_buffer(32 * n or 1)
+    _check(lib().zkaes_t_evals(C.c_uint32(n), (C.c_uint32 * (n + 1))(*colptr), (C.c_uint32 * max(total, 1))(*row), bytes(bytearray(mat)) or b"\0",
+                               (C.c_int64 * max(total, 1))(*coeff), bytes(r_alpha), C.c_uint32(len(r_alpha) // 32), b"".join(bytes(x) for x in (eta_a, eta_b, eta_c)), out))
+    return out.raw[:32 * n]
 
 
 def coset_scale(data, g, n):
diff --git a/aes_zero_knowledge_proof_circuit_amd/build.py b/aes_zero_knowledge_proof_circuit_amd/build.py
--- a/aes_zero_knowledge_proof_circuit_amd/build.py
+++ b/aes_zero_knowledge_proof_circuit_amd/build.py
@@ -11,7 +11,7 @@
 HIP_SOURCES = ["runtime.hip", "kernels_ntt.hip", "kernels_msm.hip", "kernels_poly.hip", "kernels_witness.hip", "capi_kernels.hip", "capi_probe.hip"]
 CXX_SOURCES = ["circuit.cpp", "marlin.cpp", "marlin_codec.cpp", "capi.cpp", "capi_host.cpp"]
 HOST_ONLY_SOURCES = ["circuit.cpp", "marlin_codec.cpp", "capi_host.cpp"]
-HEADERS = ["ff.cuh", "ff28.cuh", "ff29.cuh", "ec.cuh", "ec28.cuh", "te28.cuh", "gpu.hpp", "hip_util.hpp", "consts32.h", "trace_layout.h", "circuit.hpp", "marlin.hpp", "marlin_host.hpp", "capi_common.hpp", "pairing.hpp", "transcript.hpp", "arith_probe.cuh",
+HEADERS = ["ff.cuh", "ff28.cuh", "ff29.cuh", "poly29.cuh", "ec.cuh", "ec28.cuh", "te28.cuh", "gpu.hpp", "hip_util.hpp", "consts32.h", "trace_layout.h", "circuit.hpp", "marlin.hpp", "marlin_host.hpp", "capi_common.hpp", "pairing.hpp", "transcript.hpp", "arith_probe.cuh",
            os.path.join("..", "..", "include", "zkaes.h")]
 COMMON = ["-O3", "-std=c++17", "-fPIC", "-I", CSRC, "-Wno-unused-result"]
 if os.environ.get("ZK_EXTRA_DEFINES"):
diff --git a/aes_zero_knowledge_proof_circuit_amd/csrc/capi_kernels.hip b/aes_zero_knowledge_proof_circuit_amd/csrc/capi_kernels.hip
--- a/aes_zero_knowledge_proof_circuit_amd/csrc/capi_kernels.hip
+++ b/aes_zero_knowledge_proof_circuit_amd/csrc/capi_kernels.hip
@@ -563,6 +563,48 @@
         zk::gpu::q1_combine(dh, dg, d0, d1, d3, dm, i2, i2z, n, s);
         zk::gpu::d2h(h1, dh, 2 * n * sizeof(PF), s);
         zk::gpu::d2h(g1, dg, (n - 1) * sizeof(PF), s);
+    });
+}
+int zkaes_poly_scale(uint8_t *p, size_t n, const uint8_t sc[32]) {
+    return guardk([&] {
+        const char *who = "zkaes_poly_scale";
+        need(p || !n, who, "null argument"); need(n <= POLY_MAX, who, "polynomial too long");
+        const PF scf = load_f(sc, who);
+        if (!n) return;
+        zk::gpu::require_device();
+        StreamGuard s;
+        DevPtr<PF> dp = upload(p, n, s);
+        zk::gpu::poly_scale(dp, scf, n, s);
+        zk::gpu::d2h(p, dp, n * sizeof(PF), s);
+    });
+}
+int zkaes_t_evals(uint32_t n, const uint32_t *colptr, const uint32_t *row, const uint8_t *mat, const int64_t *coeff, const uint8_t *r_alpha, uint32_t n_rows, const uint8_t etas[96], uint8_t *out) {
+    return guardk([&] {
+        const char *who = "zkaes_t_evals";
+        need(colptr && r_alpha && etas && out, who, "null argument"); need(n >= 1 && n <= POLY_MAX && n_rows >= 1 && n_rows <= POLY_MAX, who, "n out of range");
+        need(colptr[0] == 0, who, "colptr must start at 0");
+        for (uint32_t h = 0; h < n; h++) need(colptr[h] <= colptr[h + 1], who, "colptr must not decrease");
+        const uint32_t total = colptr[n];
+        need(total <= POLY_MAX, who, "too many entries"); need(!total || (row && mat && coeff), who, "null argument");
+        for (uint32_t i = 0; i < total; i++) { need(row[i] < n_rows, who, "row out of range"); need(mat[i] <= 2, who, "mat must be 0, 1 or 2"); }
+        PF eta[3];
+        for (int i = 0; i < 3; i++) eta[i] = load_f(etas + 32 * i, who);
+        std::vector<uint32_t> col_seg_ptr(n + 1, 0), seg_start, seg_end, heavy;
+        for (uint32_t h = 0; h < n; h++) {
+            for (uint32_t st = colptr[h]; st < colptr[h + 1]; st += zk::gpu::T_SEG) { seg_start.push_back(st); seg_end.push_back(std::min(st + zk::gpu::T_SEG, colptr[h + 1])); }
+            col_seg_ptr[h + 1] = (uint32_t)seg_start.size();
+            if (col_seg_ptr[h + 1] - col_seg_ptr[h] > zk::gpu::T_HEAVY_SEGMENTS) heavy.push_back(h);
+        }
+        const uint32_t nseg = (uint32_t)seg_start.size(), n_heavy = (uint32_t)heavy.size();
+        zk::gpu::require_device();
+        StreamGuard s;
+        auto up = [&](const void *src, size_t bytes) { DevPtr<uint8_t> d(bytes ? bytes : 1); zk::gpu::h2d(d, src, bytes, s); return d; };
+        DevPtr<uint8_t> d_csp = up(col_seg_ptr.data(), 4 * (size_t)(n + 1)), d_ss = up(seg_start.data(), 4 * (size_t)nseg), d_se = up(seg_end.data(), 4 * (size_t)nseg),
+                        d_heavy = up(heavy.data(), 4 * (size_t)n_heavy), d_row = up(row, 4 * (size_t)total), d_mat = up(mat, total), d_coeff = up(coeff, 8 * (size_t)total);
+        DevPtr<PF> d_ra = upload(r_alpha, n_rows, s), d_partial(nseg ? nseg : 1), d_out(n);
+        zk::gpu::t_evals(d_out, n, d_partial, nseg, (const uint32_t *)d_csp.get(), (const uint32_t *)d_ss.get(), (const uint32_t *)d_se.get(), (const uint32_t *)d_heavy.get(), n_heavy,
+                         (const uint32_t *)d_row.get(), (const uint8_t *)d_mat.get(), (const int64_t *)d_coeff.get(), d_ra, eta[0], eta[1], eta[2], s);
+        zk::gpu::d2h(out, d_out, (size_t)n * sizeof(PF), s);
     });
 }
 int zkaes_coset_scale(const uint8_t *in, size_t in_len, const uint8_t g[32], size_t n, uint8_t *out) {
diff --git a/aes_zero_knowledge_proof_circuit_amd/csrc/kernels_poly.hip b/aes_zero_knowledge_proof_circuit_amd/csrc/kernels_poly.hip
--- a/aes_zero_knowledge_proof_circuit_amd/csrc/kernels_poly.hip
+++ b/aes_zero_knowledge_proof_circuit_amd/csrc/kernels_poly.hip
@@ -1,6 +1,6 @@
 #include <cstring>
 #include <rocprim/device/device_scan.hpp>
-#include "ff29.cuh"
+#include "poly29.cuh"
 #include "hip_util.hpp"
 
 namespace zk {
@@ -12,11 +12,12 @@
 void poly_set_at(F *p, size_t idx, const F &val, stream_t s) { hipLaunchKernelGGL(k_set_at, dim3(1), dim3(64), 0, (hipStream_t)s, p, idx, val, false); HIP_LAUNCH_CHECK(); }
 void poly_add_at(F *p, size_t idx, const F &val, stream_t s) { hipLaunchKernelGGL(k_set_at, dim3(1), dim3(64), 0, (hipStream_t)s, p, idx, val, true); HIP_LAUNCH_CHECK(); }
 
-__global__ void k_scale(F *p, F sc, size_t n) { size_t i = (size_t)blockIdx.x * blockDim.x + threadIdx.x; if (i < n) p[i] = p[i] * sc; }
-void poly_scale(F *p, const F &sc, size_t n, stream_t s) { if (!n) return; hipLaunchKernelGGL(k_scale, GRID(n), 0, (hipStream_t)s, p, sc, n); HIP_LAUNCH_CHECK(); }
 using G29 = Fp29<Fr377P>;
 __device__ __forceinline__ G29 ld29(const F &x) { return G29::split(x.l); }
 __device__ __forceinline__ F st29(const G29 &g) { F r; g.template canonical<1>().pack(r.l); return r; }
+using PL = Poly29<Fr377P>;
+__global__ void k_scale(F *p, G29 sc, size_t n) { size_t i = (size_t)blockIdx.x * blockDim.x + threadIdx.x; if (i < n) p[i] = st29(ld29(p[i]) * sc); }
+void poly_scale(F *p, const F &sc, size_t n, stream_t s) { if (!n) return; hipLaunchKernelGGL(k_scale, GRID(n), 0, (hipStream_t)s, p, G29::twiddle_from_std(sc), n); HIP_LAUNCH_CHECK(); }
 struct LincombArgs { const F *p[8]; size_t len[8]; G29 sc[8]; int count; };
 __global__ void k_lincomb_n(F *__restrict__ out, LincombArgs a, size_t n) {
     size_t i = (size_t)blockIdx.x * blockDim.x + threadIdx.x;
@@ -87,56 +88,45 @@
 }
 
 constexpr int DL_B = 16;
-__global__ void k_divlin_local(F *__restrict__ q, const F *__restrict__ p, size_t len, F z, F *__restrict__ v, F *__restrict__ zp) {
-    if (blockIdx.x == 0 && threadIdx.x < DL_B) zp[threadIdx.x] = z.pow_u64(threadIdx.x);
+__global__ void k_divlin_local(F *__restrict__ q, const F *__restrict__ p, size_t len, G29 z, F *__restrict__ v, F *__restrict__ zp) {
+    if (blockIdx.x == 0 && threadIdx.x < DL_B) zp[threadIdx.x] = PL::st_tw(PL::pow_tw(z, threadIdx.x));
     const size_t t = (size_t)blockIdx.x * blockDim.x + threadIdx.x, s0 = t * DL_B;
     if (s0 >= len) return;
     const size_t e = s0 + DL_B < len ? s0 + DL_B : len;
-    F l = F::zero();
-    for (size_t i = e; i-- > s0;) {
-        if (i + 1 < len) q[i] = l;
-        l = p[i] + z * l;
-    }
-    v[t] = l;
+    v[t] = st29(PL::divlin_block(q, p, s0, e, len, z));
 }
 constexpr int DL_TOP_THREADS = 256;
 constexpr size_t DL_TOP = (size_t)DL_TOP_THREADS * DL_B;
-__global__ void __launch_bounds__(DL_TOP_THREADS) k_divlin_top(F *__restrict__ q, const F *__restrict__ p, size_t len, F z) {
-    __shared__ F sh[DL_TOP_THREADS];
+__global__ void __launch_bounds__(DL_TOP_THREADS) k_divlin_top(F *__restrict__ q, const F *__restrict__ p, size_t len, G29 z) {
+    static_assert(DL_TOP_THREADS <= 256, "the scan's value bound (< 12 p) is written for at most eight doubling steps");
+    __shared__ G29 sh[DL_TOP_THREADS];
     const uint32_t t = threadIdx.x;
     const size_t s0 = (size_t)t * DL_B, e = s0 + DL_B < len ? s0 + DL_B : len;
-    F l = F::zero();
-    if (s0 < len) {
-        for (size_t i = e; i-- > s0;) {
-            if (i + 1 < len) q[i] = l;
-            l = p[i] + z * l;
-        }
-    }
-    sh[t] = l;
-    __syncthreads();
-    F y = z.pow_u64(DL_B);
+    sh[t] = s0 < len ? PL::divlin_block(q, p, s0, e, len, z) : G29::zero();
+    __syncthreads();
+    G29 y = PL::pow_tw(z, DL_B);
     for (int k = 1; k < DL_TOP_THREADS; k <<= 1) {
-        const F other = t + k < DL_TOP_THREADS ? sh[t + k] : F::zero();
+        const G29 other = t + k < DL_TOP_THREADS ? sh[t + k] : G29::zero();
         __syncthreads();
         sh[t] = sh[t] + y * other;
         __syncthreads();
-        y = y.sqr();
+        y = y * y;
     }
     if (s0 >= len || e >= len) return;
-    const F c = sh[t + 1];
-    F w = F::one();
-    for (size_t i = e; i-- > s0;) { q[i] = q[i] + w * c; w = w * z; }
+    const G29 c = sh[t + 1];
+    G29 w = PL::one_tw();
+    for (size_t i = e; i-- > s0;) { q[i] = PL::divlin_apply(q[i], w, c); w = w * z; }
 }
 __global__ void __launch_bounds__(256) k_divlin_apply(F *__restrict__ q, size_t qlen, const F *__restrict__ zp_table, const F *__restrict__ carry, size_t nblocks) {
-    __shared__ F zp[DL_B];
-    if (threadIdx.x < DL_B) zp[threadIdx.x] = zp_table[threadIdx.x];
+    __shared__ G29 zp[DL_B];
+    if (threadIdx.x < DL_B) zp[threadIdx.x] = ld29(zp_table[threadIdx.x]);
     __syncthreads();
     const size_t i = (size_t)blockIdx.x * blockDim.x + threadIdx.x;
     if (i >= qlen) return;
     const size_t t = i / DL_B;
     if (t + 1 >= nblocks) return;
     const size_t e = (t + 1) * DL_B;
-    q[i] = q[i] + zp[e - 1 - i] * carry[t];
+    q[i] = PL::divlin_apply(q[i], zp[e - 1 - i], ld29(carry[t]));
 }
 size_t divide_by_linear_scratch(size_t len) {
     size_t total = 8;
@@ -145,10 +135,10 @@
 }
 static void divlin_rec(F *q, const F *p, size_t len, const F &z, F *scratch, hipStream_t s) {
     if (len < 2) return;
-    if (len <= DL_TOP) { hipLaunchKernelGGL(k_divlin_top, dim3(1), dim3(DL_TOP_THREADS), 0, s, q, p, len, z); HIP_LAUNCH_CHECK(); return; }
+    if (len <= DL_TOP) { hipLaunchKernelGGL(k_divlin_top, dim3(1), dim3(DL_TOP_THREADS), 0, s, q, p, len, G29::twiddle_from_std(z)); HIP_LAUNCH_CHECK(); return; }
     const size_t nblocks = (len + DL_B - 1) / DL_B;
     F *v = scratch, *carry = scratch + nblocks + 1, *zp = carry + nblocks + 1;
-    hipLaunchKernelGGL(k_divlin_local, GRID(nblocks), 0, s, q, p, len, z, v, zp); HIP_LAUNCH_CHECK();
+    hipLaunchKernelGGL(k_divlin_local, GRID(nblocks), 0, s, q, p, len, G29::twiddle_from_std(z), v, zp); HIP_LAUNCH_CHECK();
     divlin_rec(carry, v, nblocks, z.pow_u64(DL_B), zp + DL_B, s);
     hipLaunchKernelGGL(k_divlin_apply, GRID(len - 1), 0, s, q, len - 1, (const F *)zp, (const F *)carry, nblocks); HIP_LAUNCH_CHECK();
 }
@@ -162,20 +152,20 @@
 }
 
 constexpr size_t EV_CHUNK = 16, EV_COMBINE_MAX = 1024;
-__global__ void k_eval_chunks(const F *__restrict__ p, size_t len, F x, F *__restrict__ partial) {
+__global__ void k_eval_chunks(const F *__restrict__ p, size_t len, G29 x, F *__restrict__ partial) {
     size_t t = (size_t)blockIdx.x * blockDim.x + threadIdx.x;
     size_t nch = (len + EV_CHUNK - 1) / EV_CHUNK;
     if (t >= nch) return;
     size_t s0 = t * EV_CHUNK, e = s0 + EV_CHUNK < len ? s0 + EV_CHUNK : len;
-    F acc = F::zero();
-    for (size_t i = e; i-- > s0;) acc = acc * x + p[i];
-    partial[t] = acc;
-}
-__global__ void __launch_bounds__(256) k_eval_combine(const F *__restrict__ partial, size_t nch, F y, F *__restrict__ out) {
+    partial[t] = st29(PL::horner_chunk(p, s0, e, x));
+}
+__global__ void __launch_bounds__(256) k_eval_combine(const F *__restrict__ partial, size_t nch, G29 y, F *__restrict__ out) {
     __shared__ F sh[256];
     uint32_t t = threadIdx.x;
-    F y256 = y.pow_u64(256), pw = y.pow_u64(t), acc = F::zero();
-    for (size_t i = t; i < nch; i += 256) { acc = acc + partial[i] * pw; pw = pw * y256; }
+    const G29 y256 = PL::pow_tw(y, 256);
+    G29 pw = PL::pow_tw(y, t);
+    F acc = F::zero();
+    for (size_t i = t; i < nch; i += 256) { acc = acc + st29(ld29(partial[i]) * pw); pw = pw * y256; }
     sh[t] = acc;
     __syncthreads();
     for (int s = 128; s > 0; s >>= 1) { if ((int)t < s) sh[t] = sh[t] + sh[t + s]; __syncthreads(); }
@@ -192,10 +182,10 @@
     F y = x;
     do {
         size_t nch = (n + EV_CHUNK - 1) / EV_CHUNK;
-        hipLaunchKernelGGL(k_eval_chunks, GRID(nch), 0, s, src, n, y, scratch); HIP_LAUNCH_CHECK();
+        hipLaunchKernelGGL(k_eval_chunks, GRID(nch), 0, s, src, n, G29::twiddle_from_std(y), scratch); HIP_LAUNCH_CHECK();
         src = scratch; scratch += nch; n = nch; y = y.pow_u64(EV_CHUNK);
     } while (n > EV_COMBINE_MAX);
-    hipLaunchKernelGGL(k_eval_combine, dim3(1), dim3(256), 0, s, src, n, y, out); HIP_LAUNCH_CHECK();
+    hipLaunchKernelGGL(k_eval_combine, dim3(1), dim3(256), 0, s, src, n, G29::twiddle_from_std(y), out); HIP_LAUNCH_CHECK();
 }
 void poly_eval_multi(const F *const *p, const size_t *len, const F *x, int count, F *out, F *scratch, size_t scratch_elems, stream_t s_) {
     hipStream_t s = (hipStream_t)s_;
@@ -263,10 +253,12 @@
 }
 constexpr int VQ_MAX_COSETS = 3, VQ_STEP = 10;
 struct VqArgs { F *out[VQ_MAX_COSETS]; const F *tab; const F *elems; uint32_t n; int lg_n; bool unit_g[VQ_MAX_COSETS]; };
-__device__ __forceinline__ F vq_factor(const VqArgs &A, int c, int k, uint32_t j) {
-    const F e = A.elems[(size_t)j << k];
-    return A.tab[k] + (A.unit_g[c] ? e : e * A.tab[(size_t)(c + 1) * A.lg_n + k]);
-}
+__device__ __forceinline__ G29 vq_factor(const VqArgs &A, int c, int k, uint32_t j) {
+    const G29 e = ld29(A.elems[(size_t)j << k]);
+    return ld29(A.tab[k]) + (A.unit_g[c] ? e : e * ld29(A.tab[(size_t)(c + 1) * A.lg_n + k]));
+}
+__device__ __forceinline__ F vq_pack(const G29 &g) { F r; g.pack(r.l); return r; }
+__device__ __forceinline__ G29 vq_node(const G29 &factor, const F &parent) { return factor.shl5() * ld29(parent); }
 __global__ void __launch_bounds__(1024) k_vq_top(VqArgs A, F *__restrict__ mid) {
     __shared__ F buf[2][1 << VQ_STEP];
     const int c = blockIdx.x, L = A.lg_n, k_stop = L > VQ_STEP ? L - VQ_STEP : 0;
@@ -276,13 +268,13 @@
     int cur = 0;
     for (int k = L - 1; k >= k_stop; k--) {
         const uint32_t s = A.n >> k;
-        if (t < s) buf[cur ^ 1][t] = vq_factor(A, c, k, t) * buf[cur][t & ((s >> 1) - 1)];
+        if (t < s) buf[cur ^ 1][t] = vq_pack(vq_node(vq_factor(A, c, k, t), buf[cur][t & ((s >> 1) - 1)]));
         __syncthreads();
         cur ^= 1;
     }
     const uint32_t s = A.n >> k_stop;
     F *dst = k_stop == 0 ? A.out[c] : mid + (size_t)c * (1u << VQ_STEP);
-    if (t < s) dst[t] = buf[cur][t];
+    if (t < s) dst[t] = st29(ld29(buf[cur][t]));
 }
 __global__ void __launch_bounds__(256) k_vq_expand(VqArgs A, const F *__restrict__ src, F *__restrict__ dst, int k_hi, int k_lo) {
     __shared__ F buf[2][1 << VQ_STEP];
@@ -292,15 +284,15 @@
     if (t == 0) buf[0][0] = src[(size_t)c * s_hi + j];
     __syncthreads();
     int cur = 0;
-    for (int k = k_hi - 1; k >= k_lo; k--) {
+    for (int k = k_hi - 1; k > k_lo; k--) {
         const uint32_t cnt = 1u << (k_hi - k);
-        for (uint32_t m = t; m < cnt; m += 256) buf[cur ^ 1][m] = vq_factor(A, c, k, j + m * s_hi) * buf[cur][m & ((cnt >> 1) - 1)];
+        for (uint32_t m = t; m < cnt; m += 256) buf[cur ^ 1][m] = vq_pack(vq_node(vq_factor(A, c, k, j + m * s_hi), buf[cur][m & ((cnt >> 1) - 1)]));
         __syncthreads();
         cur ^= 1;
     }
     const uint32_t cnt = 1u << (k_hi - k_lo);
     F *o = k_lo == 0 ? A.out[c] : dst + (size_t)c * (A.n >> k_lo);
-    for (uint32_t m = t; m < cnt; m += 256) o[j + (size_t)m * s_hi] = buf[cur][m];
+    for (uint32_t m = t; m < cnt; m += 256) o[j + (size_t)m * s_hi] = st29(vq_node(vq_factor(A, c, k_lo, j + m * s_hi), buf[cur][m & ((cnt >> 1) - 1)]));
 }
 static inline int vq_next_level(int k_hi) { const int r = k_hi % VQ_STEP; return k_hi - (r ? r : VQ_STEP); }
 size_t vanishing_quotient_scratch(int lg_n, int ncosets) {
@@ -322,7 +314,7 @@
     for (int c = 0; c < ncosets; c++) {
         A.unit_g[c] = g[c] == F::one();
         v = g[c];
-        for (int k = 0; k < lg_n; k++) { tab[(size_t)(c + 1) * lg_n + k] = v; v = v.sqr(); }
+        for (int k = 0; k < lg_n; k++) { G29::twiddle_from_std(v).pack(tab[(size_t)(c + 1) * lg_n + k].l); v = v.sqr(); }
     }
     h2d(scratch, tab.data(), tab.size() * sizeof(F), s_);
     A.tab = scratch; A.elems = elems; A.n = n; A.lg_n = lg_n;
@@ -387,19 +379,23 @@
     hipLaunchKernelGGL(k_z_evals_h, GRID(n), 0, (hipStream_t)s, out, z, n, m, num_witness); HIP_LAUNCH_CHECK();
 }
 __global__ void k_q1_combine(F *__restrict__ h1, F *__restrict__ g1, const F *__restrict__ q0, const F *__restrict__ q1, const F *__restrict__ q3, const F *__restrict__ mask,
-                             F inv2, F inv2zeta, size_t n) {
+                             G29 i2, G29 i4, G29 i4z, size_t n) {
     size_t i = (size_t)blockIdx.x * blockDim.x + threadIdx.x;
     if (i >= n) return;
     const F a = q1[i], b = q3[i], c = q0[i];
-    const F q_mid = (a - b) * inv2zeta;
-    const F q_hi = ((c - q_mid) - (a + b) * inv2) * inv2;
+    const G29 ga = ld29(a), gb = ld29(b);
+    const G29 v[2] = {ld29(c), G29::zero().template sub<2>(ga + gb)}, w[2] = {i2, i4};
+    const G29 x = G29::dot<2>(v, w);
+    const G29 y = ga.template sub<1>(gb) * i4z;
     const F m_lo = mask[i], m_mid = mask[n + i], m_hi = mask[2 * n + i];
-    h1[i] = q_mid + q_hi + m_mid + m_hi;
-    h1[n + i] = q_hi + m_hi;
+    h1[i] = st29(x + y + ld29(m_mid + m_hi));
+    h1[n + i] = PL::st8(x.template sub<2>(y) + ld29(m_hi));
     if (i >= 1) g1[i - 1] = c + m_lo + m_mid + m_hi;
 }
 void q1_combine(F *h1, F *g1, const F *q0, const F *q1, const F *q3, const F *mask, const F &inv2, const F &inv2zeta, size_t n, stream_t s) {
-    hipLaunchKernelGGL(k_q1_combine, GRID(n), 0, (hipStream_t)s, h1, g1, q0, q1, q3, mask, inv2, inv2zeta, n); HIP_LAUNCH_CHECK();
+    const F inv4 = inv2 * inv2;
+    hipLaunchKernelGGL(k_q1_combine, GRID(n), 0, (hipStream_t)s, h1, g1, q0, q1, q3, mask, G29::twiddle_from_std(inv2), G29::twiddle_from_std(inv4),
+                       G29::twiddle_from_std(inv2zeta * inv2), n); HIP_LAUNCH_CHECK();
 }
 __global__ void k_coset_scale(F *__restrict__ out, const F *__restrict__ in, F g, size_t in_len, size_t n) {
     size_t t = (size_t)blockIdx.x * blockDim.x + threadIdx.x;
diff --git a/aes_zero_knowledge_proof_circuit_amd/csrc/kernels_witness.hip b/aes_zero_knowledge_proof_circuit_amd/csrc/kernels_witness.hip
--- a/aes_zero_knowledge_proof_circuit_amd/csrc/kernels_witness.hip
+++ b/aes_zero_knowledge_proof_circuit_amd/csrc/kernels_witness.hip
@@ -1,11 +1,14 @@
 #include <mutex>
 #include "hip_util.hpp"
+#include "poly29.cuh"
 #include "trace_layout.h"
 
 namespace zk {
 namespace gpu {
 
 #define GRID(n) dim3((unsigned)(((n) + 255) / 256)), dim3(256)
+using G29 = Fp29<Fr377P>;
+using PL = Poly29<Fr377P>;
 
 static uint8_t *g_sbox_dev[64] = {nullptr};
 static std::mutex g_sbox_mu;
@@ -452,19 +455,14 @@
 void bits_to_field(F *out, const uint8_t *z, size_t n, stream_t s) { if (!n) return; hipLaunchKernelGGL(k_bits_to_field, GRID(n), 0, (hipStream_t)s, out, z, n); HIP_LAUNCH_CHECK(); }
 
 __global__ void k_t_partials(F *__restrict__ partial, uint32_t nseg, const uint32_t *__restrict__ seg_start, const uint32_t *__restrict__ seg_end, const uint32_t *__restrict__ row,
-                             const uint8_t *__restrict__ mat, const int64_t *__restrict__ coeff, const F *__restrict__ r_alpha, F eta_a, F eta_b, F eta_c) {
+                             const uint8_t *__restrict__ mat, const int64_t *__restrict__ coeff, const F *__restrict__ r_alpha, G29 eta_a, G29 eta_b, G29 eta_c, G29 rr2) {
     uint32_t sgi = blockIdx.x * blockDim.x + threadIdx.x;
     if (sgi >= nseg) return;
-    F acc = F::zero();
-    for (uint32_t i = seg_start[sgi]; i < seg_end[sgi]; i++) {
-        F eta = mat[i] == 0 ? eta_a : (mat[i] == 1 ? eta_b : eta_c);
-        long long c = coeff[i];
-        F term = eta * r_alpha[row[i]];
-        if (c == 1) acc = acc + term;
-        else if (c == -1) acc = acc - term;
-        else acc = acc + term * small_to_field(c);
-    }
-    partial[sgi] = acc;
+    static_assert(T_SEG <= 32, "the value bound of a segment's sums (<= 64 p) is written for at most 32 entries");
+    G29 S[3] = {G29::zero(), G29::zero(), G29::zero()};
+    for (uint32_t i = seg_start[sgi]; i < seg_end[sgi]; i++) PL::t_segment_add(S, mat[i], coeff[i], PL::ld(r_alpha[row[i]]), rr2);
+    const G29 eta[3] = {eta_a, eta_b, eta_c};
+    partial[sgi] = PL::t_segment_finish(S, eta);
 }
 __global__ void k_t_columns(F *__restrict__ out, uint32_t n, const uint32_t *__restrict__ col_seg_ptr, const F *__restrict__ partial) {
     uint32_t h = blockIdx.x * blockDim.x + threadIdx.x;
@@ -487,7 +485,10 @@
 }
 void t_evals(F *out, uint32_t n, F *partial, uint32_t nseg, const uint32_t *col_seg_ptr, const uint32_t *seg_start, const uint32_t *seg_end, const uint32_t *heavy, uint32_t n_heavy,
              const uint32_t *row, const uint8_t *mat, const int64_t *coeff, const F *r_alpha, const F &eta_a, const F &eta_b, const F &eta_c, stream_t s) {
-    if (nseg) { hipLaunchKernelGGL(k_t_partials, GRID(nseg), 0, (hipStream_t)s, partial, nseg, seg_start, seg_end, row, mat, coeff, r_alpha, eta_a, eta_b, eta_c); HIP_LAUNCH_CHECK(); }
+    if (nseg) {
+        hipLaunchKernelGGL(k_t_partials, GRID(nseg), 0, (hipStream_t)s, partial, nseg, seg_start, seg_end, row, mat, coeff, r_alpha, G29::twiddle_from_std(eta_a), G29::twiddle_from_std(eta_b),
+                           G29::twiddle_from_std(eta_c), PL::twiddle_rr2()); HIP_LAUNCH_CHECK();
+    }
     hipLaunchKernelGGL(k_t_columns, GRID(n), 0, (hipStream_t)s, out, n, col_seg_ptr, partial); HIP_LAUNCH_CHECK();
     if (n_heavy) { hipLaunchKernelGGL(k_t_heavy, dim3(n_heavy), dim3(256), 0, (hipStream_t)s, out, heavy, col_seg_ptr, partial); HIP_LAUNCH_CHECK(); }
 }
diff --git a/aes_zero_knowledge_proof_circuit_amd/csrc/poly29.cuh b/aes_zero_knowledge_proof_circuit_amd/csrc/poly29.cuh
--- /dev/null
+++ b/aes_zero_knowledge_proof_circuit_amd/csrc/poly29.cuh
@@ -0,0 +1,73 @@
+#pragma once
+#include "ff29.cuh"
+
+#ifndef ZK_POLY29_BOUND
+#define ZK_POLY29_BOUND(g, K)
+#endif
+
+namespace zk {
+
+template <class P>
+struct Poly29 {
+    using F = Fp<P>;
+    using G = Fp29<P>;
+
+    ZK_HD static G ld(const F &x) { return G::split(x.l); }
+    ZK_HD static F st(const G &g) { ZK_POLY29_BOUND(g, 4); F r; g.template canonical<1>().pack(r.l); return r; }
+    ZK_HD static F st8(const G &g) { ZK_POLY29_BOUND(g, 8); F r; g.template canonical<2>().pack(r.l); return r; }
+    ZK_HD static F st_tw(const G &g) { return st(g); }
+    ZK_HD static G one_tw() { return G::twiddle_from_std(F::one()); }
+    ZK_HD static G pow_tw(const G &zt, uint64_t e) {
+        G r = one_tw(), b = zt;
+        for (; e; e >>= 1) { if (e & 1) r = r * b; if (e > 1) b = b * b; }
+        return r;
+    }
+    ZK_HD static G twiddle_rr2() { F v = F::r2(); for (int i = 0; i < 2 * (261 - 32 * P::N); i++) v = v.dbl(); return G::split(v.l); }
+    ZK_HD static G small_tw(uint64_t mag, const G &rr2) {
+        uint32_t w[P::N];
+        for (int i = 0; i < P::N; i++) w[i] = 0;
+        w[0] = (uint32_t)mag; w[1] = (uint32_t)(mag >> 32);
+        return G::split(w) * rr2;
+    }
+
+    ZK_HD static G divlin_block(F *q, const F *p, size_t s0, size_t e, size_t len, const G &zt) {
+        size_t i = e - 1;
+        if (e < len) q[i] = F::zero();
+        G l = ld(p[i]);
+        while (i-- > s0) {
+            q[i] = st(l);
+            l = ld(p[i]) + l * zt;
+            ZK_POLY29_BOUND(l, 3);
+        }
+        return l;
+    }
+    ZK_HD static F divlin_apply(const F &q, const G &zp, const G &carry) { return st(ld(q) + carry * zp); }
+
+    ZK_HD static G horner_chunk(const F *p, size_t s0, size_t e, const G &xt) {
+        if (e <= s0) return G::zero();
+        G acc = ld(p[e - 1]);
+        for (size_t i = e - 1; i-- > s0;) acc = (acc * xt).add_lazy(ld(p[i]));
+        ZK_POLY29_BOUND(acc, 3);
+        return acc.normalized();
+    }
+
+    ZK_HD static void t_segment_add(G S[3], int m, long long c, const G &r, const G &rr2) {
+        G term;
+        if (c == 1) term = r;
+        else if (c == -1) term = G::zero().template sub<1>(r);
+        else {
+            const bool neg = c < 0;
+            const G prod = r * small_tw(neg ? 0ull - (unsigned long long)c : (unsigned long long)c, rr2);
+            term = neg ? G::zero().template sub<2>(prod) : prod;
+        }
+        if (m == 0) S[0] = S[0] + term; else if (m == 1) S[1] = S[1] + term; else S[2] = S[2] + term;
+    }
+    ZK_HD static F t_segment_finish(const G S[3], const G eta[3]) {
+        ZK_POLY29_BOUND(S[0] + S[1] + S[2], 65);
+        const G v = G::template dot<3>(S, eta);
+        ZK_POLY29_BOUND(v, 2);
+        return st(v);
+    }
+};
+
+}
diff --git a/include/zkaes.h b/include/zkaes.h
--- a/include/zkaes.h
+++ b/include/zkaes.h
@@ -143,6 +143,8 @@
 int zkaes_q1_coset_pointwise(const uint8_t *r, const uint8_t *za, const uint8_t *zb, const uint8_t *t, const uint8_t *z, const uint8_t consts[192], size_t n, uint8_t *out);
 int zkaes_h2_coset(const uint8_t *const arrays[7], const uint8_t consts[224], size_t k, uint8_t *out);
 int zkaes_q1_combine(const uint8_t *q0, const uint8_t *q1, const uint8_t *q3, const uint8_t *mask, const uint8_t inv2[32], const uint8_t inv2zeta[32], size_t n, uint8_t *h1, uint8_t *g1);
+int zkaes_poly_scale(uint8_t *p, size_t n, const uint8_t sc[32]);
+int zkaes_t_evals(uint32_t n, const uint32_t *colptr, const uint32_t *row, const uint8_t *mat, const int64_t *coeff, const uint8_t *r_alpha, uint32_t n_rows, const uint8_t etas[96], uint8_t *out);
 int zkaes_coset_scale(const uint8_t *in, size_t in_len, const uint8_t g[32], size_t n, uint8_t *out);
 int zkaes_z_poly_from_w(const uint8_t *w, size_t wlen, const uint8_t *x_poly, uint32_t m, size_t n, uint8_t *zp);
 int zkaes_ntt_padded(int field_id, const uint8_t *in, size_t in_len, size_t n, int inverse, int coset_c, int lg_big, uint8_t *out);
```

Result: no change. 98.37 (median of 6 runs) (+0.4%).
